# hwwang55/GraphGAN

Measured on AMD Instinct MI355X. Metric: sampled_edges_per_sec, higher is better.
Workload: dtype f32

## Files before the change

graphgan_amd/_lib.py:

```python
from __future__ import annotations

import ctypes
import os

_HERE = os.path.dirname(os.path.abspath(__file__))
LIB_PATH = os.path.join(_HERE, "libgraphgan_hip.so")
HEADER_PATH = os.path.join(os.path.dirname(_HERE), "include", "graphgan_hip.h")
ABI_VERSION = 9


def header_abi_version(path=HEADER_PATH):
    import re
    with open(path) as f:
        m = re.search(r"^#define\s+GG_ABI_VERSION\s+(\d+)", f.read(), flags=re.M)
    if not m:
        raise RuntimeError("GG_ABI_VERSION not found in %s" % path)
    return int(m.group(1))

GG_OK, GG_EINVAL, GG_ECAPACITY, GG_EHIP, GG_ECOMM, GG_ENOMEM, GG_EIO = 0, -1, -2, -3, -4, -5, -6
GG_OPT_ADAM_DENSE, GG_OPT_ADAM_LAZY, GG_OPT_SGD = 0, 1, 2
GG_ROOT_OK, GG_ROOT_ABORTED, GG_ROOT_EMPTY = 0, 1, 2
GG_GS_FOR_D, GG_GS_Q3_STORE = 1, 2
GRAM_MAX_GRID = 512
PAIR_NEIGHBORS_CHUNK = 512
NEIGHBOR_SUM_CHUNK = 512
NEIGHBOR_SUM_MAX_COL = 128
NEIGHBOR_MODE_LDS_CAP = 2048
TWO_HOP_LDS_CAP = 2048
PPR_LDS_CAP = 1024
PARTITION_EDGES_CHUNK = 512
SF_MAX_SWEEPS = 34
ERROR_NAMES = {GG_EINVAL: "GG_EINVAL", GG_ECAPACITY: "GG_ECAPACITY", GG_EHIP: "GG_EHIP", GG_ECOMM: "GG_ECOMM",
               GG_ENOMEM: "GG_ENOMEM", GG_EIO: "GG_EIO"}


class GGConfig(ctypes.Structure):
    _fields_ = [("lr_gen", ctypes.c_float), ("lr_dis", ctypes.c_float),
                ("lambda_gen", ctypes.c_float), ("lambda_dis", ctypes.c_float),
                ("adam_beta1", ctypes.c_float), ("adam_beta2", ctypes.c_float), ("adam_eps", ctypes.c_float),
                ("window_size", ctypes.c_int32), ("optimizer", ctypes.c_int32), ("device", ctypes.c_int32),
                ("reserved", ctypes.c_int32 * 6)]


class GGCounters(ctypes.Structure):
    _fields_ = [("walks", ctypes.c_int64), ("hops", ctypes.c_int64), ("nbr_reads", ctypes.c_int64),
                ("reward_pairs", ctypes.c_int64), ("d_pairs", ctypes.c_int64), ("g_pairs", ctypes.c_int64),
                ("d_steps", ctypes.c_int64), ("g_steps", ctypes.c_int64),
                ("last_kernel_ms", ctypes.c_double), ("walk_kernel_ms", ctypes.c_double),
                ("walk_launches", ctypes.c_int64), ("rows_scored", ctypes.c_int64), ("score_kernel_ms", ctypes.c_double),
                ("score_launches", ctypes.c_int64), ("score_chunks", ctypes.c_int64), ("score_rows", ctypes.c_int64),
                ("bfs_kernel_ms", ctypes.c_double), ("bfs_trees", ctypes.c_int64), ("score_dists", ctypes.c_int64),
                ("reward_kernel_ms", ctypes.c_double), ("reward_pairs_timed", ctypes.c_int64),
                ("d_grad_ms", ctypes.c_double), ("d_opt_ms", ctypes.c_double), ("d_pairs_timed", ctypes.c_int64), ("d_rows_timed", ctypes.c_int64),
                ("g_grad_ms", ctypes.c_double), ("g_opt_ms", ctypes.c_double), ("g_pairs_timed", ctypes.c_int64), ("g_rows_timed", ctypes.c_int64),
                ("d_passes_timed", ctypes.c_int64), ("g_passes_timed", ctypes.c_int64),
                ("g_walk_nodes_timed", ctypes.c_int64),
                ("es_gathers", ctypes.c_int64), ("es_nodes", ctypes.c_int64), ("score_gathers", ctypes.c_int64), ("score_nodes", ctypes.c_int64),
                ("walk_reruns", ctypes.c_int64)]


class GGGraph(ctypes.Structure):
    _fields_ = [("n_node", ctypes.c_int32), ("nnz", ctypes.c_int64), ("n_train_edges", ctypes.c_int64),
                ("n_test_edges", ctypes.c_int64), ("rowptr", ctypes.POINTER(ctypes.c_int64)), ("col", ctypes.POINTER(ctypes.c_int32))]


class GraphGANHipError(RuntimeError):
    def __init__(self, code, msg):
        super().__init__("%s (%d): %s" % (ERROR_NAMES.get(code, "GG_E?"), code, msg))
        self.code = code


_P = ctypes.c_void_p
_i32, _i64, _u32, _u64 = ctypes.c_int32, ctypes.c_int64, ctypes.c_uint32, ctypes.c_uint64

SIGNATURES = {
    "gg_abi_version": (ctypes.c_int, []),
    "gg_last_error": (ctypes.c_char_p, [_P]),
    "gg_create": (ctypes.c_int, [_i32, _i32, _P, _P, ctypes.POINTER(GGConfig), ctypes.POINTER(_P)]),
    "gg_destroy": (ctypes.c_int, [_P]),
    "gg_set_graph_csr": (ctypes.c_int, [_P, _P, _P]),
    "gg_host_build_trees": (_i64, [_i32, _P, _P, _P, _i32, _P, _P, _P, _i64, _i32, _P]),
    "gg_build_trees": (ctypes.c_int, [_P, _P, _i32, _i32]),
    "gg_build_trees_device": (ctypes.c_int, [_P, _P, _i32]),
    "gg_set_tree_mode": (ctypes.c_int, [_P, _i32, _i64]),
    "gg_debug_words": (ctypes.c_int, [_P, _i32, _i32, _P]),
    "gg_lazy_stats": (ctypes.c_int, [_P, _P]),
    "gg_get_lazy_trees": (ctypes.c_int, [_P, _P, _P, _P, _P, _P, _P, _P]),
    "gg_set_trees": (ctypes.c_int, [_P, _P, _i32, _P, _P, _P, _i32]),
    "gg_tree_info": (ctypes.c_int, [_P, _P, _P, _P]),
    "gg_tree_roots": (ctypes.c_int, [_P, _P]),
    "gg_save_trees": (ctypes.c_int, [_P, ctypes.c_char_p]),
    "gg_load_trees": (ctypes.c_int, [_P, ctypes.c_char_p]),
    "gg_get_trees": (ctypes.c_int, [_P, _P, _P, _P]),
    "gg_get_tree_order": (ctypes.c_int, [_P, _P, _P, _P, _P, _P]),
    "gg_walk_sample": (ctypes.c_int, [_P, _P, _P, _i32, _i32, _u64, _u32, _P, _P, _P, _i32, _P]),
    "gg_walk_info": (ctypes.c_int, [_P, _P, _P, _P]),
    "gg_get_walks": (ctypes.c_int, [_P, _P, _P, _P, _P]),
    "gg_prepare_d": (ctypes.c_int, [_P, _P, _i32, _u64, _u32, _P, _P]),
    "gg_get_d_data": (ctypes.c_int, [_P, _P, _P, _P]),
    "gg_prepare_g": (ctypes.c_int, [_P, _P, _i32, _i32, _u64, _u32, _P, _P]),
    "gg_prepare_g_begin": (ctypes.c_int, [_P, _P, _i32, _i32, _u64, _u32]),
    "gg_get_g_data": (ctypes.c_int, [_P, _P, _P, _P]),
    "gg_epoch_begin": (ctypes.c_int, [_P, _i32, _i32]),
    "gg_epoch_add": (ctypes.c_int, [_P, _P, _i32, _i32, _i32, _i32, _u64, _u32, _u32, _P, _P]),
    "gg_epoch_commit": (ctypes.c_int, [_P, _i32, _P]),
    "gg_q3_clear": (ctypes.c_int, [_P]),
    "gg_q3_get": (ctypes.c_int, [_P, _P, _P]),
    "gg_d_pass": (ctypes.c_int, [_P, _P, _i64, _i32]),
    "gg_g_pass": (ctypes.c_int, [_P, _P, _i64, _i32]),
    "gg_pair_reward": (ctypes.c_int, [_P, _P, _P, _i64, _P]),
    "gg_d_step": (ctypes.c_int, [_P, _P, _P, _P, _i32]),
    "gg_g_step": (ctypes.c_int, [_P, _P, _P, _P, _i32]),
    "gg_all_score": (ctypes.c_int, [_P, _P, _i32, _P]),
    "gg_all_score_reduce": (ctypes.c_int, [_P, _P, _i32, _i32, _i32, _P, _P, _P, _P]),
    "gg_topk_scores": (ctypes.c_int, [_P, _i32, _P, _i32, _i32, _i32, _i32, _P, _P, _P]),
    "gg_topk_metric": (ctypes.c_int, [_P, _i32, _P, _i32, _i32, _i32, _i32, _i32, _P, _i64, _P, _P, _P]),
    "gg_rank_scores": (ctypes.c_int, [_P, _i32, _P, _P, _i64, _i32, _i32, _P, _P, _P, _P]),
    "gg_top_pairs": (ctypes.c_int, [_P, _i32, _i32, _P, _i64, _i64, _i32, _i64, _P, _P, _P, _P, _P, _P]),
    "gg_distinct_degrees": (ctypes.c_int, [_P, _P]),
    "gg_pair_neighbors": (ctypes.c_int, [_P, _P, _P, _i64, _P, _i32, _P, _P, _P, _P, _P]),
    "gg_neighbor_sum": (ctypes.c_int, [_P, _P, _i32, _P, _P, _P, _i64, _P, _P]),
    "gg_label_spread": (ctypes.c_int, [_P, _P, _P, _i64, _i32, ctypes.c_double, _i32, _P, _P, _P, _i64, _P, _P, _P]),
    "gg_neighbor_mode": (ctypes.c_int, [_P, _P, _u32, _i32, _P, _i64, _P, _P]),
    "gg_label_propagation": (ctypes.c_int, [_P, _u32, _i32, _P, _P, _P, _P, _P]),
    "gg_partition_edges": (ctypes.c_int, [_P, _P, _i32, _P, _P, _P]),
    "gg_undirected_edges": (ctypes.c_int, [_P, _P, _P]),
    "gg_spanning_forest": (ctypes.c_int, [_P, _u32, _P, _i64, _P, _P, _P, _P, _P, _P]),
    "gg_two_hop_topk": (ctypes.c_int, [_P, _P, _i64, _i32, _P, _i32, _i64, _P, _P, _P, _P]),
    "gg_two_hop_rank": (ctypes.c_int, [_P, _P, _P, _i64, _P, _i32, _i64, _P, _P, _P, _P, _P]),
    "gg_ppr_topk": (ctypes.c_int, [_P, _P, _i64, _i32, _u32, _u64, _i32, _i32, _i64, _P, _P, _P, _P, _P, _P, _P]),
    "gg_ppr_rank": (ctypes.c_int, [_P, _P, _P, _i64, _u32, _u64, _i32, _i32, _i64, _P, _P, _P, _P, _P, _P, _P, _P]),
    "gg_graph_softmax": (ctypes.c_int, [_P, _P, _i32, _i32, _P, _P, _P, _P, _P, _P]),
    "gg_pretrain_set_noise": (ctypes.c_int, [_P, _P]),
    "gg_pretrain_set_walk_bias": (ctypes.c_int, [_P, _u32, _u32, _u32]),
    "gg_prepare_pretrain": (ctypes.c_int, [_P, _P, _i32, _i32, _i32, _i32, _i32, _u64, _u32, _P, _P, _P]),
    "gg_classifier_lossgrad": (ctypes.c_int, [_P, ctypes.c_int, _P, _P, _i64, ctypes.c_int, _P, _P, ctypes.c_float, _P, _P, _P]),
    "gg_classifier_fit": (ctypes.c_int, [_P, ctypes.c_int, _P, _P, _i64, ctypes.c_int, ctypes.c_int, ctypes.c_float, ctypes.c_float, _P, _P, _P, _P]),
    "gg_classifier_predict": (ctypes.c_int, [_P, ctypes.c_int, _P, _i64, ctypes.c_int, _P, _P, _P, _P]),
    "gg_classifier_ml_lossgrad": (ctypes.c_int, [_P, ctypes.c_int, _P, _P, _i64, ctypes.c_int, _P, _P, ctypes.c_float, _P, _P, _P]),
    "gg_classifier_ml_fit": (ctypes.c_int, [_P, ctypes.c_int, _P, _P, _i64, ctypes.c_int, ctypes.c_int, ctypes.c_float, ctypes.c_float, _P, _P, _P, _P]),
    "gg_classifier_ml_predict": (ctypes.c_int, [_P, ctypes.c_int, _P, _i64, ctypes.c_int, _P, _P, _P, _P, _P]),
    "gg_edge_classifier_lossgrad": (ctypes.c_int, [_P, ctypes.c_int, ctypes.c_int, _P, _P, _P, _i64, _P, _P, ctypes.c_float, _P, _P, _P]),
    "gg_edge_classifier_fit": (ctypes.c_int, [_P, ctypes.c_int, ctypes.c_int, _P, _P, _P, _i64, ctypes.c_int, ctypes.c_float, ctypes.c_float,
                                               _P, _P, _P, _P]),
    "gg_edge_classifier_predict": (ctypes.c_int, [_P, ctypes.c_int, ctypes.c_int, _P, _P, _i64, _P, _P, _P]),
    "gg_kmeans_step": (ctypes.c_int, [_P, ctypes.c_int, _P, _i64, ctypes.c_int, _P, _P, _P, _P, _P, _P, _P]),
    "gg_kmeans_fit": (ctypes.c_int, [_P, ctypes.c_int, _P, _i64, ctypes.c_int, ctypes.c_int, _P, _P, _P, _P, _P, _P, _P, _P, _P]),
    "gg_silhouette": (ctypes.c_int, [_P, ctypes.c_int, _P, _P, _i64, ctypes.c_int, _P, _i64, ctypes.c_int, _P, _P, _P, _P, _P, _P]),
    "gg_gram": (ctypes.c_int, [_P, ctypes.c_int, _P, _i64, _P, _P, _P, _P]),
    "gg_get_embeddings": (ctypes.c_int, [_P, _i32, _P]),
    "gg_get_bias": (ctypes.c_int, [_P, _i32, _P]),
    "gg_write_embeddings": (ctypes.c_int, [_P, _i32, ctypes.c_char_p, _i32]),
    "gg_host_write_embeddings": (ctypes.c_int, [_P, _i64, _i32, ctypes.c_char_p, _i32]),
    "gg_write_embeddings_bin": (ctypes.c_int, [_P, _i32, ctypes.c_char_p]),
    "gg_edge_scores": (ctypes.c_int, [_P, _i32, _P, _P, _i64, _P]),
    "gg_set_embeddings": (ctypes.c_int, [_P, _i32, _P]),
    "gg_set_bias": (ctypes.c_int, [_P, _i32, _P]),
    "gg_save_state": (ctypes.c_int, [_P, ctypes.c_char_p]),
    "gg_load_state": (ctypes.c_int, [_P, ctypes.c_char_p]),
    "gg_get_counters": (ctypes.c_int, [_P, ctypes.POINTER(GGCounters)]),
    "gg_set_profiling": (ctypes.c_int, [_P, _i32]),
    "gg_set_profiling_solo": (ctypes.c_int, [_P, _i32]),
    "gg_synchronize": (ctypes.c_int, [_P]),
    "gg_comm_unique_id": (ctypes.c_int, [_P]),
    "gg_comm_init": (ctypes.c_int, [_P, _P, _i32, _i32]),
    "gg_comm_barrier": (ctypes.c_int, [_P]),
    "gg_comm_stats": (ctypes.c_int, [_P, _P]),
    "gg_comm_stats_ex": (ctypes.c_int, [_P, _P]),
    "gg_synth_powerlaw": (_i64, [_i32, _i32, _u64, _u64, _P, _i64]),
    "gg_host_read_edges": (ctypes.c_int, [ctypes.c_char_p, ctypes.c_char_p, ctypes.POINTER(GGGraph)]),
    "gg_host_free_graph": (None, [ctypes.POINTER(GGGraph)]),
}


def _load():
    if not os.path.exists(LIB_PATH):
        raise ImportError(
            "graphgan_amd: %s is missing -- build the HIP extension first "
            "(`make -C graphgan_amd/csrc` or `python -c 'import __graft_entry__ as g; g.build()'`). "
            "There is no CPU fallback." % LIB_PATH)
    lib = ctypes.CDLL(LIB_PATH)
# ... 19 lines not shown
```

graphgan_amd/csrc/epoch.hip:

```cpp
#include <algorithm>
#include <vector>

#include "gg_internal.h"

namespace gg {

int launch_pair_reward(gg_ctx *ctx, const int32_t *d_u, const int32_t *d_v, int64_t n, float *d_out);

__global__ __launch_bounds__(256) void q3_copy_kernel(const int32_t *t_root, const int64_t *t_q3off, uint32_t *t_q3, const int64_t *s_off,
                                                      uint32_t *store, int n_slots, int to_store) {
    const int s = blockIdx.x * blockDim.x + threadIdx.x;
    if (s >= n_slots) return;
    const int v = t_root[s];
    const int64_t a = t_q3off[s], b = s_off[v], words = min(t_q3off[s + 1] - a, s_off[v + 1] - b);
    for (int64_t k = 0; k < words; ++k) {
        if (to_store) store[b + k] = t_q3[a + k];
        else t_q3[a + k] = store[b + k];
    }
}

static int ensure_q3_store(gg_ctx *ctx) {
    if (ctx->q3_store_ready) return GG_OK;
    GG_CHECK(ctx, !ctx->h_rowptr.empty(), GG_EINVAL, "epoch: call gg_set_graph_csr first");
    const int n = ctx->n_node;
// ... 35 lines not shown
    if (rc != GG_OK) return rc;
    if (add) GG_HIP(ctx, hipMemcpyAsync((char *)acc.p + elem * (size_t)have, src.p, elem * (size_t)add, hipMemcpyDeviceToDevice, ctx->stream));
    return GG_OK;
}

}

using namespace gg;

extern "C" {

int gg_epoch_begin(gg_ctx *ctx, int32_t reset_d, int32_t reset_g) {
    if (!ctx) return fail(nullptr, GG_EINVAL, "ctx is NULL");
    GG_HIP(ctx, hipSetDevice(ctx->device));
    int rc = ensure_q3_store(ctx);
    if (rc != GG_OK) return rc;
    if (reset_d) {
        ctx->ep_rows = 0;
        ctx->ep_d_open = true;
    }
    if (reset_g) ctx->ep_pairs = 0;
    return GG_OK;
}

int gg_epoch_add(gg_ctx *ctx, const int32_t *roots, int32_t n_roots, int32_t do_d, int32_t do_g, int32_t n_sample, uint64_t seed,
                 uint32_t stream_d, uint32_t stream_g, int64_t *rows_total_out, int64_t *pairs_total_out) {
    if (!ctx) return fail(nullptr, GG_EINVAL, "ctx is NULL");
    GG_CHECK(ctx, n_roots >= 0 && (roots || n_roots == 0), GG_EINVAL, "gg_epoch_add: bad roots");
    if (n_roots > 1 && (do_d || do_g)) {
        std::vector<int32_t> sorted(roots, roots + n_roots);
        std::sort(sorted.begin(), sorted.end());
        const auto dup = std::adjacent_find(sorted.begin(), sorted.end());
        GG_CHECK(ctx, dup == sorted.end(), GG_EINVAL, "gg_epoch_add: root %d appears twice in one batch", dup == sorted.end() ? -1 : *dup);
    }
    GG_HIP(ctx, hipSetDevice(ctx->device));
    int rc = ensure_q3_store(ctx);
    if (rc != GG_OK) return rc;
    if (n_roots > 0 && (do_d || do_g)) {
        ctx->in_epoch_add = true;
        rc = gg_build_trees_device(ctx, roots, n_roots);
        ctx->in_epoch_add = false;
        if (rc != GG_OK) return rc;
        rc = q3_copy(ctx, n_roots, false);
        if (rc != GG_OK) return rc;
        std::vector<int32_t> &slots = ctx->ep_slots;
        if ((int32_t)slots.size() < n_roots) {
            const int32_t old = (int32_t)slots.size();
            slots.resize(n_roots);
            for (int32_t i = old; i < n_roots; ++i) slots[i] = i;
        }
        ctx->in_epoch_add = true;
        if (do_d) {
            ctx->ep_d_open = true;
            int64_t rows = 0;
            rc = gg_prepare_d(ctx, slots.data(), n_roots, seed, stream_d, &rows, nullptr);
            if (rc == GG_OK) rc = q3_copy(ctx, n_roots, true);
            if (rc == GG_OK) rc = append(ctx, ctx->ep_center, ctx->d_center, ctx->ep_rows, rows, sizeof(int32_t));
            if (rc == GG_OK) rc = append(ctx, ctx->ep_neighbor, ctx->d_neighbor, ctx->ep_rows, rows, sizeof(int32_t));
            if (rc == GG_OK) rc = append(ctx, ctx->ep_label, ctx->d_label, ctx->ep_rows, rows, sizeof(float));
            if (rc == GG_OK) ctx->ep_rows += rows;
        }
        if (rc == GG_OK && do_g) {
            int64_t pairs = 0;
            rc = gg_prepare_g(ctx, slots.data(), n_roots, n_sample, seed, stream_g, &pairs, nullptr);
            if (rc == GG_OK) rc = ensure_g_pairs(ctx);
            if (rc == GG_OK) rc = append(ctx, ctx->ep_node1, ctx->g_node1, ctx->ep_pairs, pairs, sizeof(int32_t));
            if (rc == GG_OK) rc = append(ctx, ctx->ep_node2, ctx->g_node2, ctx->ep_pairs, pairs, sizeof(int32_t));
            if (rc == GG_OK) ctx->ep_pairs += pairs;
        }
        ctx->in_epoch_add = false;
        if (rc != GG_OK) return rc;
        GG_HIP(ctx, hipStreamSynchronize(ctx->stream));
    }
    if (rows_total_out) *rows_total_out = ctx->ep_rows;
    if (pairs_total_out) *pairs_total_out = ctx->ep_pairs;
    return GG_OK;
}

int gg_epoch_commit(gg_ctx *ctx, int32_t which, int64_t *n_out) {
    if (!ctx) return fail(nullptr, GG_EINVAL, "ctx is NULL");
    GG_CHECK(ctx, which == 0 || which == 1, GG_EINVAL, "gg_epoch_commit: which must be 0 (generator pairs) or 1 (discriminator rows)");
    GG_HIP(ctx, hipSetDevice(ctx->device));
    discard_begun_walk(ctx);
    GG_HIP(ctx, hipStreamSynchronize(ctx->stream));
    int rc;
    if (which == 1) {
        const int64_t rows = ctx->ep_rows;
        GG_HIP(ctx, ctx->ep_center.reserve(sizeof(int32_t)));
        GG_HIP(ctx, ctx->ep_neighbor.reserve(sizeof(int32_t)));
        GG_HIP(ctx, ctx->ep_label.reserve(sizeof(float)));
        std::swap(ctx->d_center, ctx->ep_center);
        std::swap(ctx->d_neighbor, ctx->ep_neighbor);
        std::swap(ctx->d_label, ctx->ep_label);
        ctx->d_rows = rows;
        ctx->ep_rows = 0;
        ctx->ep_d_open = false;
        rc = exchange_count_max(ctx, ctx->d_rows, &ctx->d_rows_max);
        if (rc != GG_OK) return rc;
        if (n_out) *n_out = rows;
    } else {
        const int64_t pairs = ctx->ep_pairs;
        GG_HIP(ctx, ctx->ep_node1.reserve(sizeof(int32_t)));
        GG_HIP(ctx, ctx->ep_node2.reserve(sizeof(int32_t)));
        GG_HIP(ctx, ctx->ep_reward.reserve(sizeof(float) * (size_t)(pairs + 1)));
        rc = launch_pair_reward(ctx, ctx->ep_node1.as<int32_t>(), ctx->ep_node2.as<int32_t>(), pairs, ctx->ep_reward.as<float>());
        if (rc != GG_OK) return rc;
        GG_HIP(ctx, hipStreamSynchronize(ctx->stream));
        std::swap(ctx->g_node1, ctx->ep_node1);
        std::swap(ctx->g_node2, ctx->ep_node2);
        std::swap(ctx->g_reward, ctx->ep_reward);
        ctx->g_pairs = pairs;
        ctx->g_pairs_filled = true;
        ctx->g_paths_valid = false;
        ctx->ep_pairs = 0;
        rc = exchange_count_max(ctx, ctx->g_pairs, &ctx->g_pairs_max);
        if (rc != GG_OK) return rc;
        if (n_out) *n_out = pairs;
    }
    return GG_OK;
}

int gg_q3_clear(gg_ctx *ctx) {
    if (!ctx) return fail(nullptr, GG_EINVAL, "ctx is NULL");
    GG_HIP(ctx, hipSetDevice(ctx->device));
    int rc = ensure_q3_store(ctx);
    if (rc != GG_OK) return rc;
    GG_HIP(ctx, hipStreamSynchronize(ctx->stream));
    GG_HIP(ctx, hipMemset(ctx->q3_store.p, 0, sizeof(uint32_t) * (size_t)std::max<int64_t>(ctx->q3_words, 1)));
    return GG_OK;
}

int gg_q3_get(gg_ctx *ctx, int64_t *word_off , uint32_t *words ) {
    if (!ctx) return fail(nullptr, GG_EINVAL, "ctx is NULL");
    GG_HIP(ctx, hipSetDevice(ctx->device));
    int rc = ensure_q3_store(ctx);
    if (rc != GG_OK) return rc;
    GG_HIP(ctx, hipStreamSynchronize(ctx->stream));
    if (word_off) GG_HIP(ctx, hipMemcpy(word_off, ctx->q3s_off.p, sizeof(int64_t) * (ctx->n_node + 1), hipMemcpyDeviceToHost));
    if (words && ctx->q3_words) GG_HIP(ctx, hipMemcpy(words, ctx->q3_store.p, sizeof(uint32_t) * (size_t)ctx->q3_words, hipMemcpyDeviceToHost));
    return GG_OK;
}

}
```

graphgan_amd/csrc/gg_api.hip:

```cpp
#include <stdarg.h>
#include <stdlib.h>
#include <string.h>
#include <sys/stat.h>
#include <unistd.h>

#include <algorithm>
#include <atomic>
#include <thread>

#include "gg_internal.h"

namespace gg {

thread_local std::string g_last_error;

int fail(gg_ctx *ctx, int code, const char *fmt, ...) {
    char buf[1024];
    va_list ap;
    va_start(ap, fmt);
    vsnprintf(buf, sizeof(buf), fmt, ap);
    va_end(ap);
    g_last_error = buf;
    if (ctx) ctx->err = buf;
    return code;
// ... 132 lines not shown
    }
    return GG_OK;
}

void gg::discard_begun_walk(gg_ctx *ctx) {
    if (!ctx->g_begun) return;
    (void)hipStreamSynchronize(ctx->stream2);
    ctx->g_begun = false;
    ctx->dc_request = 0;
    ctx->walk_stream = ctx->stream;
    ctx->w_nslots = 0;
    ctx->w_total = 0;
    generator_changed(ctx);
}

int gg::walk_launch_async(gg_ctx *ctx, const int32_t *slots, const int32_t *n_walks, int32_t uniform_walks, int32_t n_slots,
                          int32_t for_d, uint64_t seed, uint32_t stream, int32_t stride, bool side_stream, bool defer_join) {
    discard_begun_walk(ctx);
    GG_CHECK(ctx, ctx->n_tree_roots > 0 || n_slots == 0, GG_EINVAL, "walk: no trees loaded (gg_build_trees / gg_set_trees)");
    GG_CHECK(ctx, n_slots >= 0 && (slots || n_slots == 0), GG_EINVAL, "walk: bad slots");
    GG_CHECK(ctx, stride >= 2, GG_ECAPACITY, "walk: stride %d < 2", stride);
    std::vector<int64_t> &ptr = ctx->h_ptr_new;
    ptr.assign(n_slots + 1, 0);
    for (int i = 0; i < n_slots; ++i) {
        GG_CHECK(ctx, slots[i] >= 0 && slots[i] < ctx->n_tree_roots, GG_EINVAL, "walk: slot %d out of range", slots[i]);
        int64_t nw;
        if (n_walks) nw = n_walks[i];
        else if (uniform_walks >= 0) nw = uniform_walks;
        else {
            GG_CHECK(ctx, !ctx->h_rowptr.empty(), GG_EINVAL, "walk: graph CSR needed for D-mode degrees");
            const int r = ctx->h_troot[slots[i]];
            nw = ctx->h_rowptr[r + 1] - ctx->h_rowptr[r];
        }
        GG_CHECK(ctx, nw >= 0, GG_EINVAL, "walk: negative n_walks");
        ptr[i + 1] = ptr[i] + nw;
    }
    const int64_t total = ptr[n_slots];
    GG_HIP(ctx, hipSetDevice(ctx->device));
    const int mode = for_d ? 1 : 0;
    ctx->w_mode = mode;
    GG_HIP(ctx, ctx->w_slots_m[mode].reserve(sizeof(int32_t) * (n_slots + 1)));
    GG_HIP(ctx, ctx->w_ptr_m[mode].reserve(sizeof(int64_t) * (n_slots + 1)));
    GG_HIP(ctx, ctx->w_status.reserve(sizeof(int32_t) * (n_slots + 1)));
    GG_HIP(ctx, ctx->w_abort.reserve(sizeof(int32_t) * (n_slots + 1)));
    GG_HIP(ctx, ctx->w_samples.reserve(sizeof(int32_t) * (total + 1)));
    GG_HIP(ctx, ctx->w_len.reserve(sizeof(int32_t) * (total + 1)));
    GG_HIP(ctx, ctx->w_first.reserve(sizeof(int32_t) * (total + 1)));
    GG_HIP(ctx, ctx->w_paths.reserve(sizeof(int32_t) * ((size_t)total * stride + 1)));
    ctx->walk_stream = side_stream ? ctx->stream2 : ctx->stream;
    if (side_stream && ctx->gen_dirty) {
        GG_HIP(ctx, hipEventRecord(ctx->ev_main_mark, ctx->stream));
        GG_HIP(ctx, hipStreamWaitEvent(ctx->stream2, ctx->ev_main_mark, 0));
        ctx->gen_dirty = false;
    } else if (side_stream && ctx->gen_pass_recorded) {
        GG_HIP(ctx, hipStreamWaitEvent(ctx->stream2, ctx->ev_gen_pass, 0));
    }
    std::vector<int32_t> &hs = ctx->h_slots_m[mode];
    if (hs.size() != (size_t)n_slots || (n_slots && memcmp(hs.data(), slots, sizeof(int32_t) * n_slots) != 0)) {
        hs.assign(slots, slots + n_slots);
        if (n_slots) GG_HIP(ctx, hipMemcpyAsync(ctx->w_slots_m[mode].p, hs.data(), sizeof(int32_t) * n_slots, hipMemcpyHostToDevice, ctx->walk_stream));
    }
    if (ctx->h_ptr_m[mode] != ptr) {
        ctx->h_ptr_m[mode].swap(ptr);
        GG_HIP(ctx, hipMemcpyAsync(ctx->w_ptr_m[mode].p, ctx->h_ptr_m[mode].data(), sizeof(int64_t) * (n_slots + 1), hipMemcpyHostToDevice, ctx->walk_stream));
    }
    ctx->w_total = total;
    ctx->w_stride = stride;
    ctx->w_nslots = n_slots;
    ctx->w_uniform = (!n_walks && uniform_walks >= 0) ? uniform_walks : -1;
    ctx->w_args = {for_d, seed, stream};
    ctx->g_paths_valid = false;
    if (ctx->g_slots_ready) {
        GG_HIP(ctx, hipStreamWaitEvent(ctx->stream, ctx->ev_slots_done, 0));
        ctx->g_slots_ready = false;
        ctx->g_slots_unused++;
    }
    if (n_slots == 0) {
        ctx->walk_stream = ctx->stream;
        return GG_OK;
    }
    return launch_and_join(ctx, n_slots, total, for_d, seed, stream, stride, !defer_join);
}

int gg::walk_finalize(gg_ctx *ctx, bool *retried) {
    if (retried) *retried = false;
    if (ctx->w_nslots == 0) {
        GG_HIP(ctx, hipStreamSynchronize(ctx->stream));
        return GG_OK;
    }
    const int64_t total = ctx->w_total;
    unsigned long long *c = ctx->h_pin;
    constexpr int CW = gg_ctx::CTR_WORDS;
    GG_HIP(ctx, hipMemcpyAsync(c, ctx->dev_ctr, sizeof(unsigned long long) * 2 * CW, hipMemcpyDeviceToHost, ctx->stream));
    GG_HIP(ctx, hipStreamSynchronize(ctx->stream));
    harvest_timings(ctx);
    for (int attempt = 0; c[3] == 2ull || (c[2] != 0ull && ctx->t_lazy); ++attempt) {
        GG_CHECK(ctx, attempt < 16, GG_EHIP, "walk: the launch was voided %d times in a row", attempt);
        if (c[2] != 0ull && ctx->t_lazy) {
            int rebuilt = 0;
            int rc = lazy_fallback_rebuild(ctx, &rebuilt);
            if (rc == GG_ECAPACITY) rc = lazy_rebuild_whole(ctx);
            if (rc != GG_OK) return rc;
            if (ctx->dc_request == 2) ctx->dc_request = 0;
            if (ctx->tree_max_depth + 3 > ctx->w_stride) {
                ctx->w_stride = ctx->tree_max_depth + 3;
                GG_HIP(ctx, ctx->w_paths.reserve(sizeof(int32_t) * ((size_t)total * ctx->w_stride + 1)));
            }
        } else {
            ctx->walk_force_sized = true;
        }
        ctx->ctr.walk_reruns += 1;
        generator_changed(ctx);
        int rc = launch_and_join(ctx, ctx->w_nslots, total, ctx->w_args.for_d, ctx->w_args.seed, ctx->w_args.stream, ctx->w_stride);
        ctx->walk_force_sized = false;
        if (rc != GG_OK) return rc;
        GG_HIP(ctx, hipMemcpyAsync(c, ctx->dev_ctr, sizeof(unsigned long long) * 2 * CW, hipMemcpyDeviceToHost, ctx->stream));
        GG_HIP(ctx, hipStreamSynchronize(ctx->stream));
        if (retried) *retried = true;
    }
    const int n_half = ctx->w_split ? 2 : 1;
    if (n_half == 2)
        for (int i = 8; i < CW; ++i) c[i] += c[CW + i];
    {
        int64_t *prof = ctx->alive_prof[ctx->w_args.for_d ? 1 : 0];
        const int run = ctx->w_levels_run;
        for (int i = 0; i < 64; ++i) prof[i] = i < run ? (int64_t)c[8 + i] : -1;
        if (run > 0 && run < 64 && ctx->w_fin_follows) prof[run] = (int64_t)c[7];
        if (ctx->w_net && c[7] > 2048ull && ctx->lv_levels_learned < ctx->tree_max_depth + 2) ctx->lv_levels_learned += 1;
    }
    unsigned long long hops = c[0], reads = c[1], rows = c[5];
    unsigned long long gathers = 0, nodes = 0;
    for (int i = 0; i < 64; ++i) { hops += c[264 + i]; reads += c[328 + i]; rows += c[200 + i]; gathers += c[520 + i]; nodes += c[584 + i]; }
    ctx->ctr.es_gathers += (int64_t)gathers;
    ctx->ctr.es_nodes += (int64_t)nodes;
    ctx->ctr.hops += (int64_t)hops;
    ctx->ctr.nbr_reads += (int64_t)reads;
    ctx->ctr.rows_scored += (int64_t)rows;
    ctx->ctr.walks += total;
    if (total && ctx->walk_timed) {
        float ms = 0.f;
        GG_HIP(ctx, hipEventElapsedTime(&ms, ctx->ev0, ctx->ev1));
        ctx->ctr.last_kernel_ms = ms;
        ctx->ctr.walk_kernel_ms += ms;
        ctx->ctr.walk_launches += 1;
        for (int i = 0; i < ctx->lv_ev_used; ++i) {
            float lms = 0.f;
            for (int k = 0; k < n_half; ++k) {
                float e = 0.f;
                GG_HIP(ctx, hipEventElapsedTime(&e, ctx->lv_ev[4 * i + 2 * k], ctx->lv_ev[4 * i + 2 * k + 1]));
                lms += e;
            }
            ctx->ctr.score_kernel_ms += lms;
            ctx->ctr.score_launches += n_half;
            ctx->ctr.score_chunks += (int64_t)(c[136 + i] >> 32);
            if (getenv("GG_WALK_DEBUG"))
                fprintf(stderr, "[walk] for_d=%d level %d alive %llu score chunks %llu prefix chunks %llu big %llu small %llu rows %llu score %.1f us\n", ctx->w_args.for_d, i,
                        c[8 + i], c[136 + i] >> 32, c[136 + i] & 0xffffffffull, c[72 + i] & 0xffffffffull, c[72 + i] >> 32, c[456 + i], lms * 1e3);
        }
        if (ctx->lv_ev_used) {
            ctx->ctr.score_rows += (int64_t)(rows - c[5]);
            unsigned long long dists = 0;
            for (int i = 0; i < 64; ++i) dists += c[392 + i];
            ctx->ctr.score_dists += (int64_t)dists;
            ctx->ctr.score_gathers += (int64_t)gathers;
            ctx->ctr.score_nodes += (int64_t)nodes;
        }
    }
    if (c[3] || c[6]) generator_changed(ctx);
    if (c[3]) return fail(ctx, GG_ECAPACITY, "walk: a path needed more than stride=%d entries", ctx->w_stride);
    if (c[6]) return fail(ctx, GG_EINVAL, "walk: non-finite generator scores (a softmax had total weight 0, or the generator's tables hold a non-finite value)");
    return GG_OK;
}

int gg::walk_resident(gg_ctx *ctx, const int32_t *slots, const int32_t *n_walks, int32_t uniform_walks, int32_t n_slots,
                      int32_t for_d, uint64_t seed, uint32_t stream, int32_t stride) {
    int rc = walk_launch_async(ctx, slots, n_walks, uniform_walks, n_slots, for_d, seed, stream, stride);
    if (rc != GG_OK) return rc;
    return walk_finalize(ctx, nullptr);
}

extern "C" {

int gg_abi_version(void) { return GG_ABI_VERSION; }

const char *gg_last_error(const gg_ctx *ctx) { return ctx ? ctx->err.c_str() : g_last_error.c_str(); }

int gg_create(int32_t n_node, int32_t n_emb, const float *emb_gen, const float *emb_dis, const gg_config *cfg,
              gg_ctx **out) {
    if (!out) return fail(nullptr, GG_EINVAL, "gg_create: out is NULL");
    *out = nullptr;
    if (n_node <= 0 || n_emb <= 0 || n_emb > 512 || !emb_gen || !emb_dis || !cfg)
        return fail(nullptr, GG_EINVAL, "gg_create: bad argument (n_node=%d n_emb=%d)", n_node, n_emb);
    if (cfg->window_size < 1) return fail(nullptr, GG_EINVAL, "gg_create: window_size = %d is below 1", cfg->window_size);
    int ndev = 0;
    hipError_t e = hipGetDeviceCount(&ndev);
    if (e != hipSuccess || ndev <= 0)
        return fail(nullptr, GG_EHIP, "gg_create: no HIP device (%s); this engine has no CPU fallback",
                    e == hipSuccess ? "count = 0" : hipGetErrorString(e));
    if (cfg->device < 0 || cfg->device >= ndev) return fail(nullptr, GG_EINVAL, "gg_create: device %d of %d", cfg->device, ndev);
    hipDeviceProp_t prop;
    GG_HIP(nullptr, hipGetDeviceProperties(&prop, cfg->device));
    if (strncmp(prop.gcnArchName, "gfx950", 6) != 0)
        return fail(nullptr, GG_EHIP, "gg_create: device %d is %s; kernels are built for gfx950 only", cfg->device, prop.gcnArchName);
    GG_HIP(nullptr, hipSetDevice(cfg->device));

    gg_ctx *ctx = new gg_ctx();
    ctx->n_node = n_node;
    ctx->n_emb = n_emb;
    ctx->ld = (n_emb + 3) / 4 * 4;
    ctx->cfg = *cfg;
    ctx->device = cfg->device;
    ctx->n_cus = prop.multiProcessorCount > 0 ? prop.multiProcessorCount : 256;
    if (const char *lv = getenv("GG_WALK_LEVELS")) ctx->walk_levels = atoi(lv);
    if (const char *pe = getenv("GG_PROFILE_EVERY")) ctx->profile_every = std::max(0, atoi(pe));
    if (const char *fw = getenv("GG_COMM_FAKE_WORLD")) ctx->fake_world = atoi(fw);
    if (const char *ow = getenv("GG_COMM_OWNER")) ctx->owner_exchange = atoi(ow);
    if (const char *bf = getenv("GG_COMM_BF16")) ctx->comm_bf16 = atoi(bf) != 0;
    if (const char *om = getenv("GG_COMM_OWNER_MIN")) ctx->owner_min_bound = atoll(om);
    if (const char *dt = getenv("GG_DETERMINISTIC")) ctx->deterministic = atoi(dt) != 0;
    if (const char *nc = getenv("GG_NO_DIST_CACHE")) ctx->dc_enabled = atoi(nc) == 0;
    if (const char *ft = getenv("GG_FIN_THRESHOLD")) ctx->fin_threshold = std::max(0, atoi(ft));
    if (const char *st = getenv("GG_STAGE_T")) ctx->sg_threshold = std::max(0, atoi(st));
    if (const char *ws = getenv("GG_WALK_SPLIT")) ctx->split_enabled = atoi(ws) != 0;
    if (const char *em = getenv("GG_ES_MODE")) ctx->es_mode = std::min(2, std::max(0, atoi(em)));
    if (const char *er = getenv("GG_ES_RATIO")) ctx->es_ratio_num = std::max(1, atoi(er));
    if (const char *eh = getenv("GG_ES_HUB")) ctx->es_hub = std::max(0, atoi(eh));
    if (const char *wm = getenv("GG_WALK_SPLIT_MIN")) ctx->split_min_walks = std::max(512, atoi(wm));
    for (auto &m : ctx->alive_prof) for (auto &v : m) v = -1;
    if (const char *dr = getenv("GG_COMM_DENSE_RATIO")) ctx->dense_exchange_ratio = (float)atof(dr);
#define GG_TRY(call)                        \
    do {                                    \
        int rc__ = (call);                  \
        if (rc__ != GG_OK) {                \
            g_last_error = ctx->err;        \
            gg_destroy(ctx);                \
            return rc__;                    \
        }                                   \
    } while (0)
    auto body = [&]() -> int {
        GG_HIP(ctx, hipStreamCreateWithFlags(&ctx->stream, hipStreamNonBlocking));
        {
            int lo = 0, hi = 0;
            const char *wp = getenv("GG_WALK_PRIORITY");
            if (wp && atoi(wp) != 0 && hipDeviceGetStreamPriorityRange(&lo, &hi) == hipSuccess && hi != lo)
                GG_HIP(ctx, hipStreamCreateWithPriority(&ctx->stream2, hipStreamNonBlocking, atoi(wp) > 0 ? hi : lo));
            else
                GG_HIP(ctx, hipStreamCreateWithFlags(&ctx->stream2, hipStreamNonBlocking));
        }
        GG_HIP(ctx, hipStreamCreateWithFlags(&ctx->stream3, hipStreamNonBlocking));
        GG_HIP(ctx, hipEventCreateWithFlags(&ctx->ev_fork, hipEventDisableTiming));
        GG_HIP(ctx, hipEventCreateWithFlags(&ctx->ev_join, hipEventDisableTiming));
        GG_HIP(ctx, hipEventCreateWithFlags(&ctx->ev_score[0], hipEventDisableTiming));
        GG_HIP(ctx, hipEventCreateWithFlags(&ctx->ev_score[1], hipEventDisableTiming));
        ctx->walk_stream = ctx->stream;
        GG_HIP(ctx, hipEventCreate(&ctx->ev0));
        GG_HIP(ctx, hipEventCreate(&ctx->ev1));
        GG_HIP(ctx, hipEventCreateWithFlags(&ctx->ev_walk_done, hipEventDisableTiming));
        GG_HIP(ctx, hipEventCreateWithFlags(&ctx->ev_gen_pass, hipEventDisableTiming));
        GG_HIP(ctx, hipEventCreateWithFlags(&ctx->ev_main_mark, hipEventDisableTiming));
        GG_HIP(ctx, hipHostMalloc((void **)&ctx->h_pin, sizeof(unsigned long long) * gg_ctx::PIN_WORDS, hipHostMallocDefault));
        memset(ctx->h_pin, 0, sizeof(unsigned long long) * gg_ctx::PIN_WORDS);
        const size_t tb = sizeof(float) * (size_t)n_node * ctx->ld, vb = sizeof(float) * (size_t)n_node;
        for (int m = 0; m < 2; ++m) {
            Model &M = ctx->model[m];
            GG_HIP(ctx, hipMalloc((void **)&M.E, tb));
            GG_HIP(ctx, hipMalloc((void **)&M.b, vb));
            GG_HIP(ctx, hipMemset(M.b, 0, vb));
            if (cfg->optimizer != GG_OPT_SGD) {
                GG_HIP(ctx, hipMalloc((void **)&M.mE, tb));
                GG_HIP(ctx, hipMalloc((void **)&M.vE, tb));
                GG_HIP(ctx, hipMalloc((void **)&M.mb, vb));
                GG_HIP(ctx, hipMalloc((void **)&M.vb, vb));
                GG_HIP(ctx, hipMemset(M.mE, 0, tb));
                GG_HIP(ctx, hipMemset(M.vE, 0, tb));
                GG_HIP(ctx, hipMemset(M.mb, 0, vb));
                GG_HIP(ctx, hipMemset(M.vb, 0, vb));
            }
            M.b1p = cfg->adam_beta1;
            M.b2p = cfg->adam_beta2;
            M.lr = m == 0 ? cfg->lr_gen : cfg->lr_dis;
            M.lambda = m == 0 ? cfg->lambda_gen : cfg->lambda_dis;
            int rc = upload_table(ctx, M.E, m == 0 ? emb_gen : emb_dis);
            if (rc != GG_OK) return rc;
        }
        GG_HIP(ctx, hipMalloc((void **)&ctx->gradE, tb));
        GG_HIP(ctx, hipMalloc((void **)&ctx->gradb, vb));
        GG_HIP(ctx, hipMemset(ctx->gradE, 0, tb));
        ctx->grad_elems_padded = (size_t)n_node * ctx->ld;
        GG_HIP(ctx, hipMemset(ctx->gradb, 0, vb));
        GG_HIP(ctx, hipMalloc((void **)&ctx->touched, sizeof(int32_t) * n_node));
        GG_HIP(ctx, hipMalloc((void **)&ctx->touched_list, sizeof(int32_t) * n_node));
        GG_HIP(ctx, hipMalloc((void **)&ctx->touched_cnt, sizeof(int32_t) * 4));
        GG_HIP(ctx, hipMemset(ctx->touched, 0, sizeof(int32_t) * n_node));
        GG_HIP(ctx, hipMemset(ctx->touched_cnt, 0, sizeof(int32_t) * 4));
        GG_HIP(ctx, hipMalloc((void **)&ctx->dev_ctr, sizeof(unsigned long long) * gg_ctx::PIN_WORDS));
        GG_HIP(ctx, hipMemset(ctx->dev_ctr, 0, sizeof(unsigned long long) * gg_ctx::PIN_WORDS));
        GG_HIP(ctx, ctx->table_bad.reserve(sizeof(unsigned long long) * 2));
        for (int m = 0; m < 2; ++m) {
            int rc = rescan_table_finite(ctx, m);
            if (rc != GG_OK) return rc;
        }
        GG_HIP(ctx, hipDeviceSynchronize());
        return GG_OK;
    };
    GG_TRY(body());
#undef GG_TRY
    *out = ctx;
    return GG_OK;
}

int gg_destroy(gg_ctx *ctx) {
    if (!ctx) return GG_OK;
    (void)hipSetDevice(ctx->device);
    if (ctx->stream) (void)hipStreamSynchronize(ctx->stream);
    if (ctx->stream2) (void)hipStreamSynchronize(ctx->stream2);
    comm_destroy(ctx);
    for (int m = 0; m < 2; ++m) {
        Model &M = ctx->model[m];
        float *ps[] = {M.E, M.b, M.mE, M.vE, M.mb, M.vb};
        for (float *p : ps)
            if (p) (void)hipFree(p);
    }
    void *ps[] = {ctx->gradE, ctx->gradb, ctx->touched, ctx->touched_list, ctx->touched_cnt, ctx->g_rowptr, ctx->g_col, ctx->dev_ctr,
                  ctx->es, ctx->es_stamp, ctx->g_rev};
    for (void *p : ps)
        if (p) (void)hipFree(p);
    free_trees(ctx);
    DevBuf *bufs[] = {&ctx->w_slots_m[0], &ctx->w_slots_m[1], &ctx->w_ptr_m[0], &ctx->w_ptr_m[1], &ctx->w_samples, &ctx->w_paths, &ctx->w_len, &ctx->w_status,
                      &ctx->w_first, &ctx->w_abort, &ctx->w_scratch, &ctx->d_center, &ctx->d_neighbor, &ctx->d_label, &ctx->d_cnt,
                      &ctx->d_ptr, &ctx->g_node1, &ctx->g_node2, &ctx->g_reward, &ctx->g_cnt, &ctx->g_ptr, &ctx->scan_tmp,
                      &ctx->step_u, &ctx->step_v, &ctx->step_x, &ctx->sg_rows, &ctx->sg_bias, &ctx->touched_ptr, &ctx->x_cnt, &ctx->x_send_ids, &ctx->x_send_rows,
                      &ctx->x_recv_ids, &ctx->x_recv_rows, &ctx->x_nglob, &ctx->x_own, &ctx->st_item, &ctx->st_item2, &ctx->st_cur, &ctx->st_prev, &ctx->st_len,
                      &ctx->st_alive, &ctx->st_rank, &ctx->bfs_key, &ctx->bfs_bm, &ctx->bfs_misc, &ctx->bfs_sparse, &ctx->bfs_rowptr32, &ctx->lv_pfx, &ctx->dc_keys, &ctx->dc_vals, &ctx->dc_words, &ctx->lv_beg, &ctx->lv_k, &ctx->lv_chunks, &ctx->lv_coff, &ctx->lv_scores, &ctx->lv_chunk_owner, &ctx->lv_prefix, &ctx->lv_big, &ctx->lv_fe, &ctx->fin_list, &ctx->table_bad, &ctx->hub_acc,
                      &ctx->q3_store, &ctx->q3s_off, &ctx->ep_center, &ctx->ep_neighbor, &ctx->ep_label, &ctx->ep_node1, &ctx->ep_node2, &ctx->ep_reward, &ctx->topk_adj,
                      &ctx->gs_es, &ctx->gs_cpre, &ctx->pt_starts, &ctx->pt_paths, &ctx->pt_len, &ctx->pt_cnt, &ctx->pt_ptr, &ctx->pt_noise, &ctx->pt_sample};
    for (DevBuf *b : bufs) b->release();
    ctx->set.release();
    for (StageIndex *ix : {&ctx->sg_own, &ctx->sg_early}) ix->release();
    for (hipEvent_t e : ctx->lv_ev)
        if (e) (void)hipEventDestroy(e);
    for (auto &tr : ctx->tm_ev)
        for (hipEvent_t e : tr)
            if (e) (void)hipEventDestroy(e);
    for (hipEvent_t e : ctx->pt_ev)
        if (e) (void)hipEventDestroy(e);
    if (ctx->h_pin) (void)hipHostFree(ctx->h_pin);
    for (hipEvent_t e : {ctx->ev_walk_done, ctx->ev_slots_done, ctx->ev_gen_pass, ctx->ev_main_mark, ctx->ev_fork, ctx->ev_join, ctx->ev_score[0], ctx->ev_score[1]})
        if (e) (void)hipEventDestroy(e);
    if (ctx->stream3) {
        (void)hipStreamSynchronize(ctx->stream3);
        (void)hipStreamDestroy(ctx->stream3);
    }
    if (ctx->stream2) {
        (void)hipStreamSynchronize(ctx->stream2);
        (void)hipStreamDestroy(ctx->stream2);
    }
    if (ctx->ev0) (void)hipEventDestroy(ctx->ev0);
    if (ctx->ev1) (void)hipEventDestroy(ctx->ev1);
    if (ctx->stream) (void)hipStreamDestroy(ctx->stream);
    delete ctx;
    return GG_OK;
}

int gg_set_graph_csr(gg_ctx *ctx, const int64_t *rowptr, const int32_t *col) {
    if (!ctx) return fail(nullptr, GG_EINVAL, "ctx is NULL");
    GG_CHECK(ctx, rowptr && rowptr[0] == 0, GG_EINVAL, "gg_set_graph_csr: rowptr[0] must be 0");
    discard_begun_walk(ctx);
    const int n = ctx->n_node;
    const int64_t nnz = rowptr[n];
    GG_CHECK(ctx, nnz >= 0 && (col || nnz == 0), GG_EINVAL, "gg_set_graph_csr: col is NULL");
    for (int v = 0; v < n; ++v) GG_CHECK(ctx, rowptr[v + 1] >= rowptr[v], GG_EINVAL, "gg_set_graph_csr: rowptr not monotone at %d", v);
    for (int64_t e = 0; e < nnz; ++e) GG_CHECK(ctx, col[e] >= 0 && col[e] < n, GG_EINVAL, "gg_set_graph_csr: col[%lld]=%d out of range", (long long)e, col[e]);
    GG_HIP(ctx, hipSetDevice(ctx->device));
    (void)hipDeviceSynchronize();
    for (void *p : {(void *)ctx->g_rowptr, (void *)ctx->g_col, (void *)ctx->es, (void *)ctx->es_stamp, (void *)ctx->g_rev})
        if (p) (void)hipFree(p);
    ctx->g_rowptr = nullptr;
    ctx->g_col = nullptr;
    ctx->es = nullptr;
    ctx->es_stamp = nullptr;
    ctx->g_rev = nullptr;
    ctx->t_edge_valid = false;
    ctx->q3_store_ready = false;
    ctx->bfs_rowptr32_valid = false;
    ctx->topk_adj.release();
    ctx->topk_adj_valid = false;
    ctx->set.drop();
    ctx->gs_es_valid = ctx->gs_cpre_valid = false;
    ctx->pt_noise_set = false;
    GG_HIP(ctx, hipMalloc((void **)&ctx->g_rowptr, sizeof(int64_t) * (n + 1)));
    GG_HIP(ctx, hipMalloc((void **)&ctx->g_col, sizeof(int32_t) * (std::max<int64_t>(nnz, 1) + 4)));
    GG_HIP(ctx, hipMemcpy(ctx->g_rowptr, rowptr, sizeof(int64_t) * (n + 1), hipMemcpyHostToDevice));
    if (nnz) GG_HIP(ctx, hipMemcpy(ctx->g_col, col, sizeof(int32_t) * nnz, hipMemcpyHostToDevice));
    ctx->g_nnz = nnz;
    ctx->g_max_deg = 0;
    for (int v = 0; v < n; ++v) ctx->g_max_deg = (int32_t)std::min<int64_t>(std::max<int64_t>(ctx->g_max_deg, rowptr[v + 1] - rowptr[v]), 0x7fffffff);
    ctx->g_multi = true;
    ctx->h_rowptr.assign(rowptr, rowptr + n + 1);
    ctx->h_col.assign(col, col + nnz);
    ctx->h_comp_size.clear();
    uint64_t h = 1469598103934665603ull;
    for (int v = 0; v <= n; ++v) h = (h ^ (uint64_t)rowptr[v]) * 1099511628211ull;
    for (int64_t e = 0; e + 1 < nnz; e += 2) h = (h ^ ((uint64_t)(uint32_t)col[e] | ((uint64_t)(uint32_t)col[e + 1] << 32))) * 1099511628211ull;
    if (nnz & 1) h = (h ^ (uint64_t)(uint32_t)col[nnz - 1]) * 1099511628211ull;
    ctx->g_hash = h;
    if (nnz > 0 && nnz < (1ll << 31)) {
        hipError_t e = hipMalloc((void **)&ctx->es, sizeof(float) * (size_t)nnz);
        if (e == hipSuccess) e = hipMalloc((void **)&ctx->es_stamp, sizeof(long long) * (size_t)n);
        if (e == hipSuccess) e = hipMalloc((void **)&ctx->g_rev, sizeof(int32_t) * (size_t)nnz);
        if (e == hipSuccess) e = hipMemset(ctx->es_stamp, 0, sizeof(long long) * (size_t)n);
        generator_changed(ctx);
        int rc = e == hipSuccess ? compute_reverse_edges(ctx) : GG_ENOMEM;
        if (rc != GG_OK) {
            (void)hipGetLastError();
            for (void *p : {(void *)ctx->es, (void *)ctx->es_stamp, (void *)ctx->g_rev})
                if (p) (void)hipFree(p);
            ctx->es = nullptr;
            ctx->es_stamp = nullptr;
            ctx->g_rev = nullptr;
            if (getenv("GG_WALK_DEBUG")) fprintf(stderr, "[graph] edge-score cache not allocated (%s): walks score privately\n", e == hipSuccess ? ctx->err.c_str() : hipGetErrorString(e));
        }
    }
    return GG_OK;
}

int gg_build_trees(gg_ctx *ctx, const int32_t *roots, int32_t n_roots, int32_t n_threads) {
    if (!ctx) return fail(nullptr, GG_EINVAL, "ctx is NULL");
    GG_CHECK(ctx, !ctx->h_rowptr.empty(), GG_EINVAL, "gg_build_trees: call gg_set_graph_csr first");
    GG_CHECK(ctx, n_roots >= 0 && (roots || n_roots == 0), GG_EINVAL, "gg_build_trees: bad roots");
    const int n = ctx->n_node;
// ... 240 lines not shown
                              sizeof(int32_t) * (2 * (size_t)h.nodes + (size_t)h.n_roots);
        if (fstat(fileno(f), &st) != 0 || (size_t)st.st_size != expect)
            rc = fail(ctx, GG_EIO, "gg_load_trees: %s is truncated (%lld bytes, expected %zu)", path, (long long)st.st_size, expect);
    }
    if (rc == GG_OK) {
        roots.resize(h.n_roots);
        base.resize((size_t)h.n_roots + 1);
        if (fread(roots.data(), sizeof(int32_t), h.n_roots, f) != (size_t)h.n_roots || fread(base.data(), sizeof(int64_t), (size_t)h.n_roots + 1, f) != (size_t)h.n_roots + 1)
            rc = fail(ctx, GG_EIO, "gg_load_trees: short read");
    }
    if (rc == GG_OK) {
        counts.resize(h.n_roots);
        for (int r = 0; r < h.n_roots && rc == GG_OK; ++r) {
            counts[r] = base[r + 1] - base[r];
            if (roots[r] < 0 || roots[r] >= ctx->n_node || counts[r] < 1 || counts[r] > ctx->n_node) rc = fail(ctx, GG_EIO, "gg_load_trees: %s: bad root table", path);
        }
        if (rc == GG_OK && (base[0] != 0 || base[h.n_roots] != h.nodes)) rc = fail(ctx, GG_EIO, "gg_load_trees: %s: bad root table", path);
    }
    if (rc == GG_OK) rc = alloc_trees(ctx, roots.data(), h.n_roots, counts.data(), nullptr);
    if (rc == GG_OK) rc = stream_dev(ctx, f, ctx->t_order, (size_t)h.nodes, false);
    if (rc == GG_OK) rc = stream_dev(ctx, f, ctx->t_cstart, (size_t)h.nodes + h.n_roots, false);
    fclose(f);
    if (rc == GG_OK) {
        int32_t *bad = (int32_t *)(ctx->dev_ctr + 2000);
        int32_t h_bad = 0;
        hipError_t e = hipMemset(bad, 0, sizeof(int32_t));
        if (e == hipSuccess) {
            hipLaunchKernelGGL(validate_trees_kernel, dim3((unsigned)cdiv(h.nodes, 256)), dim3(256), 0, ctx->stream, ctx->t_order, ctx->t_cstart,
                               ctx->t_base, ctx->t_root, h.n_roots, ctx->n_node, bad);
            e = hipStreamSynchronize(ctx->stream);
        }
        if (e == hipSuccess) e = hipMemcpy(&h_bad, bad, sizeof(int32_t), hipMemcpyDeviceToHost);
        if (e == hipSuccess) e = hipMemset(bad, 0, sizeof(int32_t));
        if (e != hipSuccess) rc = fail(ctx, GG_EHIP, "gg_load_trees: %s", hipGetErrorString(e));
        else if (h_bad || h.max_depth < 0 || h.max_depth > ctx->n_node || h.max_list < 0 || h.max_list > ctx->n_node)
            rc = fail(ctx, GG_EIO, "gg_load_trees: %s: the tree arrays are corrupt (node id out of range or child ranges not a BFS order)", path);
    }
    if (rc != GG_OK) {
        ctx->n_tree_roots = 0;
        ctx->tree_nodes = 0;
        return rc;
    }
    ctx->tree_max_depth = h.max_depth;
    ctx->tree_max_list = h.max_list;
    return derive_tree_edges(ctx);
}

int gg_walk_sample(gg_ctx *ctx, const int32_t *slots, const int32_t *n_walks, int32_t n_slots, int32_t for_d,
                   uint64_t seed, uint32_t stream, int32_t *samples, int32_t *paths, int32_t *path_len, int32_t stride,
                   int32_t *root_status) {
    if (!ctx) return fail(nullptr, GG_EINVAL, "ctx is NULL");
    GG_CHECK(ctx, n_walks || n_slots == 0, GG_EINVAL, "gg_walk_sample: n_walks is NULL");
    ctx->dc_request = 0;
    ctx->dc_valid = false;
    int rc = walk_resident(ctx, slots, n_walks, -1, n_slots, for_d ? 1 : 0, seed, stream, stride);
    if (rc != GG_OK) return rc;
    const int64_t total = ctx->w_total;
    if (samples && total) GG_HIP(ctx, hipMemcpy(samples, ctx->w_samples.p, sizeof(int32_t) * total, hipMemcpyDeviceToHost));
    if (path_len && total) GG_HIP(ctx, hipMemcpy(path_len, ctx->w_len.p, sizeof(int32_t) * total, hipMemcpyDeviceToHost));
    if (paths && total && ctx->w_stride == stride) GG_HIP(ctx, hipMemcpy(paths, ctx->w_paths.p, sizeof(int32_t) * (size_t)total * stride, hipMemcpyDeviceToHost));
    if (ctx->w_stride != stride && total) {
        std::vector<int32_t> len((size_t)total);
        GG_HIP(ctx, hipMemcpy(len.data(), ctx->w_len.p, sizeof(int32_t) * total, hipMemcpyDeviceToHost));
        for (int64_t w = 0; w < total; ++w)
            GG_CHECK(ctx, len[w] <= stride, GG_ECAPACITY, "walk: a path needed %d entries, stride is %d (gg_tree_info reports the depth of the trees as rebuilt)", len[w], stride);
        if (paths) GG_HIP(ctx, hipMemcpy2D(paths, sizeof(int32_t) * (size_t)stride, ctx->w_paths.p, sizeof(int32_t) * (size_t)ctx->w_stride, sizeof(int32_t) * (size_t)stride, (size_t)total, hipMemcpyDeviceToHost));
    }
    if (root_status && n_slots) GG_HIP(ctx, hipMemcpy(root_status, ctx->w_status.p, sizeof(int32_t) * n_slots, hipMemcpyDeviceToHost));
    return GG_OK;
}

int gg_debug_words(gg_ctx *ctx, int32_t first, int32_t n, uint64_t *out) {
    if (!ctx || !out || first < 0 || n < 0 || first + n > gg_ctx::PIN_WORDS) return fail(ctx, GG_EINVAL, "gg_debug_words: bad argument");
    GG_HIP(ctx, hipSetDevice(ctx->device));
    hipStream_t s;
    GG_HIP(ctx, hipStreamCreateWithFlags(&s, hipStreamNonBlocking));
    hipError_t e = hipMemcpyAsync(out, ctx->dev_ctr + first, sizeof(uint64_t) * (size_t)n, hipMemcpyDeviceToHost, s);
    if (e == hipSuccess) e = hipStreamSynchronize(s);
    (void)hipStreamDestroy(s);
    GG_HIP(ctx, e);
    return GG_OK;
}

int gg_set_tree_mode(gg_ctx *ctx, int32_t mode, int64_t node_cap) {
    if (!ctx) return fail(nullptr, GG_EINVAL, "ctx is NULL");
    GG_CHECK(ctx, mode >= -1 && mode <= 1 && node_cap >= 0, GG_EINVAL, "gg_set_tree_mode: mode must be -1 (auto), 0 (whole trees) or 1 (lazy), node_cap >= 0");
    ctx->tree_mode = mode;
    ctx->lz_cap = node_cap;
    return GG_OK;
}

int gg_lazy_stats(gg_ctx *ctx, int64_t *out8) {
    if (!ctx || !out8) return fail(ctx, GG_EINVAL, "gg_lazy_stats: NULL argument");
    GG_HIP(ctx, hipSetDevice(ctx->device));
    for (int i = 0; i < 24; ++i) out8[i] = 0;
    out8[0] = ctx->t_lazy ? 1 : 0;
    out8[1] = ctx->t_lazy ? ctx->lz_min_level : 0;
    out8[2] = ctx->lz_fallback_roots;
    out8[3] = ctx->lz_fallback_rounds;
    if (ctx->t_lazy && ctx->n_tree_roots > 0) {
        GG_HIP(ctx, hipStreamSynchronize(ctx->stream));
        const int R = ctx->n_tree_roots;
        std::vector<int4> info((size_t)R);
        std::vector<int32_t> cur((size_t)R);
        GG_HIP(ctx, hipMemcpy(info.data(), ctx->lz_info.p, sizeof(int4) * (size_t)R, hipMemcpyDeviceToHost));
        GG_HIP(ctx, hipMemcpy(cur.data(), ctx->lz_cursor.p, sizeof(int32_t) * (size_t)R, hipMemcpyDeviceToHost));
        for (int r = 0; r < R; ++r) {
            out8[4] += info[r].y;
            out8[5] += std::max(0, cur[r] - info[r].y);
            out8[6] += info[r].x < info[r].y ? 1 : 0;
            out8[7] = std::max<int64_t>(out8[7], info[r].z);
            if (info[r].x < info[r].y && info[r].z >= 0 && info[r].z < 8) out8[16 + info[r].z] += 1;
        }
        unsigned long long c[8];
        GG_HIP(ctx, hipMemcpy(c, ctx->dev_ctr + 1500, sizeof(c), hipMemcpyDeviceToHost));
        for (int i = 0; i < 8; ++i) out8[8 + i] = (int64_t)c[i];
    }
    return GG_OK;
}

int gg_get_lazy_trees(gg_ctx *ctx, int64_t *n_entries, int32_t *info4, int64_t *base, int32_t *order, int32_t *cstart, int32_t *edge, uint64_t *pair) {
    if (!ctx) return fail(nullptr, GG_EINVAL, "ctx is NULL");
    GG_CHECK(ctx, ctx->t_lazy, GG_EINVAL, "gg_get_lazy_trees: the resident trees are not lazy");
    GG_HIP(ctx, hipSetDevice(ctx->device));
    GG_HIP(ctx, hipDeviceSynchronize());
    const size_t R = (size_t)ctx->n_tree_roots, nodes = (size_t)ctx->arena_end;
    if (n_entries) *n_entries = (int64_t)nodes;
    if (info4) GG_HIP(ctx, hipMemcpy(info4, ctx->lz_info.p, sizeof(int4) * R, hipMemcpyDeviceToHost));
    if (base) GG_HIP(ctx, hipMemcpy(base, ctx->t_base, sizeof(int64_t) * R, hipMemcpyDeviceToHost));
    if (order) GG_HIP(ctx, hipMemcpy(order, ctx->t_order, sizeof(int32_t) * nodes, hipMemcpyDeviceToHost));
    if (cstart) GG_HIP(ctx, hipMemcpy(cstart, ctx->t_cstart, sizeof(int32_t) * (nodes + R), hipMemcpyDeviceToHost));
    if (edge) GG_HIP(ctx, hipMemcpy(edge, ctx->t_edge, sizeof(int32_t) * nodes, hipMemcpyDeviceToHost));
    if (pair) GG_HIP(ctx, hipMemcpy(pair, ctx->lz_pair.p, sizeof(uint64_t) * std::min(nodes, ctx->lz_pair.bytes / sizeof(uint64_t)), hipMemcpyDeviceToHost));
    return GG_OK;
}

int gg_walk_info(const gg_ctx *ctx, int64_t *total_walks, int32_t *stride, int32_t *n_slots) {
    if (!ctx) return fail(nullptr, GG_EINVAL, "ctx is NULL");
    if (total_walks) *total_walks = ctx->w_total;
    if (stride) *stride = ctx->w_stride;
    if (n_slots) *n_slots = ctx->w_nslots;
    return GG_OK;
}

int gg_get_walks(gg_ctx *ctx, int32_t *samples, int32_t *paths, int32_t *path_len, int32_t *root_status) {
    if (!ctx) return fail(nullptr, GG_EINVAL, "ctx is NULL");
    GG_HIP(ctx, hipSetDevice(ctx->device));
    const bool begun = ctx->g_begun;
    discard_begun_walk(ctx);
    GG_CHECK(ctx, !begun, GG_EINVAL, "gg_get_walks: the walks of the last completed launch were overwritten by gg_prepare_g_begin (fetch them before it, or after the gg_prepare_g that adopts it)");
    GG_HIP(ctx, hipStreamSynchronize(ctx->stream));
    const int64_t total = ctx->w_total;
    if (samples && total) GG_HIP(ctx, hipMemcpy(samples, ctx->w_samples.p, sizeof(int32_t) * total, hipMemcpyDeviceToHost));
    if (path_len && total) GG_HIP(ctx, hipMemcpy(path_len, ctx->w_len.p, sizeof(int32_t) * total, hipMemcpyDeviceToHost));
    if (paths && total) GG_HIP(ctx, hipMemcpy(paths, ctx->w_paths.p, sizeof(int32_t) * (size_t)total * ctx->w_stride, hipMemcpyDeviceToHost));
    if (root_status && ctx->w_nslots) GG_HIP(ctx, hipMemcpy(root_status, ctx->w_status.p, sizeof(int32_t) * ctx->w_nslots, hipMemcpyDeviceToHost));
    return GG_OK;
}

static int table_io(gg_ctx *ctx, int32_t which, float *out, const float *in, bool bias) {
    if (!ctx) return fail(nullptr, GG_EINVAL, "ctx is NULL");
    GG_CHECK(ctx, which == 0 || which == 1, GG_EINVAL, "which must be 0 (gen) or 1 (dis)");
    GG_CHECK(ctx, out || in, GG_EINVAL, "buffer is NULL");
    GG_HIP(ctx, hipSetDevice(ctx->device));
    GG_HIP(ctx, hipStreamSynchronize(ctx->stream));
    Model &M = ctx->model[which];
    const int n = ctx->n_node, d = ctx->n_emb, ld = ctx->ld;
    if (in && which == 0) { discard_begun_walk(ctx); generator_changed(ctx); }
    if (bias) {
        if (out) GG_HIP(ctx, hipMemcpy(out, M.b, sizeof(float) * n, hipMemcpyDeviceToHost));
        else GG_HIP(ctx, hipMemcpy(M.b, in, sizeof(float) * n, hipMemcpyHostToDevice));
    } else if (out) {
        GG_HIP(ctx, hipMemcpy2D(out, sizeof(float) * d, M.E, sizeof(float) * ld, sizeof(float) * d, n, hipMemcpyDeviceToHost));
    } else {
        int rc = upload_table(ctx, M.E, in);
        if (rc != GG_OK) return rc;
    }
    if (in) return rescan_table_finite(ctx, which);
    return GG_OK;
}

int gg_get_embeddings(gg_ctx *ctx, int32_t which, float *out) { return table_io(ctx, which, out, nullptr, false); }
int gg_get_bias(gg_ctx *ctx, int32_t which, float *out) { return table_io(ctx, which, out, nullptr, true); }
int gg_set_embeddings(gg_ctx *ctx, int32_t which, const float *emb) { return table_io(ctx, which, nullptr, emb, false); }
int gg_set_bias(gg_ctx *ctx, int32_t which, const float *bias) { return table_io(ctx, which, nullptr, bias, true); }

int gg_get_counters(gg_ctx *ctx, gg_counters *out) {
    if (!ctx || !out) return fail(ctx, GG_EINVAL, "gg_get_counters: NULL argument");
    if (!ctx->tm_pending.empty()) {
        GG_HIP(ctx, hipSetDevice(ctx->device));
        GG_HIP(ctx, hipStreamSynchronize(ctx->stream));
        harvest_timings(ctx);
    }
    *out = ctx->ctr;
    return GG_OK;
}

int gg_set_profiling_solo(gg_ctx *ctx, int32_t solo) {
    if (!ctx) return fail(nullptr, GG_EINVAL, "ctx is NULL");
    ctx->profile_solo = solo != 0;
    return GG_OK;
}

int gg_set_profiling(gg_ctx *ctx, int32_t every_n) {
    if (!ctx) return fail(nullptr, GG_EINVAL, "ctx is NULL");
    GG_CHECK(ctx, every_n >= 0, GG_EINVAL, "gg_set_profiling: every_n < 0");
    ctx->profile_every = every_n;
    ctx->walk_call_index = 0;
    return GG_OK;
}

int gg_synchronize(gg_ctx *ctx) {
    if (!ctx) return fail(nullptr, GG_EINVAL, "ctx is NULL");
    GG_HIP(ctx, hipSetDevice(ctx->device));
    GG_HIP(ctx, hipStreamSynchronize(ctx->stream));
    if (ctx->g_begun) GG_HIP(ctx, hipStreamSynchronize(ctx->stream2));
    harvest_timings(ctx);
    return check_exchange_flag(ctx);
}

}

int gg::check_exchange_flag(gg_ctx *ctx) {
    if (!ctx->comm && ctx->fake_world <= 1) return GG_OK;
    int32_t flag = 0;
    GG_HIP(ctx, hipMemcpy(&flag, ctx->touched_cnt + 2, sizeof(int32_t), hipMemcpyDeviceToHost));
    if (flag) return fail(ctx, GG_ECOMM, "replica exchange: a rank touched more rows than the pack capacity of its step");
    return GG_OK;
}

void gg::harvest_timings(gg_ctx *ctx) {
    size_t keep = 0;
    for (size_t i = 0; i < ctx->tm_pending.size(); ++i) {
        const gg_ctx::PendingTiming t = ctx->tm_pending[i];
        hipEvent_t *ev = ctx->tm_ev[t.slot];
        if (hipEventQuery(ev[2]) != hipSuccess) {
            ctx->tm_pending[keep++] = t;
            continue;
        }
        float a = 0.f, b = 0.f;
        (void)hipEventElapsedTime(&a, ev[0], ev[1]);
        (void)hipEventElapsedTime(&b, ev[1], ev[2]);
        const int64_t rows = t.has_rows ? (int64_t)ctx->h_pin[gg_ctx::H_ROWS + t.slot] : (int64_t)ctx->n_node;
        if (t.kind == 0) {
            ctx->ctr.reward_kernel_ms += a + b;
            ctx->ctr.reward_pairs_timed += t.units;
        } else if (t.kind == 1) {
            ctx->ctr.d_grad_ms += a; ctx->ctr.d_opt_ms += b;
            ctx->ctr.d_pairs_timed += t.units; ctx->ctr.d_rows_timed += rows; ctx->ctr.d_passes_timed += 1;
        } else {
            ctx->ctr.g_grad_ms += a; ctx->ctr.g_opt_ms += b;
            ctx->ctr.g_pairs_timed += t.units; ctx->ctr.g_rows_timed += rows; ctx->ctr.g_passes_timed += 1;
        }
    }
    ctx->tm_pending.resize(keep);
}

int gg::timing_slot(gg_ctx *ctx) {
    for (int s = 0; s < 8; ++s) {
        bool busy = false;
        for (const auto &t : ctx->tm_pending) busy |= t.slot == s;
        if (busy) continue;
        for (int k = 0; k < 3; ++k)
            if (!ctx->tm_ev[s][k] && hipEventCreate(&ctx->tm_ev[s][k]) != hipSuccess) return -1;
        return s;
    }
    return -1;
}

namespace {
struct StateHeader {
    char magic[4];
    int32_t version, n_node, n_emb, ld, optimizer;
};

int io_dev(gg_ctx *ctx, FILE *f, float *dev, size_t count, bool save, std::vector<float> &tmp) {
    tmp.resize(count);
    if (save) {
        GG_HIP(ctx, hipMemcpy(tmp.data(), dev, sizeof(float) * count, hipMemcpyDeviceToHost));
        if (fwrite(tmp.data(), sizeof(float), count, f) != count) return gg::fail(ctx, GG_EIO, "state: short write");
    } else {
        if (fread(tmp.data(), sizeof(float), count, f) != count) return gg::fail(ctx, GG_EIO, "state: short read");
        GG_HIP(ctx, hipMemcpy(dev, tmp.data(), sizeof(float) * count, hipMemcpyHostToDevice));
    }
    return GG_OK;
}

int state_io(gg_ctx *ctx, const char *path, bool save) {
    if (!ctx) return gg::fail(nullptr, GG_EINVAL, "ctx is NULL");
    GG_CHECK(ctx, path, GG_EINVAL, "state: path is NULL");
    GG_HIP(ctx, hipSetDevice(ctx->device));
    GG_HIP(ctx, hipStreamSynchronize(ctx->stream));
    if (!save) discard_begun_walk(ctx);
    const bool slots = ctx->cfg.optimizer != GG_OPT_SGD;
    const size_t ne = (size_t)ctx->n_node * ctx->ld, nb = (size_t)ctx->n_node;
    struct Scalars { int64_t t; float b1p, b2p; };
    const size_t per_model = sizeof(Scalars) + sizeof(float) * (ne + nb) * (slots ? 3 : 1);
    const size_t expect = sizeof(StateHeader) + 2 * per_model;
    const std::string tmp_path = std::string(path) + ".tmp";
    FILE *f = fopen(save ? tmp_path.c_str() : path, save ? "wb" : "rb");
    if (!f) return gg::fail(ctx, GG_EIO, "state: cannot open %s", save ? tmp_path.c_str() : path);
    StateHeader h{{'G', 'G', 'S', 'T'}, 1, ctx->n_node, ctx->n_emb, ctx->ld, ctx->cfg.optimizer};
    int rc = GG_OK;
    if (save) {
        if (fwrite(&h, sizeof(h), 1, f) != 1) rc = gg::fail(ctx, GG_EIO, "state: short write");
    } else {
        StateHeader g;
        if (fread(&g, sizeof(g), 1, f) != 1 || memcmp(g.magic, "GGST", 4) != 0 || g.version != 1)
            rc = gg::fail(ctx, GG_EIO, "state: %s is not a GGST v1 file", path);
        else if (g.n_node != h.n_node || g.n_emb != h.n_emb || g.ld != h.ld || (g.optimizer == GG_OPT_SGD) != (h.optimizer == GG_OPT_SGD))
            rc = gg::fail(ctx, GG_EINVAL, "state: shape/optimizer mismatch (file %dx%d opt %d)", g.n_node, g.n_emb, g.optimizer);
        if (rc == GG_OK) {
            struct stat st;
            if (fstat(fileno(f), &st) != 0 || (size_t)st.st_size != expect)
                rc = gg::fail(ctx, GG_EIO, "state: %s is truncated or has trailing bytes (%lld bytes, expected %zu); nothing was loaded", path,
                              (long long)st.st_size, expect);
        }
    }
    std::vector<float> tmp;
    Scalars loaded[2] = {};
    for (int m = 0; m < 2 && rc == GG_OK; ++m) {
        gg::Model &M = ctx->model[m];
        Scalars sc{M.t, M.b1p, M.b2p};
        if (save) {
            if (fwrite(&sc, sizeof(sc), 1, f) != 1) rc = gg::fail(ctx, GG_EIO, "state: short write");
        } else {
            if (fread(&sc, sizeof(sc), 1, f) != 1) rc = gg::fail(ctx, GG_EIO, "state: short read");
            else loaded[m] = sc;
        }
        if (rc == GG_OK) rc = io_dev(ctx, f, M.E, ne, save, tmp);
        if (rc == GG_OK) rc = io_dev(ctx, f, M.b, nb, save, tmp);
        if (slots) {
            if (rc == GG_OK) rc = io_dev(ctx, f, M.mE, ne, save, tmp);
            if (rc == GG_OK) rc = io_dev(ctx, f, M.vE, ne, save, tmp);
            if (rc == GG_OK) rc = io_dev(ctx, f, M.mb, nb, save, tmp);
            if (rc == GG_OK) rc = io_dev(ctx, f, M.vb, nb, save, tmp);
        }
    }
    if (save) {
        if (rc == GG_OK && (fflush(f) != 0 || fsync(fileno(f)) != 0)) rc = gg::fail(ctx, GG_EIO, "state: cannot flush %s", tmp_path.c_str());
        fclose(f);
        if (rc == GG_OK && rename(tmp_path.c_str(), path) != 0) rc = gg::fail(ctx, GG_EIO, "state: cannot rename %s to %s", tmp_path.c_str(), path);
        if (rc != GG_OK) (void)remove(tmp_path.c_str());
        return rc;
    }
    fclose(f);
    generator_changed(ctx);
    for (int m = 0; m < 2; ++m) {
        const int rs = gg::rescan_table_finite(ctx, m);
        if (rc == GG_OK) rc = rs;
    }
    if (rc == GG_OK)
        for (int m = 0; m < 2; ++m) { ctx->model[m].t = loaded[m].t; ctx->model[m].b1p = loaded[m].b1p; ctx->model[m].b2p = loaded[m].b2p; }
    return rc;
}
}

extern "C" int gg_save_state(gg_ctx *ctx, const char *path) { return state_io(ctx, path, true); }
extern "C" int gg_load_state(gg_ctx *ctx, const char *path) { return state_io(ctx, path, false); }
```

graphgan_amd/csrc/gg_internal.h:

```cpp
#pragma once
#include <hip/hip_runtime.h>
#include <stdint.h>
#include <stdio.h>
#include <string>
#include <vector>

#include "../../include/graphgan_hip.h"

namespace gg {

struct DevBuf {
    void *p = nullptr;
    size_t bytes = 0;
    hipError_t reserve(size_t need) {
        if (need <= bytes) return hipSuccess;
        if (p) {
            (void)hipDeviceSynchronize();
            (void)hipFree(p);
        }
        p = nullptr;
        bytes = 0;
        size_t want = need + need / 4 + 256;
        hipError_t e = hipMalloc(&p, want);
        if (e == hipSuccess) bytes = want;
// ... 143 lines not shown
    std::vector<int32_t> h_comp_size;

    int32_t tree_mode = -1;
    int64_t lz_cap = 0;
    bool t_lazy = false;
    bool lz_force_whole = false;
    int32_t lz_min_level = 0x7fffffff;
    uint32_t lz_stamp = 0;
    gg::DevBuf lz_info, lz_pair, lz_rank, lz_bm, lz_cursor, lz_flag, lz_limit, lz_expect, lz_list, lz_scratch, lz_fb_scratch;
    int64_t arena_next = 0, arena_end = 0;
    int64_t lz_fallback_roots = 0, lz_fallback_rounds = 0, lz_resolved = 0;
    bool g_multi = true;
    int32_t g_max_deg = 0;

    gg::DevBuf w_slots_m[2], w_ptr_m[2];
    std::vector<int32_t> h_slots_m[2];
    std::vector<int64_t> h_ptr_m[2], h_ptr_new;
    int w_mode = 0;
    int64_t alive_prof[2][64];
    int64_t fin_threshold = 0;
    int w_levels_run = 0;
    bool w_fin_follows = false;
    bool w_net = false;
    const gg::DevBuf &w_slots_buf() const { return w_slots_m[w_mode]; }
    const gg::DevBuf &w_ptr_buf() const { return w_ptr_m[w_mode]; }
    gg::DevBuf w_samples, w_paths, w_len, w_status, w_first, w_abort, w_scratch;
    gg::DevBuf st_cur, st_prev, st_len, st_alive, st_rank, st_item, st_item2, lv_beg, lv_k, lv_chunks, lv_coff, lv_scores, lv_chunk_owner, lv_prefix, lv_big, lv_fe;
    gg::DevBuf lv_pfx, dc_keys, dc_vals, dc_words;
    size_t dc_size = 0;
    int32_t dc_request = 0;
    bool dc_valid = false;
    bool dc_enabled = true;
    int64_t lv_cap_total = 0;
    int32_t lv_levels_learned = 0;
    int64_t lv_cap_chunks = 0;
    bool walk_force_sized = false;
    bool walk_used_speculation = false;
    int32_t walk_levels = 64;
    int64_t w_total = 0;
    int32_t w_stride = 0, w_nslots = 0;
    int32_t w_uniform = -1;
    struct { int32_t for_d; uint64_t seed; uint32_t stream; } w_args{};

    static constexpr int CTR_WORDS = 720;
    static constexpr int PIN_WORDS = 2048;
    static constexpr int H_TOTAL = 1960;
    static constexpr int H_ROWS = 1940;
    unsigned long long *h_pin = nullptr;
    int32_t profile_every = 1;
    int64_t walk_call_index = 0;
    bool walk_timed = false;
    bool profile_solo = true;
    struct PendingTiming { int kind; int64_t units; int slot; bool has_rows; };
    hipEvent_t tm_ev[8][3] = {};
    std::vector<PendingTiming> tm_pending;
    int64_t pass_call_index[2] = {0, 0};
    int tm_cur = -1;

    gg::DevBuf d_center, d_neighbor, d_label, d_cnt, d_ptr;
    int64_t d_rows = 0;
    gg::DevBuf g_node1, g_node2, g_reward, g_cnt, g_ptr;
    int64_t g_pairs = 0;
    bool g_paths_valid = false;
    bool g_begun = false;
    struct { int32_t n_slots = 0, n_sample = 0; uint64_t seed = 0; uint32_t stream = 0; } g_begun_args;
    gg::DevBuf touched_ptr;
    gg::DevBuf bfs_key, bfs_bm, bfs_misc, bfs_sparse, bfs_rowptr32;
    bool bfs_rowptr32_valid = false;
    gg::DevBuf q3_store, q3s_off;
    int64_t q3_words = 0;
    bool q3_store_ready = false;
    gg::DevBuf ep_center, ep_neighbor, ep_label, ep_node1, ep_node2, ep_reward;
    int64_t ep_rows = 0, ep_pairs = 0;
    std::vector<int32_t> ep_slots;
    bool in_epoch_add = false;
    int n_cus = 256;
    gg::DevBuf scan_tmp, step_u, step_v, step_x;
    bool g_pairs_filled = false;
    gg::StageIndex sg_own, sg_early;
    hipEvent_t ev_slots_done = nullptr;
    bool g_slots_ready = false;
    int64_t g_slots_walks = 0; int32_t g_slots_stride = 0;
    int g_slots_unused = 0;
    const gg::StageIndex *sg_applying = nullptr;
    gg::DevBuf sg_rows, sg_bias, hub_acc;
    int64_t hub_cap = 0;
    int sg_threshold = 64;

    unsigned long long *dev_ctr = nullptr;
    gg_counters ctr{};

    void *comm = nullptr;
    bool comm_rsag = true;
    size_t grad_elems_padded = 0;
    int64_t d_rows_max = 0, g_pairs_max = 0;
    int64_t step_bound = 0;
    int64_t comm_steps_sparse = 0, comm_steps_dense = 0, comm_bytes_sent = 0;
    int32_t rank = 0, world = 1;
    bool deterministic = true;
    float dense_exchange_ratio = 1.5f;
    int32_t fake_world = 0;
    gg::DevBuf x_cnt, x_send_ids, x_send_rows, x_recv_ids, x_recv_rows;
    gg::DevBuf x_nglob;
    gg::DevBuf x_own;
    int32_t owner_exchange = 1;
    bool comm_bf16 = false;
    int64_t owner_min_bound = 4096;
    int64_t comm_steps_owner = 0;

    gg::DevBuf topk_adj;
    bool topk_adj_valid = false;

    gg::SetGraph set;

    gg::DevBuf gs_es, gs_cpre;
    int64_t gs_chunks = 0;
    bool gs_es_valid = false, gs_cpre_valid = false;

    gg::DevBuf pt_starts, pt_paths, pt_len, pt_cnt, pt_ptr, pt_noise, pt_sample;
    bool pt_noise_set = false;
    uint64_t pt_noise_total = 0;
    int32_t pt_sample_n = 0, pt_sample_stride = 1;
    uint32_t pt_bias[3] = {1, 1, 1};
    hipEvent_t pt_ev[4] = {};
    bool ep_d_open = false;

    std::string err;
};

namespace gg {

extern thread_local std::string g_last_error;

int fail(gg_ctx *ctx, int code, const char *fmt, ...);

#define GG_HIP(ctx, call)                                                                      \
    do {                                                                                       \
        hipError_t e__ = (call);                                                               \
        if (e__ != hipSuccess)                                                                 \
            return gg::fail(ctx, GG_EHIP, "%s:%d %s -> %s", __FILE__, __LINE__, #call,         \
                            hipGetErrorString(e__));                                           \
    } while (0)

#define GG_HIP_FN(call)                                                                            \
    do {                                                                                           \
        const hipError_t e__ = (call);                                                             \
        if (e__ != hipSuccess) return gg::fail(ctx, GG_EHIP, "%s: %s", fn, hipGetErrorString(e__)); \
    } while (0)

#define GG_CHECK(ctx, cond, code, ...)                        \
    do {                                                      \
        if (!(cond)) return gg::fail(ctx, code, __VA_ARGS__); \
    } while (0)

int device_exclusive_scan(gg_ctx *ctx, const int32_t *cnt, int64_t *ptr, int64_t n);
int ensure_sorted_adjacency(gg_ctx *ctx);
int ensure_set_adjacency(gg_ctx *ctx);
int ensure_g_pairs(gg_ctx *ctx);
int device_compact_flags(gg_ctx *ctx, const int32_t *flag, int64_t n, int32_t *list, int64_t *total_out);
int device_segment_rows(gg_ctx *ctx, const int32_t *cnt, int64_t n, int T, int32_t *off, int4 *list, int64_t *totals, hipStream_t stream = nullptr,
                        DevBuf *scratch = nullptr);

int alloc_trees(gg_ctx *ctx, const int32_t *roots, int32_t n_roots, const int64_t *node_counts, const int64_t *root_children, int64_t extra_nodes = 0);
bool lazy_build_wanted(const gg_ctx *ctx);
int lazy_rebuild_whole(gg_ctx *ctx);
int lazy_fallback_rebuild(gg_ctx *ctx, int *n_out);
void component_sizes(int n, const int64_t *rowptr, const int32_t *col, std::vector<int32_t> &comp_size);
int32_t host_bfs_order(const int64_t *rowptr, const int32_t *col, int32_t root, int32_t *order, int32_t *cstart,
                       std::vector<uint32_t> &stamp, uint32_t &epoch, int32_t *depth_out, int32_t *max_children_out);
void order_to_lists(int32_t n, int32_t C, const int32_t *order, const int32_t *cstart, const uint32_t *q3, int32_t *off, int32_t *nbr);
int32_t lists_to_order(int32_t n, int32_t root, const int32_t *off, const int32_t *nbr, int32_t *order, int32_t *cstart,
                       uint32_t *q3, int32_t q3_words, int32_t *depth_out, int32_t *max_children_out);

int walk_launch_async(gg_ctx *ctx, const int32_t *slots, const int32_t *n_walks, int32_t uniform_walks, int32_t n_slots,
                      int32_t for_d, uint64_t seed, uint32_t stream, int32_t stride, bool side_stream = false, bool defer_join = false);
void discard_begun_walk(gg_ctx *ctx);
int walk_finalize(gg_ctx *ctx, bool *retried);
int timing_slot(gg_ctx *ctx);
int check_exchange_flag(gg_ctx *ctx);
void harvest_timings(gg_ctx *ctx);
int derive_tree_edges(gg_ctx *ctx);
int compute_reverse_edges(gg_ctx *ctx);
int rescan_table_finite(gg_ctx *ctx, int which);
int enqueue_path_slots(gg_ctx *ctx);
void generator_changed(gg_ctx *ctx);
int walk_resident(gg_ctx *ctx, const int32_t *slots, const int32_t *n_walks, int32_t uniform_walks, int32_t n_slots,
                  int32_t for_d, uint64_t seed, uint32_t stream, int32_t stride);
int launch_walk_sample(gg_ctx *ctx, int32_t n_slots, int64_t total_walks, int for_d, uint64_t seed, uint32_t stream,
                       int32_t stride);
int run_step(gg_ctx *ctx, int which, const int32_t *d_u, const int32_t *d_v, const float *d_x, int32_t n);
int comm_allreduce_grads(gg_ctx *ctx);
int comm_allreduce_flags(gg_ctx *ctx);
int comm_allreduce_i64(gg_ctx *ctx, int64_t *buf, size_t count);
int comm_allreduce_max_i64(gg_ctx *ctx, int64_t *buf, size_t count);
size_t comm_dense_bytes(const gg_ctx *ctx);
int exchange_count_max(gg_ctx *ctx, int64_t local, int64_t *max_out);
int comm_allgather(gg_ctx *ctx, const void *send, void *recv, size_t count, int elem_bytes);
bool comm_has_p2p(const gg_ctx *ctx);
int comm_exchange_v(gg_ctx *ctx, const float *send, const int64_t *send_off, const int64_t *send_cnt, float *recv, const int64_t *recv_off,
                    const int64_t *recv_cnt);
void comm_destroy(gg_ctx *ctx);

static inline int cdiv(int64_t a, int64_t b) { return (int)((a + b - 1) / b); }

}
```

graphgan_amd/csrc/prepare.hip:

```cpp
#include <algorithm>

#include <cstring>

#include "gg_internal.h"

namespace gg {

constexpr int SCAN_THREADS = 256;
constexpr int SCAN_ITEMS = 8;
constexpr int SCAN_TILE = SCAN_THREADS * SCAN_ITEMS;

__device__ __forceinline__ int64_t block_excl_scan(int64_t v, int64_t *total, int64_t *sh ) {
    const int lane = threadIdx.x & 63, wv = threadIdx.x >> 6;
    int64_t inc = v;
#pragma unroll
    for (int off = 1; off < 64; off <<= 1) {
        const int64_t o = __shfl_up(inc, off, 64);
        if (lane >= off) inc += o;
    }
    if (lane == 63) sh[wv] = inc;
    __syncthreads();
    int64_t base = 0, tot = 0;
#pragma unroll
    for (int i = 0; i < SCAN_THREADS / 64; ++i) {
// ... 271 lines not shown
    fetch(1, R[1], bv[1], have[1]);
    fetch(2, R[2], bv[2], have[2]);
    auto n_pairs_of = [&](int i) { return min(i, window) + min(L - 1 - i, window); };
    int base = 0;
    for (int c = 0; c < L; ++c) {
        float4 Rn[NCH];
        float nb;
        bool nh;
        fetch(c + 3, Rn, nb, nh);
        const int back_c = min(c, window);
        int base_d = base + n_pairs_of(c);
        float myval = 0.f;
        int myidx = -1;
#pragma unroll
        for (int d = 1; d <= 2; ++d) {
            if (d <= window && have[d]) {
                float acc = 0.f;
#pragma unroll
                for (int i = 0; i < NCH; ++i) {
                    acc = __builtin_fmaf(R[0][i].x, R[d][i].x, acc);
                    acc = __builtin_fmaf(R[0][i].y, R[d][i].y, acc);
                    acc = __builtin_fmaf(R[0][i].z, R[d][i].z, acc);
                    acc = __builtin_fmaf(R[0][i].w, R[d][i].w, acc);
                }
                acc += __shfl_xor(acc, 8, 64);
                acc += __shfl_xor(acc, 4, 64);
                acc += __shfl_xor(acc, 2, 64);
                acc += __shfl_xor(acc, 1, 64);
                if (t == 2 * d - 2) { myval = acc + bv[d]; myidx = base + back_c + (d - 1); }
                if (t == 2 * d - 1) { myval = acc + bv[0]; myidx = base_d + (c - max(c + d - window, 0)); }
            }
            base_d += n_pairs_of(c + d);
        }
        if (myidx >= 0) {
            const float sc = fminf(fmaxf(myval, -10.0f), 10.0f);
            out[pi0 + myidx] = logf(1.0f + expf(sc));
        }
        base += n_pairs_of(c);
#pragma unroll
        for (int i = 0; i < NCH; ++i) { R[0][i] = R[1][i]; R[1][i] = R[2][i]; R[2][i] = Rn[i]; }
        have[0] = have[1]; have[1] = have[2]; have[2] = nh;
        bv[0] = bv[1]; bv[1] = bv[2]; bv[2] = nb;
    }
}

__global__ __launch_bounds__(256) void edge_dot_f64_kernel(const float *E, int ld, const int32_t *u, const int32_t *v, int64_t n, double *out) {
    const int t = threadIdx.x & 15;
    const int64_t g0 = ((int64_t)blockIdx.x * blockDim.x + threadIdx.x) >> 4, ng = ((int64_t)gridDim.x * blockDim.x) >> 4;
    for (int64_t p = g0; p < n; p += ng) {
        const float *ra = E + (int64_t)u[p] * ld, *rb = E + (int64_t)v[p] * ld;
        double acc = 0.0;
        for (int k = t; k < ld; k += 16) acc = fma((double)ra[k], (double)rb[k], acc);
        acc += __shfl_xor(acc, 8, 64);
        acc += __shfl_xor(acc, 4, 64);
        acc += __shfl_xor(acc, 2, 64);
        acc += __shfl_xor(acc, 1, 64);
        if (t == 0) out[p] = acc;
    }
}

int launch_pair_reward(gg_ctx *ctx, const int32_t *d_u, const int32_t *d_v, int64_t n, float *d_out) {
    if (n == 0) return GG_OK;
    const Model &D = ctx->model[1];
    int64_t blocks = (n * 16 + 255) / 256;
    if (blocks > 256 * 16) blocks = 256 * 16;
    hipLaunchKernelGGL(pair_reward_kernel, dim3((unsigned)blocks), dim3(256), 0, ctx->stream, D.E, D.b, ctx->ld, d_u, d_v, n,
                       (const int64_t *)nullptr, d_out);
    GG_HIP(ctx, hipGetLastError());
    ctx->ctr.reward_pairs += n;
    return GG_OK;
}

__global__ void d_count_kernel(const int32_t *status, const int64_t *walk_ptr, int n_slots, int32_t *cnt, const unsigned long long *flag) {
    const int i = blockIdx.x * blockDim.x + threadIdx.x;
    if (i >= n_slots) return;
    if (*flag == 2ull) { cnt[i] = 0; return; }
    const int64_t deg = walk_ptr[i + 1] - walk_ptr[i];
    cnt[i] = (status[i] == GG_ROOT_OK && deg > 0) ? (int32_t)(2 * deg) : 0;
}

__global__ __launch_bounds__(256) void d_fill_kernel(const int32_t *slots, const int32_t *t_root, const int64_t *g_rowptr,
                                                     const int32_t *g_col, const int32_t *samples, const int64_t *walk_ptr,
                                                     const int64_t *row_ptr, int n_slots, int32_t *center, int32_t *neighbor,
                                                     float *label, const unsigned long long *flag) {
    const int lane = threadIdx.x & 63;
    const int i = (blockIdx.x * blockDim.x + threadIdx.x) >> 6;
    if (i >= n_slots || *flag == 2ull) return;
    const int64_t o = row_ptr[i], rows = row_ptr[i + 1] - o;
    if (rows == 0) return;
    const int64_t deg = rows / 2;
    const int root = t_root[slots[i]];
    const int64_t e0 = g_rowptr[root], w0 = walk_ptr[i];
    for (int64_t e = lane; e < deg; e += 64) {
        center[o + e] = root;
        neighbor[o + e] = g_col[e0 + e];
        label[o + e] = 1.0f;
        center[o + deg + e] = root;
        neighbor[o + deg + e] = samples[w0 + e];
        label[o + deg + e] = 0.0f;
    }
}

static inline int effective_window(const gg_ctx *ctx, int stride) { return std::min<int>(ctx->cfg.window_size, stride); }

static int fill_g_pairs(gg_ctx *ctx) {
    const int64_t nw = ctx->w_total;
    hipLaunchKernelGGL(pair_fill_kernel, dim3(cdiv(nw, 256)), dim3(256), 0, ctx->stream, ctx->w_paths.as<int32_t>(),
                       ctx->w_len.as<int32_t>(), ctx->w_stride, nw, effective_window(ctx, ctx->w_stride), ctx->g_ptr.as<int64_t>(),
                       ctx->g_node1.as<int32_t>(), ctx->g_node2.as<int32_t>(), ctx->dev_ctr + 3);
    GG_HIP(ctx, hipGetLastError());
    ctx->g_pairs_filled = true;
    return GG_OK;
}

int ensure_g_pairs(gg_ctx *ctx) {
    if (ctx->g_pairs_filled || ctx->g_pairs == 0) return GG_OK;
    GG_CHECK(ctx, ctx->g_paths_valid, GG_EINVAL,
             "the walks of the last gg_prepare_g were overwritten by a later walk launch before its pairs were read: fetch the pairs "
             "(gg_get_g_data) or run the minibatch passes before the next prepare call");
    return fill_g_pairs(ctx);
}

}

using namespace gg;

extern "C" {

static int enqueue_d_rows(gg_ctx *ctx, int32_t n_slots) {
    hipLaunchKernelGGL(d_count_kernel, dim3(cdiv(n_slots, 256)), dim3(256), 0, ctx->stream, ctx->w_status.as<int32_t>(),
                       ctx->w_ptr_buf().as<int64_t>(), n_slots, ctx->d_cnt.as<int32_t>(), ctx->dev_ctr + 3);
    int rc = device_exclusive_scan(ctx, ctx->d_cnt.as<int32_t>(), ctx->d_ptr.as<int64_t>(), n_slots);
    if (rc != GG_OK) return rc;
    hipLaunchKernelGGL(d_fill_kernel, dim3(cdiv((int64_t)n_slots * 64, 256)), dim3(256), 0, ctx->stream,
                       ctx->w_slots_buf().as<int32_t>(), ctx->t_root, ctx->g_rowptr, ctx->g_col, ctx->w_samples.as<int32_t>(),
                       ctx->w_ptr_buf().as<int64_t>(), ctx->d_ptr.as<int64_t>(), n_slots, ctx->d_center.as<int32_t>(),
                       ctx->d_neighbor.as<int32_t>(), ctx->d_label.as<float>(), ctx->dev_ctr + 3);
    GG_HIP(ctx, hipMemcpyAsync(ctx->h_pin + gg_ctx::H_TOTAL, ctx->d_ptr.as<int64_t>() + n_slots, sizeof(int64_t), hipMemcpyDeviceToHost, ctx->stream));
    GG_HIP(ctx, hipGetLastError());
    return GG_OK;
}

int gg_prepare_d(gg_ctx *ctx, const int32_t *slots, int32_t n_slots, uint64_t seed, uint32_t stream, int64_t *n_rows_out,
                 int32_t *root_status) {
    if (!ctx) return fail(nullptr, GG_EINVAL, "ctx is NULL");
    GG_CHECK(ctx, ctx->g_rowptr, GG_EINVAL, "gg_prepare_d: call gg_set_graph_csr first");
    const int stride = ctx->tree_max_depth + 3;
    ctx->d_rows = 0;
    ctx->dc_valid = false;
    discard_begun_walk(ctx);
    ctx->dc_request = ctx->dc_enabled ? 1 : 0;
    int rc = walk_launch_async(ctx, slots, nullptr, -1, n_slots, 1, seed, stream, stride);
    if (rc != GG_OK) { ctx->dc_request = 0; return rc; }
    if (n_slots > 0) {
        const int64_t cap = 2 * ctx->w_total;
        GG_HIP(ctx, ctx->d_cnt.reserve(sizeof(int32_t) * n_slots));
        GG_HIP(ctx, ctx->d_ptr.reserve(sizeof(int64_t) * (n_slots + 1)));
        GG_HIP(ctx, ctx->d_center.reserve(sizeof(int32_t) * (cap + 1)));
        GG_HIP(ctx, ctx->d_neighbor.reserve(sizeof(int32_t) * (cap + 1)));
        GG_HIP(ctx, ctx->d_label.reserve(sizeof(float) * (cap + 1)));
        rc = enqueue_d_rows(ctx, n_slots);
        if (rc != GG_OK) return rc;
    }
    bool retried = false;
    rc = walk_finalize(ctx, &retried);
    ctx->dc_request = 0;
    if (rc != GG_OK) return rc;
    if (n_slots > 0) {
        if (retried) {
            rc = enqueue_d_rows(ctx, n_slots);
            if (rc != GG_OK) return rc;
            GG_HIP(ctx, hipStreamSynchronize(ctx->stream));
        }
        ctx->d_rows = (int64_t)ctx->h_pin[gg_ctx::H_TOTAL];
        ctx->dc_valid = ctx->dc_enabled && ctx->walk_levels > 0;
        if (root_status) GG_HIP(ctx, hipMemcpy(root_status, ctx->w_status.p, sizeof(int32_t) * n_slots, hipMemcpyDeviceToHost));
    }
    if (!ctx->in_epoch_add) {
        rc = exchange_count_max(ctx, ctx->d_rows, &ctx->d_rows_max);
        if (rc != GG_OK) return rc;
    }
    if (n_rows_out) *n_rows_out = ctx->d_rows;
    return GG_OK;
}

int gg_get_d_data(gg_ctx *ctx, int32_t *center, int32_t *neighbor, float *label) {
    if (!ctx) return fail(nullptr, GG_EINVAL, "ctx is NULL");
    const int64_t n = ctx->d_rows;
    if (n == 0) return GG_OK;
    GG_HIP(ctx, hipSetDevice(ctx->device));
    GG_HIP(ctx, hipStreamSynchronize(ctx->stream));
    if (center) GG_HIP(ctx, hipMemcpy(center, ctx->d_center.p, sizeof(int32_t) * n, hipMemcpyDeviceToHost));
    if (neighbor) GG_HIP(ctx, hipMemcpy(neighbor, ctx->d_neighbor.p, sizeof(int32_t) * n, hipMemcpyDeviceToHost));
    if (label) GG_HIP(ctx, hipMemcpy(label, ctx->d_label.p, sizeof(float) * n, hipMemcpyDeviceToHost));
    return GG_OK;
}

static int enqueue_g_pairs(gg_ctx *ctx, int64_t nw, int64_t cap) {
    const int window = ctx->cfg.window_size;
    hipLaunchKernelGGL(pair_count_kernel, dim3(cdiv(nw, 256)), dim3(256), 0, ctx->stream, ctx->w_len.as<int32_t>(), nw,
                       effective_window(ctx, ctx->w_stride), ctx->g_cnt.as<int32_t>(), ctx->dev_ctr + 3);
    int rc = device_exclusive_scan(ctx, ctx->g_cnt.as<int32_t>(), ctx->g_ptr.as<int64_t>(), nw);
    if (rc != GG_OK) return rc;
    const int nch = (ctx->ld / 4 + 15) / 16;
    const bool path_reward = window <= 2 && nch <= 4 && ctx->ld % 4 == 0 && !getenv("GG_NO_PATH_REWARD");
    ctx->g_pairs_filled = false;
    if (!path_reward) {
        rc = fill_g_pairs(ctx);
        if (rc != GG_OK) return rc;
    }
    const Model &D = ctx->model[1];
    const int ts = ctx->walk_timed ? timing_slot(ctx) : -1;
    if (ts >= 0) GG_HIP(ctx, hipEventRecord(ctx->tm_ev[ts][0], ctx->stream));
    if (path_reward) {
        const dim3 grid(cdiv(nw * 16, 256)), blk(256);
#define GG_PATH_REWARD(N)                                                                                                              \
    hipLaunchKernelGGL(path_reward_kernel<N>, grid, blk, 0, ctx->stream, D.E, D.b, ctx->ld, ctx->w_paths.as<int32_t>(),                 \
                       ctx->w_len.as<int32_t>(), ctx->w_stride, nw, window, ctx->g_ptr.as<int64_t>(), ctx->g_reward.as<float>(), ctx->dev_ctr + 3)
        if (nch <= 1) GG_PATH_REWARD(1);
        else if (nch == 2) GG_PATH_REWARD(2);
        else GG_PATH_REWARD(4);
#undef GG_PATH_REWARD
    } else {
        hipLaunchKernelGGL(pair_reward_kernel, dim3(256 * 16), dim3(256), 0, ctx->stream, D.E, D.b, ctx->ld, ctx->g_node1.as<int32_t>(),
                           ctx->g_node2.as<int32_t>(), (int64_t)-1, ctx->g_ptr.as<int64_t>() + nw, ctx->g_reward.as<float>());
    }
    if (ts >= 0) {
        GG_HIP(ctx, hipEventRecord(ctx->tm_ev[ts][1], ctx->stream));
        GG_HIP(ctx, hipEventRecord(ctx->tm_ev[ts][2], ctx->stream));
        ctx->tm_pending.push_back({0, 0, ts, false});
    }
    GG_HIP(ctx, hipMemcpyAsync(ctx->h_pin + gg_ctx::H_TOTAL, ctx->g_ptr.as<int64_t>() + nw, sizeof(int64_t), hipMemcpyDeviceToHost, ctx->stream));
    GG_HIP(ctx, hipGetLastError());
    (void)cap;
    return GG_OK;
}

int gg_prepare_g_begin(gg_ctx *ctx, const int32_t *slots, int32_t n_slots, int32_t n_sample, uint64_t seed, uint32_t stream) {
    if (!ctx) return fail(nullptr, GG_EINVAL, "ctx is NULL");
    GG_CHECK(ctx, n_sample >= 0, GG_EINVAL, "gg_prepare_g_begin: n_sample < 0");
    const int stride = ctx->tree_max_depth + 3;
    discard_begun_walk(ctx);
    ctx->dc_request = ctx->dc_valid ? 2 : 0;
    int rc = walk_launch_async(ctx, slots, nullptr, n_sample, n_slots, 0, seed, stream, stride, true, true);
    if (rc != GG_OK) { ctx->dc_request = 0; return rc; }
    if (n_slots == 0) { ctx->dc_request = 0; return GG_OK; }
    ctx->g_begun = true;
    ctx->g_begun_args.n_slots = n_slots;
    ctx->g_begun_args.n_sample = n_sample;
    ctx->g_begun_args.seed = seed;
    ctx->g_begun_args.stream = stream;
    return GG_OK;
}

int gg_prepare_g(gg_ctx *ctx, const int32_t *slots, int32_t n_slots, int32_t n_sample, uint64_t seed, uint32_t stream,
                 int64_t *n_pairs_out, int32_t *root_status) {
    if (!ctx) return fail(nullptr, GG_EINVAL, "ctx is NULL");
// ... 119 lines not shown
```

graphgan_amd/csrc/pretrain.hip:

```cpp
#include <algorithm>
#include <vector>

#include "gg_arith.h"
#include "gg_internal.h"

namespace gg {

constexpr int PT_MAX_LEN = 256, PT_MAX_WINDOW = 16, PT_MAX_NEG = 64;
constexpr int PT_WAVES = 4;
constexpr int PT_SAMPLE = 2048;
constexpr int H_PT_TOTAL = gg_ctx::H_TOTAL + 8;

__host__ __device__ __forceinline__ int pt_pairs_of(int i, int len, int window) {
    const int back = i < window ? i : window, fwd = len - 1 - i < window ? len - 1 - i : window;
    return back + fwd;
}

static int64_t pt_pairs_of_path(int len, int window) {
    int64_t c = 0;
    for (int i = 0; i < len; ++i) c += pt_pairs_of(i, len, window);
    return c;
}

__global__ __launch_bounds__(256) void pt_walk_kernel(const int64_t *__restrict__ rowptr, const int32_t *__restrict__ col,
// ... 223 lines not shown
                        node = (int32_t)threshold(m, (uint64_t)n_node);
                    }
                    while (node == c || node == x) node = node + 1 == n_node ? 0 : node + 1;
                    nb = node;
                    lab = 0.0f;
                }
                center[o + r] = c;
                neighbor[o + r] = nb;
                label[o + r] = lab;
            }
        }
        __syncthreads();
    }
}

}

using namespace gg;

extern "C" {

int gg_pretrain_set_noise(gg_ctx *ctx, const uint32_t *weight) {
    if (!ctx) return fail(nullptr, GG_EINVAL, "ctx is NULL");
    GG_HIP(ctx, hipSetDevice(ctx->device));
    GG_HIP(ctx, hipStreamSynchronize(ctx->stream));
    if (!weight) {
        ctx->pt_noise_set = false;
        return GG_OK;
    }
    const int64_t n = ctx->n_node;
    std::vector<uint64_t> cum((size_t)n);
    uint64_t run = 0;
    for (int64_t j = 0; j < n; ++j) cum[j] = (run += weight[j]);
    GG_CHECK(ctx, run >= 1, GG_EINVAL, "gg_pretrain_set_noise: every weight is zero");
    const int64_t stride = (n + PT_SAMPLE - 1) / PT_SAMPLE, ns = (n + stride - 1) / stride;
    std::vector<uint64_t> sample((size_t)ns);
    for (int64_t k = 0; k < ns; ++k) sample[k] = cum[std::min<int64_t>((k + 1) * stride, n) - 1];
    ctx->pt_noise_set = false;
    GG_HIP(ctx, ctx->pt_noise.reserve(sizeof(uint64_t) * (size_t)n));
    GG_HIP(ctx, ctx->pt_sample.reserve(sizeof(uint64_t) * PT_SAMPLE));
    GG_HIP(ctx, hipMemcpy(ctx->pt_noise.p, cum.data(), sizeof(uint64_t) * (size_t)n, hipMemcpyHostToDevice));
    GG_HIP(ctx, hipMemcpy(ctx->pt_sample.p, sample.data(), sizeof(uint64_t) * (size_t)ns, hipMemcpyHostToDevice));
    ctx->pt_noise_total = run;
    ctx->pt_sample_n = (int32_t)ns;
    ctx->pt_sample_stride = (int32_t)stride;
    ctx->pt_noise_set = true;
    return GG_OK;
}

int gg_pretrain_set_walk_bias(gg_ctx *ctx, uint32_t w_ret, uint32_t w_com, uint32_t w_out) {
    if (!ctx) return fail(nullptr, GG_EINVAL, "ctx is NULL");
    for (uint32_t v : {w_ret, w_com, w_out})
        GG_CHECK(ctx, v >= 1 && v <= 65536, GG_EINVAL, "gg_pretrain_set_walk_bias: weights must be in [1, 65536], got (%u, %u, %u)", w_ret, w_com, w_out);
    ctx->pt_bias[0] = w_ret;
    ctx->pt_bias[1] = w_com;
    ctx->pt_bias[2] = w_out;
    return GG_OK;
}

int gg_prepare_pretrain(gg_ctx *ctx, const int32_t *starts, int32_t n_starts, int32_t walks_per_start, int32_t walk_len,
                        int32_t window, int32_t n_neg, uint64_t seed, uint32_t stream, int64_t *n_rows_out, int32_t *paths,
                        int32_t *path_len) {
    if (!ctx) return fail(nullptr, GG_EINVAL, "ctx is NULL");
    GG_CHECK(ctx, ctx->g_rowptr, GG_EINVAL, "gg_prepare_pretrain: call gg_set_graph_csr first");
    GG_CHECK(ctx, !ctx->comm, GG_EINVAL, "gg_prepare_pretrain: a communicator is attached (pre-training is single rank)");
    GG_CHECK(ctx, !ctx->ep_d_open, GG_EINVAL, "gg_prepare_pretrain: called between gg_epoch_begin and gg_epoch_commit(1)");
    GG_CHECK(ctx, n_starts >= 0 && (starts || n_starts == 0), GG_EINVAL, "gg_prepare_pretrain: bad starts");
    GG_CHECK(ctx, walks_per_start >= 1, GG_EINVAL, "gg_prepare_pretrain: walks_per_start must be >= 1");
    GG_CHECK(ctx, walk_len >= 1 && walk_len <= PT_MAX_LEN, GG_EINVAL, "gg_prepare_pretrain: walk_len must be in [1, %d]", PT_MAX_LEN);
    GG_CHECK(ctx, window >= 1 && window <= PT_MAX_WINDOW, GG_EINVAL, "gg_prepare_pretrain: window must be in [1, %d]", PT_MAX_WINDOW);
    GG_CHECK(ctx, n_neg >= 0 && n_neg <= PT_MAX_NEG, GG_EINVAL, "gg_prepare_pretrain: n_neg must be in [0, %d]", PT_MAX_NEG);
    GG_CHECK(ctx, ctx->n_node >= 3, GG_EINVAL, "gg_prepare_pretrain: the collision rule of the negatives needs n_node >= 3");
    for (int32_t i = 0; i < n_starts; ++i)
        GG_CHECK(ctx, starts[i] >= 0 && starts[i] < ctx->n_node, GG_EINVAL, "gg_prepare_pretrain: starts[%d] = %d out of range", i, starts[i]);
    const int64_t nw = (int64_t)n_starts * walks_per_start;
    GG_CHECK(ctx, nw <= 0x7fffffffll, GG_ECAPACITY, "gg_prepare_pretrain: %lld walks in one call", (long long)nw);
    GG_HIP(ctx, hipSetDevice(ctx->device));
    const uint32_t *wb = ctx->pt_bias;
    const bool biased = !(wb[0] == wb[1] && wb[1] == wb[2]);
    if (biased && nw > 0) {
        const int rc = ensure_sorted_adjacency(ctx);
        if (rc != GG_OK) return rc;
    }
    ctx->d_rows = 0;
    if (nw > 0) {
        const int64_t rows_bound = nw * (1 + n_neg) * pt_pairs_of_path(walk_len, window);
        const bool sized = rows_bound <= 0x7fffffffll;
        GG_HIP(ctx, ctx->pt_starts.reserve(sizeof(int32_t) * (size_t)n_starts));
        GG_HIP(ctx, ctx->pt_paths.reserve(sizeof(int32_t) * (size_t)nw * walk_len));
        GG_HIP(ctx, ctx->pt_len.reserve(sizeof(int32_t) * (size_t)nw));
        GG_HIP(ctx, ctx->pt_cnt.reserve(sizeof(int32_t) * (size_t)nw));
        GG_HIP(ctx, ctx->pt_ptr.reserve(sizeof(int64_t) * (size_t)(nw + 1)));
        const bool timed = ctx->profile_every == 1;
        if (timed && !ctx->pt_ev[0])
            for (hipEvent_t &e : ctx->pt_ev) GG_HIP(ctx, hipEventCreate(&e));
        GG_HIP(ctx, hipMemcpyAsync(ctx->pt_starts.p, starts, sizeof(int32_t) * (size_t)n_starts, hipMemcpyHostToDevice, ctx->stream));
        if (timed) GG_HIP(ctx, hipEventRecord(ctx->pt_ev[0], ctx->stream));
        if (biased)
            hipLaunchKernelGGL(pt_walk_bias_kernel, dim3(cdiv(nw, 256)), dim3(256), 0, ctx->stream, ctx->g_rowptr, ctx->g_col,
                               ctx->topk_adj.as<int32_t>(), ctx->pt_starts.as<int32_t>(), nw, walks_per_start, walk_len, seed, stream,
                               PtBias{wb[0], wb[1], wb[2], std::max(wb[0], std::max(wb[1], wb[2]))}, ctx->pt_paths.as<int32_t>(),
                               ctx->pt_len.as<int32_t>());
        else
            hipLaunchKernelGGL(pt_walk_kernel, dim3(cdiv(nw, 256)), dim3(256), 0, ctx->stream, ctx->g_rowptr, ctx->g_col,
                               ctx->pt_starts.as<int32_t>(), nw, walks_per_start, walk_len, seed, stream, ctx->pt_paths.as<int32_t>(),
                               ctx->pt_len.as<int32_t>());
        if (timed) GG_HIP(ctx, hipEventRecord(ctx->pt_ev[1], ctx->stream));
        hipLaunchKernelGGL(pt_count_kernel, dim3(cdiv(nw, 256)), dim3(256), 0, ctx->stream, ctx->pt_len.as<int32_t>(), nw, window, n_neg,
                           ctx->pt_cnt.as<int32_t>());
        GG_HIP(ctx, hipGetLastError());
        int rc = device_exclusive_scan(ctx, ctx->pt_cnt.as<int32_t>(), ctx->pt_ptr.as<int64_t>(), nw);
        if (rc != GG_OK) return rc;
        GG_HIP(ctx, hipMemcpyAsync(ctx->h_pin + H_PT_TOTAL, ctx->pt_ptr.as<int64_t>() + nw, sizeof(int64_t), hipMemcpyDeviceToHost, ctx->stream));
        int64_t cap = rows_bound;
        if (!sized) {
            GG_HIP(ctx, hipStreamSynchronize(ctx->stream));
            cap = (int64_t)ctx->h_pin[H_PT_TOTAL];
            GG_CHECK(ctx, cap <= 0x7fffffffll, GG_ECAPACITY, "gg_prepare_pretrain: %lld rows in one call (at most 2^31 - 1): pass fewer starts",
                     (long long)cap);
        }
        GG_HIP(ctx, ctx->d_center.reserve(sizeof(int32_t) * (size_t)(cap + 1)));
        GG_HIP(ctx, ctx->d_neighbor.reserve(sizeof(int32_t) * (size_t)(cap + 1)));
        GG_HIP(ctx, ctx->d_label.reserve(sizeof(float) * (size_t)(cap + 1)));
        const bool noise = ctx->pt_noise_set;
        const int64_t blocks = std::min<int64_t>((nw + PT_WAVES - 1) / PT_WAVES, (int64_t)ctx->n_cus * 12);
        if (timed) GG_HIP(ctx, hipEventRecord(ctx->pt_ev[2], ctx->stream));
        hipLaunchKernelGGL(pt_fill_kernel, dim3((unsigned)blocks), dim3(64 * PT_WAVES), 0, ctx->stream, ctx->pt_paths.as<int32_t>(),
                           ctx->pt_len.as<int32_t>(), ctx->pt_starts.as<int32_t>(), ctx->pt_ptr.as<int64_t>(), nw, walks_per_start, walk_len,
                           window, n_neg, seed, stream, ctx->n_node, noise ? ctx->pt_noise.as<uint64_t>() : (const uint64_t *)nullptr,
                           noise ? ctx->pt_noise_total : 0ull, ctx->pt_sample.as<uint64_t>(), noise ? ctx->pt_sample_n : 0,
                           noise ? ctx->pt_sample_stride : 1, ctx->d_center.as<int32_t>(), ctx->d_neighbor.as<int32_t>(),
                           ctx->d_label.as<float>());
        if (timed) GG_HIP(ctx, hipEventRecord(ctx->pt_ev[3], ctx->stream));
        GG_HIP(ctx, hipGetLastError());
        GG_HIP(ctx, hipStreamSynchronize(ctx->stream));
        harvest_timings(ctx);
        ctx->d_rows = (int64_t)ctx->h_pin[H_PT_TOTAL];
        if (timed) {
            float walk_ms = 0.f, fill_ms = 0.f;
            GG_HIP(ctx, hipEventElapsedTime(&walk_ms, ctx->pt_ev[0], ctx->pt_ev[1]));
            GG_HIP(ctx, hipEventElapsedTime(&fill_ms, ctx->pt_ev[2], ctx->pt_ev[3]));
            ctx->ctr.walk_kernel_ms += walk_ms;
            ctx->ctr.walk_launches += 1;
            ctx->ctr.last_kernel_ms = fill_ms;
        }
        if (paths) GG_HIP(ctx, hipMemcpy(paths, ctx->pt_paths.p, sizeof(int32_t) * (size_t)nw * walk_len, hipMemcpyDeviceToHost));
        if (path_len) GG_HIP(ctx, hipMemcpy(path_len, ctx->pt_len.p, sizeof(int32_t) * (size_t)nw, hipMemcpyDeviceToHost));
    } else {
        GG_HIP(ctx, hipStreamSynchronize(ctx->stream));
    }
    ctx->d_rows_max = ctx->d_rows;
    if (n_rows_out) *n_rows_out = ctx->d_rows;
    return GG_OK;
}

}
```

graphgan_amd/csrc/steps.hip:

```cpp
#include <stdlib.h>

#include <algorithm>
#include <cmath>
#include <vector>

#include "gg_internal.h"

namespace gg {

struct HubAcc {
    unsigned long long *acc;
    int64_t cap;
    float scale;
};
__device__ __forceinline__ unsigned long long *hub_row(const HubAcc &h, int slot, int ld) {
    const int64_t k = -3 - (int64_t)slot;
    return (slot <= -3 && k < h.cap) ? h.acc + k * (ld + 1) : nullptr;
}
__device__ __forceinline__ void hub_add(unsigned long long *p, float x, float scale) {
    atomicAdd(p, (unsigned long long)__float2ll_rn(x * scale));
}

struct StepArgs {
    float *E, *b;
    float *gE, *gb;
    int32_t *touched, *touched_list, *touched_cnt;
    int ld, track;
    const int32_t *u, *v;
    const float *x;
    int n;
    float lambda, inv_n;
    const int64_t *n_glob;
    int is_d;
    int ppg;
    const int32_t *slot_v, *slot_u;
    float *stage, *stage_b;
    HubAcc hub;
};

__global__ __launch_bounds__(256) void pair_occ_count_kernel(const int32_t *u, const int32_t *v, int n, int ppg, int32_t *cnt,
                                                             int32_t *slot_v, int32_t *slot_u) {
    const int p = blockIdx.x * blockDim.x + threadIdx.x;
    if (p >= n) return;
    slot_v[p] = atomicAdd(&cnt[v[p]], 1);
    const bool run_end = p == n - 1 || (p + 1) % ppg == 0 || u[p + 1] != u[p];
    slot_u[p] = run_end ? atomicAdd(&cnt[u[p]], 1) : -2;
}

__global__ __launch_bounds__(256) void pair_occ_slot_kernel(const int32_t *u, const int32_t *v, int n, const int32_t *cnt, const int32_t *off,
                                                            int T, int32_t *slot_v, int32_t *slot_u, int32_t *key) {
    const int p = blockIdx.x * blockDim.x + threadIdx.x;
    if (p >= n) return;
    const int iv = v[p], iu = u[p];
    const int sv = cnt[iv] <= T ? off[iv] + slot_v[p] : -3 - off[iv];
    slot_v[p] = sv;
    if (sv >= 0) key[sv] = 2 * p + 1;
    if (slot_u[p] != -2) {
        const int su = cnt[iu] <= T ? off[iu] + slot_u[p] : -3 - off[iu];
        slot_u[p] = su;
        if (su >= 0) key[su] = 2 * p;
    }
}

constexpr int PAIRS_PER_GROUP = 16;

template <int NF, bool STAGED>
__global__ __launch_bounds__(256) void pair_grad_kernel(const StepArgs a) {
    const int t = threadIdx.x & 15;
    const int g = (blockIdx.x * blockDim.x + threadIdx.x) >> 4;
    const int p0 = g * a.ppg;
    if (p0 >= a.n) return;
    const int p1 = min(p0 + a.ppg, a.n);
    const int nchunk = a.ld >> 2;
    const float inv_n = a.n_glob ? 1.0f / (float)(*a.n_glob) : a.inv_n;
    float accu[NF];
#pragma unroll
    for (int i = 0; i < NF; ++i) accu[i] = 0.f;
    int run_u = a.u[p0];
    auto flush_u = [&](int q) {
        const int sl = STAGED ? a.slot_u[q] : -1;
        if (STAGED && sl >= 0) {
            float *g = a.stage + (int64_t)sl * a.ld;
#pragma unroll
            for (int i = 0; i < NF; ++i) {
                const int f = t + 16 * i;
                if (f < a.ld) g[f] = accu[i];
            }
            if (t == 0) a.stage_b[sl] = 0.f;
            return;
        }
        float *gu = a.gE + (int64_t)run_u * a.ld;
#pragma unroll
        for (int i = 0; i < NF; ++i) {
            const int f = t + 16 * i;
            if (f < a.ld) atomicAdd(gu + f, accu[i]);
        }
        if (t == 0 && a.track) a.touched[run_u] = 1;
    };
    for (int p = p0; p < p1; ++p) {
        const int iu = a.u[p], iv = a.v[p];
        if (iu != run_u) {
            flush_u(p - 1);
#pragma unroll
            for (int i = 0; i < NF; ++i) accu[i] = 0.f;
            run_u = iu;
        }
        const float4 *ru = (const float4 *)(a.E + (int64_t)iu * a.ld);
        const float4 *rv = (const float4 *)(a.E + (int64_t)iv * a.ld);
        float acc = 0.f;
        for (int c = t; c < nchunk; c += 16) {
            const float4 x = ru[c], y = rv[c];
            acc = __builtin_fmaf(x.x, y.x, acc);
            acc = __builtin_fmaf(x.y, y.y, acc);
            acc = __builtin_fmaf(x.z, y.z, acc);
            acc = __builtin_fmaf(x.w, y.w, acc);
        }
        acc += __shfl_xor(acc, 8, 64);
        acc += __shfl_xor(acc, 4, 64);
        acc += __shfl_xor(acc, 2, 64);
        acc += __shfl_xor(acc, 1, 64);
        const float bv = a.b[iv];
        const float s = acc + bv;
        const float sg = 1.0f / (1.0f + expf(-s));
        float ds;
        if (a.is_d) {
            ds = sg - a.x[p];
        } else {
            const bool inside = (sg >= 1e-5f) && (sg <= 1.0f);
            ds = inside ? -(a.x[p] * inv_n) * (1.0f - sg) : 0.0f;
        }
        const float *fu = (const float *)ru, *fv = (const float *)rv;
        const int slv = STAGED ? a.slot_v[p] : -1;
        const bool st = STAGED && slv >= 0;
        float *gv = st ? a.stage + (int64_t)slv * a.ld : a.gE + (int64_t)iv * a.ld;
#pragma unroll
        for (int i = 0; i < NF; ++i) {
            const int f = t + 16 * i;
            if (f < a.ld) {
                const float x = fu[f], y = fv[f];
                accu[i] += ds * y + a.lambda * x;
                const float gval = ds * x + a.lambda * y;
                if (st) gv[f] = gval;
                else atomicAdd(gv + f, gval);
            }
        }
        if (t == 0) {
            const float gbv = a.is_d ? ds + a.lambda * bv : ds;
            if (st) {
                a.stage_b[slv] = gbv;
            } else {
                atomicAdd(a.gb + iv, gbv);
                if (a.track) a.touched[iv] = 1;
            }
        }
    }
    flush_u(p1 - 1);
}

template <int NF, bool STAGED>
__global__ __launch_bounds__(256) void pair_grad16_kernel(const StepArgs a) {
    const int t = threadIdx.x & 15;
    const int64_t g = ((int64_t)blockIdx.x * blockDim.x + threadIdx.x) >> 4;
    const int64_t p0 = g * 16;
    if (p0 >= a.n) return;
    const int np = (int)min((int64_t)16, (int64_t)a.n - p0);
    const float inv_n = a.n_glob ? 1.0f / (float)(*a.n_glob) : a.inv_n;
    const bool mine = t < np;
    const int myu = mine ? a.u[p0 + t] : 0, myv = mine ? a.v[p0 + t] : 0;
    const float myx = mine ? a.x[p0 + t] : 0.f;
    const int my_sv = (STAGED && mine) ? a.slot_v[p0 + t] : -1;
    const int my_su = (STAGED && mine) ? a.slot_u[p0 + t] : -1;
    const float mybv = a.b[myv];
    const int nextu = __shfl(myu, (t + 1) & 15, 16);
    const bool my_end = mine && (t == np - 1 || nextu != myu);
    auto fetch = [&](int j, float (&ru)[NF], float (&rv)[NF]) {
        const int jj = j < np ? j : 0;
        const float *su = a.E + (int64_t)__shfl(myu, jj, 16) * a.ld, *sv = a.E + (int64_t)__shfl(myv, jj, 16) * a.ld;
#pragma unroll
        for (int i = 0; i < NF; ++i) {
            const int f = t + 16 * i;
            const int fc = f < a.ld ? f : a.ld - 1;
            ru[i] = su[fc];
            rv[i] = sv[fc];
        }
    };
    float U[3][NF], V[3][NF], accu[NF];
#pragma unroll
    for (int i = 0; i < NF; ++i) accu[i] = 0.f;
    fetch(0, U[0], V[0]);
    fetch(1, U[1], V[1]);
#pragma unroll 1
    for (int j0 = 0; j0 < np; j0 += 3) {
#pragma unroll
        for (int r = 0; r < 3; ++r) {
            const int j = j0 + r;
            if (j >= np) break;
            fetch(j + 2, U[(r + 2) % 3], V[(r + 2) % 3]);
            float acc = 0.f;
#pragma unroll
            for (int i = 0; i < NF; ++i) {
                const bool in = t + 16 * i < a.ld;
                const float x = in ? U[r][i] : 0.f, y = in ? V[r][i] : 0.f;
                U[r][i] = x; V[r][i] = y;
                acc = __builtin_fmaf(x, y, acc);
            }
            acc += __shfl_xor(acc, 8, 64);
            acc += __shfl_xor(acc, 4, 64);
            acc += __shfl_xor(acc, 2, 64);
            acc += __shfl_xor(acc, 1, 64);
            const float bv = __shfl(mybv, j, 16), xj = __shfl(myx, j, 16);
            const float s = acc + bv;
            const float sg = 1.0f / (1.0f + expf(-s));
            float ds;
            if (a.is_d) {
                ds = sg - xj;
            } else {
                const bool inside = (sg >= 1e-5f) && (sg <= 1.0f);
                ds = inside ? -(xj * inv_n) * (1.0f - sg) : 0.0f;
            }
            const int iv = __shfl(myv, j, 16), iu = __shfl(myu, j, 16);
            const int slv = __shfl(my_sv, j, 16), slu = __shfl(my_su, j, 16);
            const bool st = STAGED && slv >= 0;
            unsigned long long *hv = STAGED && !st ? hub_row(a.hub, slv, a.ld) : nullptr;
            float *gv = st ? a.stage + (int64_t)slv * a.ld : a.gE + (int64_t)iv * a.ld;
#pragma unroll
            for (int i = 0; i < NF; ++i) {
                const int f = t + 16 * i;
                if (f < a.ld) {
                    accu[i] += ds * V[r][i] + a.lambda * U[r][i];
                    const float gval = ds * U[r][i] + a.lambda * V[r][i];
                    if (st) gv[f] = gval;
                    else if (STAGED && hv) hub_add(hv + f, gval, a.hub.scale);
                    else atomicAdd(gv + f, gval);
                }
            }
            if (t == 0) {
                const float gbv = a.is_d ? ds + a.lambda * bv : ds;
                if (st) {
                    a.stage_b[slv] = gbv;
                } else {
                    if (STAGED && hv) hub_add(hv + a.ld, gbv, a.hub.scale);
                    else atomicAdd(a.gb + iv, gbv);
                    if (a.track) a.touched[iv] = 1;
                }
            }
            if (__shfl((int)my_end, j, 16)) {
                if (STAGED && slu >= 0) {
// ... 885 lines not shown
    o.sg_cnt = ix.cnt.as<int32_t>(); o.sg_list = ix.list.as<int4>(); o.sg_tot = ix.tot.as<int64_t>(); o.stage_key = ix.key.as<int32_t>();
}

__global__ void set_count_kernel(int64_t *dst, int64_t v) { *dst = v; }

static int global_pair_count(gg_ctx *ctx, int64_t n_local, const int64_t **out) {
    *out = nullptr;
    const int world = ctx->comm ? ctx->world : ctx->fake_world;
    if (world <= 1) return GG_OK;
    GG_HIP(ctx, ctx->x_nglob.reserve(sizeof(int64_t) * 2));
    int64_t *w = ctx->x_nglob.as<int64_t>();
    hipLaunchKernelGGL(set_count_kernel, dim3(1), dim3(1), 0, ctx->stream, w, ctx->comm ? n_local : n_local * world);
    if (ctx->comm) {
        int rc = comm_allreduce_i64(ctx, w, 1);
        if (rc != GG_OK) return rc;
    }
    *out = w;
    return GG_OK;
}

static int64_t stage_bytes_cap() {
    static const int64_t cap = [] {
        const char *e = getenv("GG_STAGE_MAX_BYTES");
        return e ? (int64_t)atoll(e) : (int64_t)24 << 30;
    }();
    return cap;
}

__global__ __launch_bounds__(256) void hub_index_kernel(const int32_t *cnt, int64_t n, int T, int32_t *off, int32_t *rows, int64_t *nhub) {
    const int64_t i = (int64_t)blockIdx.x * blockDim.x + threadIdx.x;
    if (i >= n || cnt[i] <= T) return;
    const int h = (int)atomicAdd((unsigned long long *)nhub, 1ull);
    off[i] = h;
    rows[h] = (int32_t)i;
}

__global__ __launch_bounds__(256) void hub_finalize_kernel(unsigned long long *acc, const int32_t *rows, const int64_t *nhub, int64_t cap, int ld,
                                                           double inv_scale, float *gE, float *gb) {
    const int64_t n = min(*nhub, cap) * (ld + 1);
    for (int64_t i = (int64_t)blockIdx.x * blockDim.x + threadIdx.x; i < n; i += (int64_t)gridDim.x * blockDim.x) {
        const unsigned long long v = acc[i];
        if (!v) continue;
        acc[i] = 0ull;
        const int64_t h = i / (ld + 1);
        const int f = (int)(i - h * (ld + 1));
        const float x = (float)((double)(long long)v * inv_scale);
        if (f < ld) gE[(int64_t)rows[h] * ld + f] += x;
        else gb[rows[h]] += x;
    }
}

static float hub_scale(bool per_pair_mean, int64_t n) {
    return std::ldexp(1.0f, 32 + (per_pair_mean && n > 1 ? (int)std::ilogb((double)n) : 0));
}

static HubAcc hub_args(gg_ctx *ctx, float scale) {
    return HubAcc{ctx->hub_acc.as<unsigned long long>(), ctx->hub_cap, scale};
}

int StageIndex::reserve(gg_ctx *ctx, int64_t n_node, int64_t n_occ, int64_t n_key, hipStream_t stream) {
    const size_t cnt_before = cnt.bytes;
    GG_HIP(ctx, cnt.reserve(sizeof(int32_t) * (size_t)n_node));
    if (cnt.bytes != cnt_before || !counts_zero) GG_HIP(ctx, hipMemsetAsync(cnt.p, 0, cnt.bytes, stream));
    counts_zero = false;
    for (DevBuf *b : {&off, &hub}) GG_HIP(ctx, b->reserve(sizeof(int32_t) * (size_t)n_node));
    GG_HIP(ctx, list.reserve(sizeof(int4) * (size_t)n_node));
    GG_HIP(ctx, slot.reserve(sizeof(int32_t) * (size_t)n_occ));
    GG_HIP(ctx, key.reserve(sizeof(int32_t) * (size_t)n_key));
    GG_HIP(ctx, tot.reserve(sizeof(int64_t) * 4));
    return GG_OK;
}

static int index_rows(gg_ctx *ctx, StageIndex &ix, hipStream_t stream) {
    int32_t *cnt = ix.cnt.as<int32_t>(), *off = ix.off.as<int32_t>();
    int64_t *tot = ix.tot.as<int64_t>();
    const int rc = device_segment_rows(ctx, cnt, ctx->n_node, ctx->sg_threshold, off, ix.list.as<int4>(), tot, stream, stream == ctx->stream ? nullptr : &ix.scan);
    if (rc != GG_OK) return rc;
    GG_HIP(ctx, hipMemsetAsync(tot + 2, 0, sizeof(int64_t), stream));
    hipLaunchKernelGGL(hub_index_kernel, dim3((unsigned)cdiv(ctx->n_node, 256)), dim3(256), 0, stream, cnt, (int64_t)ctx->n_node, ctx->sg_threshold, off,
                       ix.hub.as<int32_t>(), tot + 2);
    return GG_OK;
}

static int build_from_pairs(gg_ctx *ctx, StageIndex &ix, const int32_t *u, const int32_t *v, int32_t n, int ppg, hipStream_t stream) {
    int32_t *cnt = ix.cnt.as<int32_t>(), *slot_v = ix.slots(), *slot_u = slot_v + n;
    hipLaunchKernelGGL(pair_occ_count_kernel, dim3(cdiv(n, 256)), dim3(256), 0, stream, u, v, n, ppg, cnt, slot_v, slot_u);
    const int rc = index_rows(ctx, ix, stream);
    if (rc != GG_OK) return rc;
    hipLaunchKernelGGL(pair_occ_slot_kernel, dim3(cdiv(n, 256)), dim3(256), 0, stream, u, v, n, cnt, ix.off.as<int32_t>(), ctx->sg_threshold, slot_v, slot_u,
                       ix.key.as<int32_t>());
    GG_HIP(ctx, hipGetLastError());
    return GG_OK;
}

static int build_from_paths(gg_ctx *ctx, StageIndex &ix, const int32_t *paths, const int32_t *len, int32_t stride, int64_t n_walks, const unsigned long long *flag, hipStream_t stream) {
    const dim3 grid((unsigned)cdiv(n_walks * (int64_t)stride, 256));
    int32_t *cnt = ix.cnt.as<int32_t>();
    hipLaunchKernelGGL(path_count_kernel, grid, dim3(256), 0, stream, paths, len, stride, n_walks, cnt, ix.slots(), flag);
    const int rc = index_rows(ctx, ix, stream);
    if (rc != GG_OK) return rc;
    hipLaunchKernelGGL(path_slot_kernel, grid, dim3(256), 0, stream, paths, len, stride, n_walks, cnt, ix.off.as<int32_t>(), ctx->sg_threshold, ix.slots(),
                       ix.key.as<int32_t>(), flag);
    GG_HIP(ctx, hipGetLastError());
    return GG_OK;
}

static void hub_finalize(gg_ctx *ctx, const StageIndex &ix, float scale) {
    const int64_t n = ctx->hub_cap * (ctx->ld + 1);
    const unsigned nb = (unsigned)std::max<int64_t>(1, std::min<int64_t>(cdiv(n, 256), 2048));
    hipLaunchKernelGGL(hub_finalize_kernel, dim3(nb), dim3(256), 0, ctx->stream, ctx->hub_acc.as<unsigned long long>(), ix.hub.as<int32_t>(),
                       ix.tot.as<int64_t>() + 2, ctx->hub_cap, ctx->ld, 1.0 / (double)scale, ctx->gradE, ctx->gradb);
}

static int staged_reserve(gg_ctx *ctx, int64_t n_occ, int64_t n_stage) {
    if (n_stage * (int64_t)(ctx->ld + 2) * 4 > stage_bytes_cap()) return 1;
    const bool was_dirty = !ctx->sg_own.counts_zero;
    const int rc = ctx->sg_own.reserve(ctx, ctx->n_node, n_occ, n_stage, ctx->stream);
    if (rc != GG_OK) return rc;
    GG_HIP(ctx, ctx->sg_bias.reserve(sizeof(float) * (size_t)n_stage));
    {
        const int64_t cap = std::min<int64_t>(ctx->n_node, n_occ / ((int64_t)ctx->sg_threshold + 1) + 1);
        const size_t before = ctx->hub_acc.bytes;
        if (ctx->hub_acc.reserve(sizeof(unsigned long long) * (size_t)cap * (ctx->ld + 1)) != hipSuccess) {
            (void)hipGetLastError();
            ctx->hub_cap = 0;
            return 1;
        }
        if (ctx->hub_acc.bytes != before || was_dirty) GG_HIP(ctx, hipMemsetAsync(ctx->hub_acc.p, 0, ctx->hub_acc.bytes, ctx->stream));
        ctx->hub_cap = (int64_t)(ctx->hub_acc.bytes / (sizeof(unsigned long long) * (ctx->ld + 1)));
    }
    if (ctx->sg_rows.reserve(sizeof(float) * (size_t)n_stage * ctx->ld) != hipSuccess) {
        (void)hipGetLastError();
        return 1;
    }
    return GG_OK;
}

template <int MODE>
static void launch_staged_opt(gg_ctx *ctx, const OptArgs &o, int64_t max_rows) {
    const dim3 g((unsigned)std::max<int64_t>(1, (max_rows * 16 + 255) / 256)), b(256);
    if (ctx->ld <= 64) hipLaunchKernelGGL((staged_opt_kernel<MODE, 1>), g, b, 0, ctx->stream, o);
    else if (ctx->ld <= 128) hipLaunchKernelGGL((staged_opt_kernel<MODE, 2>), g, b, 0, ctx->stream, o);
    else hipLaunchKernelGGL((staged_opt_kernel<MODE, 4>), g, b, 0, ctx->stream, o);
}

static int staged_finish(gg_ctx *ctx, int which, int64_t n, int64_t n_occ, StageIndex &ix, float scale) {
    hub_finalize(ctx, ix, scale);
    if (ctx->tm_cur >= 0) GG_HIP(ctx, hipEventRecord(ctx->tm_ev[ctx->tm_cur][1], ctx->stream));
    OptArgs o = make_opt_args(ctx, which);
    set_index_args(o, ix);
    o.stage = ctx->sg_rows.as<float>(); o.stage_b = ctx->sg_bias.as<float>();
    const int64_t max_rows = std::min<int64_t>(n_occ, ctx->n_node);
    const bool replicas = ctx->comm || ctx->fake_world > 1;
    if (replicas) launch_staged_opt<2>(ctx, o, max_rows);
    else if (ctx->cfg.optimizer == GG_OPT_SGD) launch_staged_opt<1>(ctx, o, max_rows);
    else launch_staged_opt<0>(ctx, o, max_rows);
    ctx->sg_applying = &ix;
    const int rc = apply_optimizer(ctx, which, n);
    ctx->sg_applying = nullptr;
    if (rc != GG_OK) return rc;
    if (!replicas)
        hipLaunchKernelGGL(add_word_kernel, dim3(1), dim3(1), 0, ctx->stream, ctx->touched_ptr.as<int64_t>() + ctx->n_node, o.sg_tot);
    GG_HIP(ctx, hipGetLastError());
    ix.counts_zero = true;
    return GG_OK;
}

static bool staged_allowed(const gg_ctx *ctx) {
    return ctx->sg_threshold > 0 && ctx->ld <= 256 && ctx->cfg.optimizer != GG_OPT_ADAM_DENSE && !getenv("GG_NO_STAGED_GRAD");
}

template <bool STAGED>
static void launch_pair_grad(gg_ctx *ctx, const StepArgs &s, int blocks, int nf) {
    const dim3 g(blocks), b(256);
    if (STAGED || (s.ppg == PAIRS_PER_GROUP && nf <= 16 && !getenv("GG_OLD_PAIR_GRAD"))) {
        if (nf <= 4) hipLaunchKernelGGL((pair_grad16_kernel<4, STAGED>), g, b, 0, ctx->stream, s);
        else if (nf <= 8) hipLaunchKernelGGL((pair_grad16_kernel<8, STAGED>), g, b, 0, ctx->stream, s);
        else hipLaunchKernelGGL((pair_grad16_kernel<16, STAGED>), g, b, 0, ctx->stream, s);
    } else if constexpr (!STAGED) {
        if (nf <= 4) hipLaunchKernelGGL((pair_grad_kernel<4, false>), g, b, 0, ctx->stream, s);
        else if (nf <= 8) hipLaunchKernelGGL((pair_grad_kernel<8, false>), g, b, 0, ctx->stream, s);
        else if (nf <= 16) hipLaunchKernelGGL((pair_grad_kernel<16, false>), g, b, 0, ctx->stream, s);
        else hipLaunchKernelGGL((pair_grad_kernel<32, false>), g, b, 0, ctx->stream, s);
    }
}

int run_step(gg_ctx *ctx, int which, const int32_t *d_u, const int32_t *d_v, const float *d_x, int32_t n) {
    if (n <= 0) return GG_OK;
    Model &M = ctx->model[which];
    const int opt = ctx->cfg.optimizer;
    StepArgs s{};
    s.E = M.E; s.b = M.b; s.gE = ctx->gradE; s.gb = ctx->gradb;
    s.touched = ctx->touched; s.touched_list = ctx->touched_list; s.touched_cnt = ctx->touched_cnt;
    s.ld = ctx->ld;
    s.track = opt != GG_OPT_ADAM_DENSE;
    s.u = d_u; s.v = d_v; s.x = d_x; s.n = n;
    s.lambda = M.lambda;
    s.inv_n = 1.0f / (float)n;
    s.is_d = which == 1;
    if (which == 0) {
        int rc = global_pair_count(ctx, n, &s.n_glob);
        if (rc != GG_OK) return rc;
    }
    s.ppg = n >= 16384 ? PAIRS_PER_GROUP : (n >= 2048 ? 4 : 1);
    if (ctx->deterministic && n <= DET_MAX_PAIRS) {
        const int nfd = (ctx->ld + 15) / 16;
        const bool replicas = ctx->comm || ctx->fake_world > 1;
        const int fused = (!replicas && opt != GG_OPT_ADAM_DENSE && det_rows_fit_lds(ctx, s) && !getenv("GG_NO_FUSED_SMALL_STEP")) ? (opt == GG_OPT_SGD ? 2 : 1) : 0;
        const OptArgs o = make_opt_args(ctx, which);
        hipError_t e;
        if (nfd <= 4) e = launch_pair_grad_det<4>(ctx, s, o, fused);
        else if (nfd <= 8) e = launch_pair_grad_det<8>(ctx, s, o, fused);
        else if (nfd <= 16) e = launch_pair_grad_det<16>(ctx, s, o, fused);
        else e = launch_pair_grad_det<32>(ctx, s, o, fused);
        GG_HIP(ctx, e);
        if (fused) {
            GG_HIP(ctx, hipGetLastError());
            step_done(ctx, which, n);
            return GG_OK;
        }
        return apply_optimizer(ctx, which, n);
    }
    const int groups = cdiv(n, s.ppg);
    const int blocks = cdiv((int64_t)groups * 16, 256);
    const int nf = (ctx->ld + 15) / 16;
    const int fit = n >= 16384 && n < (1 << 30) && staged_allowed(ctx) ? staged_reserve(ctx, 2 * (int64_t)n, 2 * (int64_t)n) : 1;
    if (fit < 0) return fit;
    if (fit == GG_OK) {
        StageIndex &ix = ctx->sg_own;
        const int rc = build_from_pairs(ctx, ix, d_u, d_v, n, s.ppg, ctx->stream);
        if (rc != GG_OK) return rc;
        s.slot_v = ix.slots(); s.slot_u = s.slot_v + n;
        s.stage = ctx->sg_rows.as<float>(); s.stage_b = ctx->sg_bias.as<float>();
        const float scale = hub_scale(!s.is_d, n);
        s.hub = hub_args(ctx, scale);
        launch_pair_grad<true>(ctx, s, blocks, nf);
        return staged_finish(ctx, which, n, 2 * (int64_t)n, ix, scale);
    }
    launch_pair_grad<false>(ctx, s, blocks, nf);
    if (ctx->tm_cur >= 0) GG_HIP(ctx, hipEventRecord(ctx->tm_ev[ctx->tm_cur][1], ctx->stream));
    return apply_optimizer(ctx, which, n);
}

template <bool STAGED>
static void launch_path_grad(gg_ctx *ctx, const PathArgs &p, int blocks, int nf) {
    const dim3 g(blocks), b(256);
    if (p.stride <= 17) {
        if (nf <= 4) hipLaunchKernelGGL((path_grad_kernel<4, STAGED, true>), g, b, 0, ctx->stream, p);
        else if (nf <= 8) hipLaunchKernelGGL((path_grad_kernel<8, STAGED, true>), g, b, 0, ctx->stream, p);
        else hipLaunchKernelGGL((path_grad_kernel<16, STAGED, true>), g, b, 0, ctx->stream, p);
    } else {
        if (nf <= 4) hipLaunchKernelGGL((path_grad_kernel<4, STAGED, false>), g, b, 0, ctx->stream, p);
        else if (nf <= 8) hipLaunchKernelGGL((path_grad_kernel<8, STAGED, false>), g, b, 0, ctx->stream, p);
        else hipLaunchKernelGGL((path_grad_kernel<16, STAGED, false>), g, b, 0, ctx->stream, p);
    }
}

int run_path_step(gg_ctx *ctx) {
    Model &M = ctx->model[0];
    const int64_t n = ctx->g_pairs;
    PathArgs p{};
    p.E = M.E; p.b = M.b; p.gE = ctx->gradE; p.gb = ctx->gradb;
    p.touched = ctx->touched; p.touched_list = ctx->touched_list; p.touched_cnt = ctx->touched_cnt;
    p.ld = ctx->ld;
    p.track = ctx->cfg.optimizer != GG_OPT_ADAM_DENSE;
    p.window = ctx->cfg.window_size;
    p.paths = ctx->w_paths.as<int32_t>();
    p.path_len = ctx->w_len.as<int32_t>();
    p.stride = ctx->w_stride;
    p.pair_ptr = ctx->g_ptr.as<int64_t>();
    p.reward = ctx->g_reward.as<float>();
    p.n_walks = ctx->w_total;
    p.lambda = M.lambda;
    p.inv_n = 1.0f / (float)n;
    {
        int rc = global_pair_count(ctx, n, &p.n_glob);
        if (rc != GG_OK) return rc;
    }
    const int blocks = cdiv(p.n_walks * 16, 256);
    const int nf = (ctx->ld + 15) / 16;
    const int64_t n_pos = p.n_walks * (int64_t)p.stride;
    const int64_t n_stage = std::min<int64_t>(n_pos, p.window >= 2 ? (n + 6 * p.n_walks) / 4 + 1 : (n + 2 * p.n_walks) / 2 + 1);
    const int fit = staged_allowed(ctx) && n_pos < (1ll << 31) ? staged_reserve(ctx, n_pos, n_stage) : 1;
    if (fit < 0) return fit;
    if (fit != GG_OK) {
        launch_path_grad<false>(ctx, p, blocks, nf);
        if (ctx->tm_cur >= 0) GG_HIP(ctx, hipEventRecord(ctx->tm_ev[ctx->tm_cur][1], ctx->stream));
        return apply_optimizer(ctx, 0, n);
    }
    const bool early = ctx->g_slots_ready && ctx->g_slots_walks == p.n_walks && ctx->g_slots_stride == p.stride;
    ctx->g_slots_ready = false;
    ctx->g_slots_unused = 0;
    StageIndex &ix = early ? ctx->sg_early : ctx->sg_own;
    if (early) {
        ctx->sg_own.counts_zero = true;
        GG_HIP(ctx, hipStreamWaitEvent(ctx->stream, ctx->ev_slots_done, 0));
    } else {
        const int rc = build_from_paths(ctx, ix, p.paths, p.path_len, p.stride, p.n_walks, nullptr, ctx->stream);
        if (rc != GG_OK) return rc;
    }
    p.slot = ix.slots();
    p.stage = ctx->sg_rows.as<float>();
    p.stage_b = ctx->sg_bias.as<float>();
    const float scale = hub_scale(true, n);
    p.hub = hub_args(ctx, scale);
    launch_path_grad<true>(ctx, p, blocks, nf);
    return staged_finish(ctx, 0, n, n_pos, ix, scale);
}

int enqueue_path_slots(gg_ctx *ctx) {
    ctx->g_slots_ready = false;
    if (ctx->walk_stream == ctx->stream || ctx->in_epoch_add || getenv("GG_NO_EARLY_SLOTS")) return GG_OK;
    const int64_t n_walks = ctx->w_total, n_pos = n_walks * (int64_t)ctx->w_stride;
    if (!staged_allowed(ctx) || ctx->cfg.window_size > 2 || n_walks == 0 || n_pos >= (1ll << 31)) return GG_OK;
// ... 324 lines not shown
    }
    if (rc != GG_OK) return rc;

    OptArgs o = make_opt_args(ctx, which);
    if (ctx->sg_applying) o.sg_cnt = ctx->sg_applying->cnt.as<int32_t>();
    if (opt == GG_OPT_ADAM_DENSE) {
        int64_t nb = (o.nE / 4 + 255) / 256;
        if (nb > 2048) nb = 2048;
        if (nb < 1) nb = 1;
        hipLaunchKernelGGL(adam_dense_kernel, dim3((unsigned)nb), dim3(256), 0, ctx->stream, o);
    } else {
        GG_HIP(ctx, ctx->touched_ptr.reserve(sizeof(int64_t) * ((size_t)ctx->n_node + 1)));
        o.touched_ptr = ctx->touched_ptr.as<int64_t>();
        o.touched_total = o.touched_ptr + ctx->n_node;
        const int world = ctx->comm ? ctx->world : ctx->fake_world;
        if (world > 1 || (ctx->comm && ctx->world == 1)) {
            rc = exchange_sparse(ctx, o, world < 1 ? 1 : world, ctx->step_bound > 0 ? ctx->step_bound : n);
            if (rc != GG_OK) return rc;
        }
        rc = device_compact_flags(ctx, ctx->touched, ctx->n_node, ctx->touched_list, ctx->touched_ptr.as<int64_t>() + ctx->n_node);
        if (rc != GG_OK) return rc;
        int nb = cdiv((int64_t)std::min<int64_t>(2ll * n * ctx->world, ctx->n_node) * 16, 256);
        if (nb > 4096) nb = 4096;
        if (nb < 1) nb = 1;
        if (opt == GG_OPT_SGD) hipLaunchKernelGGL(sparse_opt_kernel<1>, dim3(nb), dim3(256), 0, ctx->stream, o);
        else hipLaunchKernelGGL(sparse_opt_kernel<0>, dim3(nb), dim3(256), 0, ctx->stream, o);
    }
    GG_HIP(ctx, hipGetLastError());
    step_done(ctx, which, n);
    return GG_OK;
}

void step_done(gg_ctx *ctx, int which, int64_t n) {
    Model &M = ctx->model[which];
    if (which == 0) { ctx->gen_dirty = true; generator_changed(ctx); }
    M.t += 1;
    M.b1p = M.b1p * ctx->cfg.adam_beta1;
    M.b2p = M.b2p * ctx->cfg.adam_beta2;
    if (which == 1) { ctx->ctr.d_pairs += n; ctx->ctr.d_steps += 1; }
    else { ctx->ctr.g_pairs += n; ctx->ctr.g_steps += 1; }
}

}

using namespace gg;

static int host_step(gg_ctx *ctx, int which, const int32_t *u, const int32_t *v, const float *x, int32_t n) {
    if (!ctx) return fail(nullptr, GG_EINVAL, "ctx is NULL");
    if (which == 0) discard_begun_walk(ctx);
    GG_CHECK(ctx, n >= 0 && (n == 0 || (u && v && x)), GG_EINVAL, "step: bad argument");
    if (n == 0) return GG_OK;
    for (int i = 0; i < n; ++i)
        GG_CHECK(ctx, u[i] >= 0 && u[i] < ctx->n_node && v[i] >= 0 && v[i] < ctx->n_node, GG_EINVAL, "step: id out of range at %d", i);
    GG_HIP(ctx, hipSetDevice(ctx->device));
    GG_HIP(ctx, ctx->step_u.reserve(sizeof(int32_t) * n));
    GG_HIP(ctx, ctx->step_v.reserve(sizeof(int32_t) * n));
    GG_HIP(ctx, ctx->step_x.reserve(sizeof(float) * n));
    GG_HIP(ctx, hipMemcpyAsync(ctx->step_u.p, u, sizeof(int32_t) * n, hipMemcpyHostToDevice, ctx->stream));
    GG_HIP(ctx, hipMemcpyAsync(ctx->step_v.p, v, sizeof(int32_t) * n, hipMemcpyHostToDevice, ctx->stream));
    GG_HIP(ctx, hipMemcpyAsync(ctx->step_x.p, x, sizeof(float) * n, hipMemcpyHostToDevice, ctx->stream));
    ctx->step_bound = n;
    if (ctx->comm && ctx->world > 1 && ctx->cfg.optimizer != GG_OPT_ADAM_DENSE) {
        GG_HIP(ctx, ctx->x_nglob.reserve(sizeof(int64_t) * 4));
        int64_t *w = ctx->x_nglob.as<int64_t>() + 3;
        const int64_t mine = n;
        GG_HIP(ctx, hipMemcpyAsync(w, &mine, sizeof(int64_t), hipMemcpyHostToDevice, ctx->stream));
        int rc0 = comm_allreduce_max_i64(ctx, w, 1);
        if (rc0 != GG_OK) return rc0;
        int64_t mx = n;
        GG_HIP(ctx, hipMemcpyAsync(&mx, w, sizeof(int64_t), hipMemcpyDeviceToHost, ctx->stream));
        GG_HIP(ctx, hipStreamSynchronize(ctx->stream));
        ctx->step_bound = mx;
    }
    int rc = run_step(ctx, which, ctx->step_u.as<int32_t>(), ctx->step_v.as<int32_t>(), ctx->step_x.as<float>(), n);
    if (rc != GG_OK) return rc;
    GG_HIP(ctx, hipStreamSynchronize(ctx->stream));
    return GG_OK;
}

static int run_pass(gg_ctx *ctx, int which, const int64_t *starts, int64_t n_batches, int32_t batch_size) {
    if (!ctx) return fail(nullptr, GG_EINVAL, "ctx is NULL");
    if (which == 0) discard_begun_walk(ctx);
    GG_CHECK(ctx, batch_size > 0 && n_batches >= 0 && (starts || n_batches == 0), GG_EINVAL, "pass: bad argument");
    const int64_t rows = which == 1 ? ctx->d_rows : ctx->g_pairs;
    const int32_t *u = which == 1 ? ctx->d_center.as<int32_t>() : ctx->g_node1.as<int32_t>();
    const int32_t *v = which == 1 ? ctx->d_neighbor.as<int32_t>() : ctx->g_node2.as<int32_t>();
    const float *x = which == 1 ? ctx->d_label.as<float>() : ctx->g_reward.as<float>();
    GG_HIP(ctx, hipSetDevice(ctx->device));
    const int64_t rows_max = std::max(rows, which == 1 ? ctx->d_rows_max : ctx->g_pairs_max);
    auto empty_step = [&]() -> int {
        if (!ctx->comm) return GG_OK;
        if (which == 0) {
            const int64_t *unused = nullptr;
            int rc = global_pair_count(ctx, 0, &unused);
            if (rc != GG_OK) return rc;
        }
        return apply_optimizer(ctx, which, 0);
    };
    if (rows == 0) {
        ctx->step_bound = std::min<int64_t>(batch_size, rows_max);
        for (int64_t k = 0; k < n_batches; ++k) {
            int rc = empty_step();
            if (rc != GG_OK) return rc;
        }
        if (ctx->comm && n_batches > 0) GG_HIP(ctx, hipStreamSynchronize(ctx->stream));
        return GG_OK;
    }
    const bool timed = ctx->profile_every == 1;
    if (timed) GG_HIP(ctx, hipEventRecord(ctx->ev0, ctx->stream));
    const bool whole = n_batches == 1 && starts[0] == 0 && batch_size >= rows && rows > 0;
    ctx->tm_cur = -1;
    if (whole && ctx->profile_every > 0 && (ctx->pass_call_index[which]++ % ctx->profile_every) == 0 && !(ctx->deterministic && rows <= DET_MAX_PAIRS)) {
        ctx->tm_cur = timing_slot(ctx);
        if (ctx->tm_cur >= 0) GG_HIP(ctx, hipEventRecord(ctx->tm_ev[ctx->tm_cur][0], ctx->stream));
    }
    ctx->step_bound = std::min<int64_t>(batch_size, rows_max);
    if (which == 0 && whole && ctx->g_paths_valid && ctx->cfg.window_size <= 2 && ctx->ld <= 256 && !getenv("GG_NO_PATH_GRAD")) {
        int rc = run_path_step(ctx);
        if (rc != GG_OK) { ctx->tm_cur = -1; return rc; }
    } else {
        if (which == 0) {
            int rc = ensure_g_pairs(ctx);
            if (rc != GG_OK) { ctx->tm_cur = -1; return rc; }
        }
        for (int64_t k = 0; k < n_batches; ++k) {
            const int64_t s = starts[k];
            if (s < 0) {
                int rc = empty_step();
                if (rc != GG_OK) return rc;
                continue;
            }
            GG_CHECK(ctx, s < rows, GG_EINVAL, "pass: start %lld outside the %lld prepared rows", (long long)s, (long long)rows);
            const int32_t n = (int32_t)std::min<int64_t>(batch_size, rows - s);
            int rc = run_step(ctx, which, u + s, v + s, x + s, n);
            if (rc != GG_OK) return rc;
        }
    }
    if (ctx->tm_cur >= 0) {
        const int ts = ctx->tm_cur;
        ctx->tm_cur = -1;
        GG_HIP(ctx, hipEventRecord(ctx->tm_ev[ts][2], ctx->stream));
        const bool has_rows = ctx->cfg.optimizer != GG_OPT_ADAM_DENSE;
        if (has_rows)
            GG_HIP(ctx, hipMemcpyAsync(ctx->h_pin + gg_ctx::H_ROWS + ts, ctx->touched_ptr.as<int64_t>() + ctx->n_node, sizeof(int64_t),
                                       hipMemcpyDeviceToHost, ctx->stream));
        ctx->tm_pending.push_back({which == 1 ? 1 : 2, rows, ts, has_rows});
    }
    if (which == 0) {
        GG_HIP(ctx, hipEventRecord(ctx->ev_gen_pass, ctx->stream));
        ctx->gen_pass_recorded = true;
        ctx->gen_dirty = false;
    }
    if (timed) {
        GG_HIP(ctx, hipEventRecord(ctx->ev1, ctx->stream));
        GG_HIP(ctx, hipStreamSynchronize(ctx->stream));
        harvest_timings(ctx);
        float ms = 0.f;
        GG_HIP(ctx, hipEventElapsedTime(&ms, ctx->ev0, ctx->ev1));
        ctx->ctr.last_kernel_ms = ms;
    }
    return GG_OK;
}

extern "C" {

int gg_d_step(gg_ctx *ctx, const int32_t *u, const int32_t *v, const float *label, int32_t n) { return host_step(ctx, 1, u, v, label, n); }
int gg_g_step(gg_ctx *ctx, const int32_t *u, const int32_t *v, const float *reward, int32_t n) { return host_step(ctx, 0, u, v, reward, n); }
int gg_d_pass(gg_ctx *ctx, const int64_t *starts, int64_t n_batches, int32_t batch_size) { return run_pass(ctx, 1, starts, n_batches, batch_size); }
int gg_g_pass(gg_ctx *ctx, const int64_t *starts, int64_t n_batches, int32_t batch_size) { return run_pass(ctx, 0, starts, n_batches, batch_size); }

}
```

graphgan_amd/engine.py:

```python
from __future__ import annotations

import ctypes

import numpy as np

from . import _lib
from ._lib import GGConfig, GGCounters, check, lib
from .evaluation.embedding_spectrum import pca_cov, pca_eig
from .evaluation import link_heuristics as _lheur
from .evaluation import label_propagation as _lprop
from .evaluation import graph_communities as _gcomm
from .evaluation import graph_ranking as _grank
from .evaluation import graph_ppr as _gppr


def _ptr(a):
    return None if a is None else a.ctypes.data_as(ctypes.c_void_p)


def _i32(a):
    return np.ascontiguousarray(a, dtype=np.int32)


EDGE_OPERATORS = ("hadamard", "average", "l1", "l2")
# ... 108 lines not shown
    def __getitem__(self, v):
        return self.col[self.rowptr[v]:self.rowptr[v + 1]].tolist()

    def get(self, v, default=None):
        return self[v] if 0 <= v < len(self) else default

    def keys(self):
        return range(len(self))

    def __iter__(self):
        return iter(range(len(self)))

    def __contains__(self, v):
        return 0 <= v < len(self)


def host_write_embeddings(path, emb, n_threads=0):
    emb = np.ascontiguousarray(emb, dtype=np.float32)
    check(lib.gg_host_write_embeddings(_ptr(emb), emb.shape[0], emb.shape[1], str(path).encode(), n_threads))


def synth_powerlaw(n_node, m, seed_graph=1, seed_perm=2):
    n = check(lib.gg_synth_powerlaw(n_node, m, seed_graph, seed_perm, None, 0))
    edges = np.empty((int(n), 2), dtype=np.int32)
    check(lib.gg_synth_powerlaw(n_node, m, seed_graph, seed_perm, _ptr(edges), int(n)))
    return edges


class Engine:

    def __init__(self, emb_gen, emb_dis, lr_gen=1e-3, lr_dis=1e-3, lambda_gen=1e-5, lambda_dis=1e-5, window_size=2,
                 optimizer=_lib.GG_OPT_ADAM_DENSE, device=0, adam_beta1=0.9, adam_beta2=0.999, adam_eps=1e-8):
        eg = np.ascontiguousarray(emb_gen, dtype=np.float32)
        ed = np.ascontiguousarray(emb_dis, dtype=np.float32)
        assert eg.shape == ed.shape and eg.ndim == 2
        self.n_node, self.n_emb = int(eg.shape[0]), int(eg.shape[1])
        cfg = GGConfig(lr_gen, lr_dis, lambda_gen, lambda_dis, adam_beta1, adam_beta2, adam_eps, window_size, optimizer, device)
        self._ctx = ctypes.c_void_p()
        check(lib.gg_create(self.n_node, self.n_emb, _ptr(eg), _ptr(ed), ctypes.byref(cfg), ctypes.byref(self._ctx)))
        self.tree_roots = np.zeros(0, dtype=np.int32)
        self.max_depth = 0
        self._rowptr = None
        self._col = None
        self._set_adj = None
        self.tree_mode = (-1, 0)
        self.last_graph_softmax_ms = 0.0

    def close(self):
        if getattr(self, "_ctx", None) is not None and self._ctx.value:
            lib.gg_destroy(self._ctx)
            self._ctx = ctypes.c_void_p()

    def __del__(self):
        try:
            self.close()
        except Exception:
            pass

    def _ck(self, rc):
        return check(rc, self._ctx)

    def set_graph_csr(self, rowptr, col):
        rowptr = np.ascontiguousarray(rowptr, dtype=np.int64)
        col = _i32(col)
        self._ck(lib.gg_set_graph_csr(self._ctx, _ptr(rowptr), _ptr(col)))
        self._rowptr = rowptr
        self._col = col
        self._set_adj = None

    def build_trees(self, roots, n_threads=0, device=False):
        roots = _i32(roots)
        if device:
            self._ck(lib.gg_build_trees_device(self._ctx, _ptr(roots), len(roots)))
        else:
            self._ck(lib.gg_build_trees(self._ctx, _ptr(roots), len(roots), n_threads))
        self._after_trees(roots)

    def tree_bytes_estimate(self, n_roots):
        return float(n_roots) * 12.0 * (self.n_node + 1)

    def set_tree_mode(self, mode, node_cap=0):
        self._ck(lib.gg_set_tree_mode(self._ctx, int(mode), int(node_cap)))
        self.tree_mode = (int(mode), int(node_cap))

    def lazy_stats(self):
        out = np.zeros(24, dtype=np.int64)
        self._ck(lib.gg_lazy_stats(self._ctx, _ptr(out)))
        return dict(lazy=bool(out[0]), min_level=int(out[1]), fallback_roots=int(out[2]), fallback_rounds=int(out[3]), exact_nodes=int(out[4]),
                    pool_entries=int(out[5]), lazy_slots=int(out[6]), max_level=int(out[7]), resolved=[int(x) for x in out[8:11]],
                    candidates=int(out[11]), scan_rounds=int(out[12]), max_rounds=int(out[13]), max_degree_resolved=int(out[14]), coop_lists=int(out[15]),
                    slots_by_level=[int(x) for x in out[16:24]])

    def get_lazy_trees(self):
        R = len(self.tree_roots)
        n = ctypes.c_int64()
        self._ck(lib.gg_get_lazy_trees(self._ctx, ctypes.byref(n), None, None, None, None, None, None))
        n = n.value
        info, base = np.zeros((R, 4), np.int32), np.zeros(R, np.int64)
        order, cstart, edge, pair = np.zeros(n, np.int32), np.zeros(n + R, np.int32), np.zeros(n, np.int32), np.zeros(n, np.uint64)
        self._ck(lib.gg_get_lazy_trees(self._ctx, None, _ptr(info), _ptr(base), _ptr(order), _ptr(cstart), _ptr(edge), _ptr(pair)))
        return dict(info=info, base=base, order=order, cstart=cstart, edge=edge, pair=pair)

    def set_trees(self, roots, off, nbr, nbr_base, max_depth=0):
        roots, off, nbr = _i32(roots), _i32(off), _i32(nbr)
        nbr_base = np.ascontiguousarray(nbr_base, dtype=np.int64)
        self._ck(lib.gg_set_trees(self._ctx, _ptr(roots), len(roots), _ptr(off), _ptr(nbr), _ptr(nbr_base), max_depth))
        self._after_trees(roots)

    def _after_trees(self, roots):
        self.tree_roots = roots.copy()
        nr, ne, md = ctypes.c_int32(), ctypes.c_int64(), ctypes.c_int32()
        self._ck(lib.gg_tree_info(self._ctx, ctypes.byref(nr), ctypes.byref(ne), ctypes.byref(md)))
        self.tree_entries, self.max_depth = ne.value, md.value

    def save_trees(self, path):
        self._ck(lib.gg_save_trees(self._ctx, str(path).encode()))

    def load_trees(self, path):
        self._ck(lib.gg_load_trees(self._ctx, str(path).encode()))
        nr = ctypes.c_int32()
        self._ck(lib.gg_tree_info(self._ctx, ctypes.byref(nr), None, None))
        roots = np.zeros(nr.value, dtype=np.int32)
        self._ck(lib.gg_tree_roots(self._ctx, _ptr(roots)))
        self._after_trees(roots)

    def get_trees(self):
        R = len(self.tree_roots)
        off = np.zeros((R, self.n_node + 1), dtype=np.int32)
        nbr = np.zeros(max(self.tree_entries, 1), dtype=np.int32)
        base = np.zeros(R + 1, dtype=np.int64)
        self._ck(lib.gg_get_trees(self._ctx, _ptr(off), _ptr(nbr), _ptr(base)))
        return off, nbr[: self.tree_entries], base

    def get_tree_order(self):
        R = len(self.tree_roots)
        base = np.zeros(R + 1, dtype=np.int64)
        self._ck(lib.gg_get_tree_order(self._ctx, _ptr(base), None, None, None, None))
        nodes = int(base[R])
        order, cstart, edge = np.zeros(nodes, np.int32), np.zeros(nodes + R, np.int32), np.zeros(nodes, np.int32)
        valid = ctypes.c_int32()
        self._ck(lib.gg_get_tree_order(self._ctx, _ptr(base), _ptr(order), _ptr(cstart), _ptr(edge), ctypes.byref(valid)))
        return base, order, cstart, edge, bool(valid.value)

    def walk_sample(self, slots, n_walks, for_d, seed, stream, stride=None, fetch=True):
        slots, n_walks = _i32(slots), _i32(n_walks)
        stride = int(stride or (self.max_depth + 3))
        total = int(n_walks.sum())
        if not fetch:
            self._ck(lib.gg_walk_sample(self._ctx, _ptr(slots), _ptr(n_walks), len(slots), int(bool(for_d)), seed, stream,
                                        None, None, None, stride, None))
            return None
        samples = np.full(total, -1, dtype=np.int32)
        paths = np.full((total, stride), -1, dtype=np.int32)
        plen = np.zeros(total, dtype=np.int32)
        status = np.zeros(len(slots), dtype=np.int32)
        self._ck(lib.gg_walk_sample(self._ctx, _ptr(slots), _ptr(n_walks), len(slots), int(bool(for_d)), seed, stream,
                                    _ptr(samples), _ptr(paths), _ptr(plen), stride, _ptr(status)))
        self._after_trees(self.tree_roots)
        return dict(samples=samples, paths=paths, path_len=plen, root_status=status)

    def get_walks(self):
        tot, stride, ns = ctypes.c_int64(), ctypes.c_int32(), ctypes.c_int32()
        self._ck(lib.gg_walk_info(self._ctx, ctypes.byref(tot), ctypes.byref(stride), ctypes.byref(ns)))
        total, stride, ns = tot.value, stride.value, ns.value
        samples = np.full(total, -1, dtype=np.int32)
        paths = np.full((total, max(stride, 1)), -1, dtype=np.int32)
# ... 940 lines not shown
```

include/graphgan_hip.h:

```cpp
#ifndef GRAPHGAN_HIP_H
#define GRAPHGAN_HIP_H

#include <stdint.h>

#ifdef __cplusplus
extern "C" {
#endif

#define GG_ABI_VERSION 9

enum {
    GG_OK = 0,
    GG_EINVAL = -1,
    GG_ECAPACITY = -2,
    GG_EHIP = -3,
    GG_ECOMM = -4,
    GG_ENOMEM = -5,
    GG_EIO = -6
};

enum {
    GG_OPT_ADAM_DENSE = 0,
    GG_OPT_ADAM_LAZY = 1,
    GG_OPT_SGD = 2
// ... 13 lines not shown
    float adam_beta1;
    float adam_beta2;
    float adam_eps;
    int32_t window_size;
    int32_t optimizer;
    int32_t device;
    int32_t reserved[6];
} gg_config;

typedef struct gg_counters {
    int64_t walks;
    int64_t hops;
    int64_t nbr_reads;
    int64_t reward_pairs;
    int64_t d_pairs;
    int64_t g_pairs;
    int64_t d_steps;
    int64_t g_steps;
    double last_kernel_ms;
    double walk_kernel_ms;
    int64_t walk_launches;
    int64_t rows_scored;
    double score_kernel_ms;
    int64_t score_launches;
    int64_t score_chunks;
    int64_t score_rows;
    double bfs_kernel_ms;
    int64_t bfs_trees;
    int64_t score_dists;
    double reward_kernel_ms;
    int64_t reward_pairs_timed;
    double d_grad_ms, d_opt_ms;
    int64_t d_pairs_timed, d_rows_timed;
    double g_grad_ms, g_opt_ms;
    int64_t g_pairs_timed, g_rows_timed;
    int64_t d_passes_timed, g_passes_timed;
    int64_t g_walk_nodes_timed;
    int64_t es_gathers;
    int64_t es_nodes;
    int64_t score_gathers;
    int64_t score_nodes;
    int64_t walk_reruns;
} gg_counters;

typedef struct gg_ctx gg_ctx;

int gg_abi_version(void);
const char *gg_last_error(const gg_ctx *ctx);

int gg_create(int32_t n_node, int32_t n_emb, const float *emb_gen, const float *emb_dis,
              const gg_config *cfg, gg_ctx **out);
int gg_destroy(gg_ctx *ctx);

int gg_set_graph_csr(gg_ctx *ctx, const int64_t *rowptr , const int32_t *col);

int64_t gg_host_build_trees(int32_t n_node, const int64_t *rowptr, const int32_t *col,
                            const int32_t *roots, int32_t n_roots,
                            int32_t *off , int32_t *nbr, int64_t *nbr_base ,
                            int64_t cap, int32_t n_threads, int32_t *max_depth_out);

int gg_build_trees(gg_ctx *ctx, const int32_t *roots, int32_t n_roots, int32_t n_threads);
int gg_build_trees_device(gg_ctx *ctx, const int32_t *roots, int32_t n_roots);
int gg_set_tree_mode(gg_ctx *ctx, int32_t mode, int64_t node_cap);
int gg_debug_words(gg_ctx *ctx, int32_t first, int32_t n, uint64_t *out);
int gg_lazy_stats(gg_ctx *ctx, int64_t *out24);
int gg_get_lazy_trees(gg_ctx *ctx, int64_t *n_entries, int32_t *info4, int64_t *base, int32_t *order, int32_t *cstart, int32_t *edge, uint64_t *pair);
int gg_set_trees(gg_ctx *ctx, const int32_t *roots, int32_t n_roots, const int32_t *off,
                 const int32_t *nbr, const int64_t *nbr_base, int32_t max_depth);
int gg_tree_info(const gg_ctx *ctx, int32_t *n_roots, int64_t *n_entries, int32_t *max_depth);
int gg_tree_roots(const gg_ctx *ctx, int32_t *roots );
int gg_save_trees(gg_ctx *ctx, const char *path);
int gg_load_trees(gg_ctx *ctx, const char *path);
int gg_get_trees(gg_ctx *ctx, int32_t *off, int32_t *nbr, int64_t *nbr_base);
int gg_get_tree_order(gg_ctx *ctx, int64_t *base, int32_t *order, int32_t *cstart, int32_t *edge, int32_t *edges_valid);

int gg_walk_sample(gg_ctx *ctx, const int32_t *slots, const int32_t *n_walks, int32_t n_slots,
                   int32_t for_d, uint64_t seed, uint32_t stream,
                   int32_t *samples, int32_t *paths, int32_t *path_len, int32_t stride,
                   int32_t *root_status);

int gg_walk_info(const gg_ctx *ctx, int64_t *total_walks, int32_t *stride, int32_t *n_slots);
int gg_get_walks(gg_ctx *ctx, int32_t *samples, int32_t *paths, int32_t *path_len, int32_t *root_status);

int gg_prepare_d(gg_ctx *ctx, const int32_t *slots, int32_t n_slots, uint64_t seed, uint32_t stream,
                 int64_t *n_rows_out, int32_t *root_status );
int gg_get_d_data(gg_ctx *ctx, int32_t *center, int32_t *neighbor, float *label);
int gg_prepare_g(gg_ctx *ctx, const int32_t *slots, int32_t n_slots, int32_t n_sample, uint64_t seed,
                 uint32_t stream, int64_t *n_pairs_out, int32_t *root_status);
int gg_prepare_g_begin(gg_ctx *ctx, const int32_t *slots, int32_t n_slots, int32_t n_sample, uint64_t seed, uint32_t stream);
int gg_get_g_data(gg_ctx *ctx, int32_t *node_1, int32_t *node_2, float *reward);

int gg_epoch_begin(gg_ctx *ctx, int32_t reset_d, int32_t reset_g);
int gg_epoch_add(gg_ctx *ctx, const int32_t *roots, int32_t n_roots, int32_t do_d, int32_t do_g, int32_t n_sample, uint64_t seed,
                 uint32_t stream_d, uint32_t stream_g, int64_t *rows_total_out, int64_t *pairs_total_out);
int gg_epoch_commit(gg_ctx *ctx, int32_t which, int64_t *n_out);
int gg_q3_clear(gg_ctx *ctx);
int gg_q3_get(gg_ctx *ctx, int64_t *word_off , uint32_t *words );

int gg_d_pass(gg_ctx *ctx, const int64_t *starts, int64_t n_batches, int32_t batch_size);
int gg_g_pass(gg_ctx *ctx, const int64_t *starts, int64_t n_batches, int32_t batch_size);

int gg_pair_reward(gg_ctx *ctx, const int32_t *u, const int32_t *v, int64_t n, float *out);
int gg_d_step(gg_ctx *ctx, const int32_t *u, const int32_t *v, const float *label, int32_t n);
int gg_g_step(gg_ctx *ctx, const int32_t *u, const int32_t *v, const float *reward, int32_t n);

int gg_all_score(gg_ctx *ctx, const int32_t *rows, int32_t n_rows, float *out);

int gg_all_score_reduce(gg_ctx *ctx, const int32_t *rows, int32_t n_rows, int32_t precision, int32_t want_lse, float *row_max,
                        int32_t *row_argmax, float *row_lse, double *kernel_ms_out);

int gg_topk_scores(gg_ctx *ctx, int32_t which, const int32_t *rows, int32_t n_rows, int32_t k, int32_t precision, int32_t exclude,
                   int32_t *out_col, float *out_score, double *kernel_ms_out);

int gg_rank_scores(gg_ctx *ctx, int32_t which, const int32_t *u, const int32_t *v, int64_t m, int32_t precision, int32_t exclude,
                   int32_t *rank_out, int32_t *n_cand_out, float *score_out, double *kernel_ms_out);

#define GG_GS_FOR_D     1
#define GG_GS_Q3_STORE  2
int gg_graph_softmax(gg_ctx *ctx, const int32_t *slots, int32_t n_slots, int32_t flags,
                     float *logp ,
                     const int64_t *q_off , const int32_t *q_node, float *q_logp,
                     float *abort_mass , double *kernel_ms_out);

int gg_pretrain_set_noise(gg_ctx *ctx, const uint32_t *weight );
int gg_pretrain_set_walk_bias(gg_ctx *ctx, uint32_t w_ret, uint32_t w_com, uint32_t w_out );
int gg_prepare_pretrain(gg_ctx *ctx, const int32_t *starts, int32_t n_starts, int32_t walks_per_start, int32_t walk_len,
                        int32_t window, int32_t n_neg, uint64_t seed, uint32_t stream, int64_t *n_rows_out,
                        int32_t *paths , int32_t *path_len );

int gg_classifier_lossgrad(gg_ctx *ctx, int which, const int32_t *nodes, const int32_t *labels, int64_t m, int n_class,
                           const float *W, const float *b, float l2, float *loss_out, float *gW_out, float *gb_out);
int gg_classifier_fit(gg_ctx *ctx, int which, const int32_t *nodes, const int32_t *labels, int64_t m, int n_class,
                      int iters, float lr, float l2, float *W_inout, float *b_inout, float *loss_out , double *ms_out);
int gg_classifier_predict(gg_ctx *ctx, int which, const int32_t *nodes, int64_t m, int n_class, const float *W, const float *b,
                          int32_t *pred_out, float *logits_out );

int gg_classifier_ml_lossgrad(gg_ctx *ctx, int which, const int32_t *nodes, const uint32_t *label_bits, int64_t m, int n_class,
                              const float *W, const float *b, float l2, float *loss_out, float *gW_out, float *gb_out);
int gg_classifier_ml_fit(gg_ctx *ctx, int which, const int32_t *nodes, const uint32_t *label_bits, int64_t m, int n_class,
                         int iters, float lr, float l2, float *W_inout, float *b_inout, float *loss_out , double *ms_out);
int gg_classifier_ml_predict(gg_ctx *ctx, int which, const int32_t *nodes, int64_t m, int n_class, const float *W, const float *b,
                             const int32_t *k , uint32_t *pred_bits , float *logits_out );

int gg_edge_classifier_lossgrad(gg_ctx *ctx, int which, int op, const int32_t *u, const int32_t *v, const int32_t *y , int64_t m,
                                const float *w, const float *b , float l2, float *loss_out, float *gw_out , float *gb_out );
int gg_edge_classifier_fit(gg_ctx *ctx, int which, int op, const int32_t *u, const int32_t *v, const int32_t *y, int64_t m, int iters,
                           float lr, float l2, float *w_inout, float *b_inout, float *loss_out , double *ms_out);
int gg_edge_classifier_predict(gg_ctx *ctx, int which, int op, const int32_t *u, const int32_t *v, int64_t m, const float *w,
                               const float *b, float *logits_out );

int gg_kmeans_step(gg_ctx *ctx, int which, const int32_t *nodes, int64_t m, int k, const float *centroids ,
                   const int32_t *centroid_nodes , int32_t *assign_out , float *dist2_out ,
                   float *sums_out , int32_t *counts_out , double *inertia_out );
int gg_kmeans_fit(gg_ctx *ctx, int which, const int32_t *nodes, int64_t m, int k, int max_iters, float *centroids_inout ,
                  const int32_t *init_nodes , int32_t *assign_out, float *dist2_out, int32_t *counts_out,
                  double *inertia_out , int32_t *iters_out, int32_t *converged_out, double *ms_out);

int gg_silhouette(gg_ctx *ctx, int which, const int32_t *nodes, const int32_t *assign, int64_t m, int k,
                  const int64_t *rows , int64_t n_rows, int precision ,
                  float *sil_out, float *a_out, float *b_out, int32_t *nearest_out ,
                  double *mean_out , double *ms_out);

int gg_gram(gg_ctx *ctx, int which, const int32_t *nodes, int64_t m, const float *center ,
            double *sums_out , double *gram_out , double *ms_out);

int gg_topk_metric(gg_ctx *ctx, int32_t which, const int32_t *rows, int32_t n_rows, int32_t k, int32_t precision, int32_t metric,
// ... 91 lines not shown
```

Before: 652.1 million.

## Speculatively enqueue discriminator gradient right after row generation, gated on device

After building discriminator rows in prepare_d, the staged discriminator gradient pass (index build plus pair gradient) is enqueued on the stream right away. A device-side go flag, written by d_fill_kernel, gates it so no host round trip is needed first, and the walk finalize waits on an event instead of a full stream sync. A later run_step whose inputs match adopts the speculative work and only runs the finish stage. Any other path that touches discriminator state drops it and clears the hub flags. This is meant to hide host sync latency between row preparation and the gradient step, at the cost of wasted GPU work and extra invalidation logic when the speculation is not used.

```diff
diff --git a/graphgan_amd/_lib.py b/graphgan_amd/_lib.py
--- a/graphgan_amd/_lib.py
+++ b/graphgan_amd/_lib.py
@@ -97,6 +97,7 @@
     "gg_walk_info": (ctypes.c_int, [_P, _P, _P, _P]),
     "gg_get_walks": (ctypes.c_int, [_P, _P, _P, _P, _P]),
     "gg_prepare_d": (ctypes.c_int, [_P, _P, _i32, _u64, _u32, _P, _P]),
+    "gg_debug_early_d": (ctypes.c_int, [_P, _P]),
     "gg_get_d_data": (ctypes.c_int, [_P, _P, _P, _P]),
     "gg_prepare_g": (ctypes.c_int, [_P, _P, _i32, _i32, _u64, _u32, _P, _P]),
     "gg_prepare_g_begin": (ctypes.c_int, [_P, _P, _i32, _i32, _u64, _u32]),
diff --git a/graphgan_amd/csrc/epoch.hip b/graphgan_amd/csrc/epoch.hip
--- a/graphgan_amd/csrc/epoch.hip
+++ b/graphgan_amd/csrc/epoch.hip
@@ -141,8 +141,9 @@
     GG_CHECK(ctx, which == 0 || which == 1, GG_EINVAL, "gg_epoch_commit: which must be 0 (generator pairs) or 1 (discriminator rows)");
     GG_HIP(ctx, hipSetDevice(ctx->device));
     discard_begun_walk(ctx);
+    int rc = which == 1 ? drop_early_d(ctx) : GG_OK;
+    if (rc != GG_OK) return rc;
     GG_HIP(ctx, hipStreamSynchronize(ctx->stream));
-    int rc;
     if (which == 1) {
         const int64_t rows = ctx->ep_rows;
         GG_HIP(ctx, ctx->ep_center.reserve(sizeof(int32_t)));
diff --git a/graphgan_amd/csrc/gg_api.hip b/graphgan_amd/csrc/gg_api.hip
--- a/graphgan_amd/csrc/gg_api.hip
+++ b/graphgan_amd/csrc/gg_api.hip
@@ -238,7 +238,12 @@
     return launch_and_join(ctx, n_slots, total, for_d, seed, stream, stride, !defer_join);
 }
 
-int gg::walk_finalize(gg_ctx *ctx, bool *retried) {
+int gg::walk_enqueue_readback(gg_ctx *ctx) {
+    GG_HIP(ctx, hipMemcpyAsync(ctx->h_pin, ctx->dev_ctr, sizeof(unsigned long long) * 2 * gg_ctx::CTR_WORDS, hipMemcpyDeviceToHost, ctx->stream));
+    return GG_OK;
+}
+
+int gg::walk_finalize(gg_ctx *ctx, bool *retried, hipEvent_t ready) {
     if (retried) *retried = false;
     if (ctx->w_nslots == 0) {
         GG_HIP(ctx, hipStreamSynchronize(ctx->stream));
@@ -247,8 +252,13 @@
     const int64_t total = ctx->w_total;
     unsigned long long *c = ctx->h_pin;
     constexpr int CW = gg_ctx::CTR_WORDS;
-    GG_HIP(ctx, hipMemcpyAsync(c, ctx->dev_ctr, sizeof(unsigned long long) * 2 * CW, hipMemcpyDeviceToHost, ctx->stream));
-    GG_HIP(ctx, hipStreamSynchronize(ctx->stream));
+    if (ready) {
+        GG_HIP(ctx, hipEventSynchronize(ready));
+    } else {
+        const int rc = walk_enqueue_readback(ctx);
+        if (rc != GG_OK) return rc;
+        GG_HIP(ctx, hipStreamSynchronize(ctx->stream));
+    }
     harvest_timings(ctx);
     for (int attempt = 0; c[3] == 2ull || (c[2] != 0ull && ctx->t_lazy); ++attempt) {
         GG_CHECK(ctx, attempt < 16, GG_EHIP, "walk: the launch was voided %d times in a row", attempt);
@@ -375,6 +385,7 @@
     if (const char *om = getenv("GG_COMM_OWNER_MIN")) ctx->owner_min_bound = atoll(om);
     if (const char *dt = getenv("GG_DETERMINISTIC")) ctx->deterministic = atoi(dt) != 0;
     if (const char *nc = getenv("GG_NO_DIST_CACHE")) ctx->dc_enabled = atoi(nc) == 0;
+    if (getenv("GG_NO_EARLY_D_GRAD")) ctx->d_early_on = false;
     if (const char *ft = getenv("GG_FIN_THRESHOLD")) ctx->fin_threshold = std::max(0, atoi(ft));
     if (const char *st = getenv("GG_STAGE_T")) ctx->sg_threshold = std::max(0, atoi(st));
     if (const char *ws = getenv("GG_WALK_SPLIT")) ctx->split_enabled = atoi(ws) != 0;
@@ -414,6 +425,7 @@
         GG_HIP(ctx, hipEventCreateWithFlags(&ctx->ev_walk_done, hipEventDisableTiming));
         GG_HIP(ctx, hipEventCreateWithFlags(&ctx->ev_gen_pass, hipEventDisableTiming));
         GG_HIP(ctx, hipEventCreateWithFlags(&ctx->ev_main_mark, hipEventDisableTiming));
+        GG_HIP(ctx, hipEventCreateWithFlags(&ctx->ev_rows_ready, hipEventDisableTiming));
         GG_HIP(ctx, hipHostMalloc((void **)&ctx->h_pin, sizeof(unsigned long long) * gg_ctx::PIN_WORDS, hipHostMallocDefault));
         memset(ctx->h_pin, 0, sizeof(unsigned long long) * gg_ctx::PIN_WORDS);
         const size_t tb = sizeof(float) * (size_t)n_node * ctx->ld, vb = sizeof(float) * (size_t)n_node;
@@ -487,7 +499,7 @@
                       &ctx->d_ptr, &ctx->g_node1, &ctx->g_node2, &ctx->g_reward, &ctx->g_cnt, &ctx->g_ptr, &ctx->scan_tmp,
                       &ctx->step_u, &ctx->step_v, &ctx->step_x, &ctx->sg_rows, &ctx->sg_bias, &ctx->touched_ptr, &ctx->x_cnt, &ctx->x_send_ids, &ctx->x_send_rows,
                       &ctx->x_recv_ids, &ctx->x_recv_rows, &ctx->x_nglob, &ctx->x_own, &ctx->st_item, &ctx->st_item2, &ctx->st_cur, &ctx->st_prev, &ctx->st_len,
-                      &ctx->st_alive, &ctx->st_rank, &ctx->bfs_key, &ctx->bfs_bm, &ctx->bfs_misc, &ctx->bfs_sparse, &ctx->bfs_rowptr32, &ctx->lv_pfx, &ctx->dc_keys, &ctx->dc_vals, &ctx->dc_words, &ctx->lv_beg, &ctx->lv_k, &ctx->lv_chunks, &ctx->lv_coff, &ctx->lv_scores, &ctx->lv_chunk_owner, &ctx->lv_prefix, &ctx->lv_big, &ctx->lv_fe, &ctx->fin_list, &ctx->table_bad, &ctx->hub_acc,
+                      &ctx->st_alive, &ctx->st_rank, &ctx->bfs_key, &ctx->bfs_bm, &ctx->bfs_misc, &ctx->bfs_sparse, &ctx->bfs_rowptr32, &ctx->lv_pfx, &ctx->dc_keys, &ctx->dc_vals, &ctx->dc_words, &ctx->lv_beg, &ctx->lv_k, &ctx->lv_chunks, &ctx->lv_coff, &ctx->lv_scores, &ctx->lv_chunk_owner, &ctx->lv_prefix, &ctx->lv_big, &ctx->lv_fe, &ctx->fin_list, &ctx->table_bad, &ctx->hub_acc, &ctx->d_early_go,
                       &ctx->q3_store, &ctx->q3s_off, &ctx->ep_center, &ctx->ep_neighbor, &ctx->ep_label, &ctx->ep_node1, &ctx->ep_node2, &ctx->ep_reward, &ctx->topk_adj,
                       &ctx->gs_es, &ctx->gs_cpre, &ctx->pt_starts, &ctx->pt_paths, &ctx->pt_len, &ctx->pt_cnt, &ctx->pt_ptr, &ctx->pt_noise, &ctx->pt_sample};
     for (DevBuf *b : bufs) b->release();
@@ -501,7 +513,7 @@
     for (hipEvent_t e : ctx->pt_ev)
         if (e) (void)hipEventDestroy(e);
     if (ctx->h_pin) (void)hipHostFree(ctx->h_pin);
-    for (hipEvent_t e : {ctx->ev_walk_done, ctx->ev_slots_done, ctx->ev_gen_pass, ctx->ev_main_mark, ctx->ev_fork, ctx->ev_join, ctx->ev_score[0], ctx->ev_score[1]})
+    for (hipEvent_t e : {ctx->ev_walk_done, ctx->ev_slots_done, ctx->ev_gen_pass, ctx->ev_main_mark, ctx->ev_rows_ready, ctx->ev_fork, ctx->ev_join, ctx->ev_score[0], ctx->ev_score[1]})
         if (e) (void)hipEventDestroy(e);
     if (ctx->stream3) {
         (void)hipStreamSynchronize(ctx->stream3);
@@ -908,6 +920,13 @@
     return GG_OK;
 }
 
+int gg_debug_early_d(gg_ctx *ctx, int64_t *out) {
+    if (!ctx || !out) return fail(ctx, GG_EINVAL, "gg_debug_early_d: NULL argument");
+    for (int i = 0; i < 3; ++i) out[i] = ctx->d_early_stats[i];
+    out[3] = ctx->d_early_valid ? 1 : 0;
+    return GG_OK;
+}
+
 int gg_set_tree_mode(gg_ctx *ctx, int32_t mode, int64_t node_cap) {
     if (!ctx) return fail(nullptr, GG_EINVAL, "ctx is NULL");
     GG_CHECK(ctx, mode >= -1 && mode <= 1 && node_cap >= 0, GG_EINVAL, "gg_set_tree_mode: mode must be -1 (auto), 0 (whole trees) or 1 (lazy), node_cap >= 0");
@@ -989,6 +1008,10 @@
     GG_CHECK(ctx, which == 0 || which == 1, GG_EINVAL, "which must be 0 (gen) or 1 (dis)");
     GG_CHECK(ctx, out || in, GG_EINVAL, "buffer is NULL");
     GG_HIP(ctx, hipSetDevice(ctx->device));
+    if (in && which == 1) {
+        const int rc = drop_early_d(ctx);
+        if (rc != GG_OK) return rc;
+    }
     GG_HIP(ctx, hipStreamSynchronize(ctx->stream));
     Model &M = ctx->model[which];
     const int n = ctx->n_node, d = ctx->n_emb, ld = ctx->ld;
@@ -1084,7 +1107,7 @@
 
 int gg::timing_slot(gg_ctx *ctx) {
     for (int s = 0; s < 8; ++s) {
-        bool busy = false;
+        bool busy = s == ctx->d_early_ts;
         for (const auto &t : ctx->tm_pending) busy |= t.slot == s;
         if (busy) continue;
         for (int k = 0; k < 3; ++k)
@@ -1116,6 +1139,10 @@
     if (!ctx) return gg::fail(nullptr, GG_EINVAL, "ctx is NULL");
     GG_CHECK(ctx, path, GG_EINVAL, "state: path is NULL");
     GG_HIP(ctx, hipSetDevice(ctx->device));
+    if (!save) {
+        const int rc0 = drop_early_d(ctx);
+        if (rc0 != GG_OK) return rc0;
+    }
     GG_HIP(ctx, hipStreamSynchronize(ctx->stream));
     if (!save) discard_begun_walk(ctx);
     const bool slots = ctx->cfg.optimizer != GG_OPT_SGD;
diff --git a/graphgan_amd/csrc/gg_internal.h b/graphgan_amd/csrc/gg_internal.h
--- a/graphgan_amd/csrc/gg_internal.h
+++ b/graphgan_amd/csrc/gg_internal.h
@@ -249,6 +249,15 @@
     bool g_slots_ready = false;
     int64_t g_slots_walks = 0; int32_t g_slots_stride = 0;
     int g_slots_unused = 0;
+    bool d_early_on = true;
+    bool d_early_valid = false;
+    int64_t d_early_n = 0;
+    const void *d_early_buf[3] = {};
+    int d_early_ts = -1;
+    int d_early_unused = 0;
+    int64_t d_early_stats[3] = {};
+    gg::DevBuf d_early_go;
+    hipEvent_t ev_rows_ready = nullptr;
     const gg::StageIndex *sg_applying = nullptr;
     gg::DevBuf sg_rows, sg_bias, hub_acc;
     int64_t hub_cap = 0;
@@ -342,7 +351,10 @@
 int walk_launch_async(gg_ctx *ctx, const int32_t *slots, const int32_t *n_walks, int32_t uniform_walks, int32_t n_slots,
                       int32_t for_d, uint64_t seed, uint32_t stream, int32_t stride, bool side_stream = false, bool defer_join = false);
 void discard_begun_walk(gg_ctx *ctx);
-int walk_finalize(gg_ctx *ctx, bool *retried);
+int walk_enqueue_readback(gg_ctx *ctx);
+int walk_finalize(gg_ctx *ctx, bool *retried, hipEvent_t ready = nullptr);
+int enqueue_early_d(gg_ctx *ctx);
+int drop_early_d(gg_ctx *ctx);
 int timing_slot(gg_ctx *ctx);
 int check_exchange_flag(gg_ctx *ctx);
 void harvest_timings(gg_ctx *ctx);
diff --git a/graphgan_amd/csrc/prepare.hip b/graphgan_amd/csrc/prepare.hip
--- a/graphgan_amd/csrc/prepare.hip
+++ b/graphgan_amd/csrc/prepare.hip
@@ -377,9 +377,10 @@
 __global__ __launch_bounds__(256) void d_fill_kernel(const int32_t *slots, const int32_t *t_root, const int64_t *g_rowptr,
                                                      const int32_t *g_col, const int32_t *samples, const int64_t *walk_ptr,
                                                      const int64_t *row_ptr, int n_slots, int32_t *center, int32_t *neighbor,
-                                                     float *label, const unsigned long long *flag) {
+                                                     float *label, const unsigned long long *flag, int64_t expect, int32_t *go) {
     const int lane = threadIdx.x & 63;
     const int i = (blockIdx.x * blockDim.x + threadIdx.x) >> 6;
+    if (blockIdx.x == 0 && threadIdx.x == 0) *go = (*flag != 2ull && row_ptr[n_slots] == expect) ? 1 : 0;
     if (i >= n_slots || *flag == 2ull) return;
     const int64_t o = row_ptr[i], rows = row_ptr[i + 1] - o;
     if (rows == 0) return;
@@ -430,7 +431,7 @@
     hipLaunchKernelGGL(d_fill_kernel, dim3(cdiv((int64_t)n_slots * 64, 256)), dim3(256), 0, ctx->stream,
                        ctx->w_slots_buf().as<int32_t>(), ctx->t_root, ctx->g_rowptr, ctx->g_col, ctx->w_samples.as<int32_t>(),
                        ctx->w_ptr_buf().as<int64_t>(), ctx->d_ptr.as<int64_t>(), n_slots, ctx->d_center.as<int32_t>(),
-                       ctx->d_neighbor.as<int32_t>(), ctx->d_label.as<float>(), ctx->dev_ctr + 3);
+                       ctx->d_neighbor.as<int32_t>(), ctx->d_label.as<float>(), ctx->dev_ctr + 3, 2 * ctx->w_total, ctx->d_early_go.as<int32_t>());
     GG_HIP(ctx, hipMemcpyAsync(ctx->h_pin + gg_ctx::H_TOTAL, ctx->d_ptr.as<int64_t>() + n_slots, sizeof(int64_t), hipMemcpyDeviceToHost, ctx->stream));
     GG_HIP(ctx, hipGetLastError());
     return GG_OK;
@@ -444,8 +445,11 @@
     ctx->d_rows = 0;
     ctx->dc_valid = false;
     discard_begun_walk(ctx);
+    int rc = drop_early_d(ctx);
+    if (rc != GG_OK) return rc;
     ctx->dc_request = ctx->dc_enabled ? 1 : 0;
-    int rc = walk_launch_async(ctx, slots, nullptr, -1, n_slots, 1, seed, stream, stride);
+    const bool sized_launch = ctx->walk_levels > 0 && ctx->lv_cap_chunks == 0;
+    rc = walk_launch_async(ctx, slots, nullptr, -1, n_slots, 1, seed, stream, stride);
     if (rc != GG_OK) { ctx->dc_request = 0; return rc; }
     if (n_slots > 0) {
         const int64_t cap = 2 * ctx->w_total;
@@ -454,20 +458,34 @@
         GG_HIP(ctx, ctx->d_center.reserve(sizeof(int32_t) * (cap + 1)));
         GG_HIP(ctx, ctx->d_neighbor.reserve(sizeof(int32_t) * (cap + 1)));
         GG_HIP(ctx, ctx->d_label.reserve(sizeof(float) * (cap + 1)));
+        GG_HIP(ctx, ctx->d_early_go.reserve(sizeof(int32_t)));
         rc = enqueue_d_rows(ctx, n_slots);
         if (rc != GG_OK) return rc;
+        rc = walk_enqueue_readback(ctx);
+        if (rc != GG_OK) return rc;
+        GG_HIP(ctx, hipEventRecord(ctx->ev_rows_ready, ctx->stream));
+        if (!sized_launch) {
+            rc = enqueue_early_d(ctx);
+            if (rc != GG_OK) return rc;
+        }
     }
     bool retried = false;
-    rc = walk_finalize(ctx, &retried);
+    rc = walk_finalize(ctx, &retried, n_slots > 0 ? ctx->ev_rows_ready : nullptr);
     ctx->dc_request = 0;
-    if (rc != GG_OK) return rc;
+    if (rc != GG_OK) { (void)drop_early_d(ctx); return rc; }
     if (n_slots > 0) {
         if (retried) {
+            rc = drop_early_d(ctx);
+            if (rc != GG_OK) return rc;
             rc = enqueue_d_rows(ctx, n_slots);
             if (rc != GG_OK) return rc;
             GG_HIP(ctx, hipStreamSynchronize(ctx->stream));
         }
         ctx->d_rows = (int64_t)ctx->h_pin[gg_ctx::H_TOTAL];
+        if (ctx->d_early_valid && ctx->d_rows != ctx->d_early_n) {
+            rc = drop_early_d(ctx);
+            if (rc != GG_OK) return rc;
+        }
         ctx->dc_valid = ctx->dc_enabled && ctx->walk_levels > 0;
         if (root_status) GG_HIP(ctx, hipMemcpy(root_status, ctx->w_status.p, sizeof(int32_t) * n_slots, hipMemcpyDeviceToHost));
     }
diff --git a/graphgan_amd/csrc/pretrain.hip b/graphgan_amd/csrc/pretrain.hip
--- a/graphgan_amd/csrc/pretrain.hip
+++ b/graphgan_amd/csrc/pretrain.hip
@@ -329,6 +329,10 @@
         const int rc = ensure_sorted_adjacency(ctx);
         if (rc != GG_OK) return rc;
     }
+    {
+        const int rc = drop_early_d(ctx);
+        if (rc != GG_OK) return rc;
+    }
     ctx->d_rows = 0;
     if (nw > 0) {
         const int64_t rows_bound = nw * (1 + n_neg) * pt_pairs_of_path(walk_len, window);
diff --git a/graphgan_amd/csrc/steps.hip b/graphgan_amd/csrc/steps.hip
--- a/graphgan_amd/csrc/steps.hip
+++ b/graphgan_amd/csrc/steps.hip
@@ -20,6 +20,8 @@
 __device__ __forceinline__ void hub_add(unsigned long long *p, float x, float scale) {
     atomicAdd(p, (unsigned long long)__float2ll_rn(x * scale));
 }
+
+__device__ __forceinline__ bool gate_shut(const int32_t *go) { return go && *go == 0; }
 
 struct StepArgs {
     float *E, *b;
@@ -36,21 +38,22 @@
     const int32_t *slot_v, *slot_u;
     float *stage, *stage_b;
     HubAcc hub;
+    const int32_t *gate;
 };
 
 __global__ __launch_bounds__(256) void pair_occ_count_kernel(const int32_t *u, const int32_t *v, int n, int ppg, int32_t *cnt,
-                                                             int32_t *slot_v, int32_t *slot_u) {
+                                                             int32_t *slot_v, int32_t *slot_u, const int32_t *gate) {
     const int p = blockIdx.x * blockDim.x + threadIdx.x;
-    if (p >= n) return;
+    if (p >= n || gate_shut(gate)) return;
     slot_v[p] = atomicAdd(&cnt[v[p]], 1);
     const bool run_end = p == n - 1 || (p + 1) % ppg == 0 || u[p + 1] != u[p];
     slot_u[p] = run_end ? atomicAdd(&cnt[u[p]], 1) : -2;
 }
 
 __global__ __launch_bounds__(256) void pair_occ_slot_kernel(const int32_t *u, const int32_t *v, int n, const int32_t *cnt, const int32_t *off,
-                                                            int T, int32_t *slot_v, int32_t *slot_u, int32_t *key) {
+                                                            int T, int32_t *slot_v, int32_t *slot_u, int32_t *key, const int32_t *gate) {
     const int p = blockIdx.x * blockDim.x + threadIdx.x;
-    if (p >= n) return;
+    if (p >= n || gate_shut(gate)) return;
     const int iv = v[p], iu = u[p];
     const int sv = cnt[iv] <= T ? off[iv] + slot_v[p] : -3 - off[iv];
     slot_v[p] = sv;
@@ -162,7 +165,7 @@
     const int t = threadIdx.x & 15;
     const int64_t g = ((int64_t)blockIdx.x * blockDim.x + threadIdx.x) >> 4;
     const int64_t p0 = g * 16;
-    if (p0 >= a.n) return;
+    if (p0 >= a.n || (STAGED && gate_shut(a.gate))) return;
     const int np = (int)min((int64_t)16, (int64_t)a.n - p0);
     const float inv_n = a.n_glob ? 1.0f / (float)(*a.n_glob) : a.inv_n;
     const bool mine = t < np;
@@ -1214,13 +1217,13 @@
     return GG_OK;
 }
 
-static int build_from_pairs(gg_ctx *ctx, StageIndex &ix, const int32_t *u, const int32_t *v, int32_t n, int ppg, hipStream_t stream) {
+static int build_from_pairs(gg_ctx *ctx, StageIndex &ix, const int32_t *u, const int32_t *v, int32_t n, int ppg, hipStream_t stream, const int32_t *gate) {
     int32_t *cnt = ix.cnt.as<int32_t>(), *slot_v = ix.slots(), *slot_u = slot_v + n;
-    hipLaunchKernelGGL(pair_occ_count_kernel, dim3(cdiv(n, 256)), dim3(256), 0, stream, u, v, n, ppg, cnt, slot_v, slot_u);
+    hipLaunchKernelGGL(pair_occ_count_kernel, dim3(cdiv(n, 256)), dim3(256), 0, stream, u, v, n, ppg, cnt, slot_v, slot_u, gate);
     const int rc = index_rows(ctx, ix, stream);
     if (rc != GG_OK) return rc;
     hipLaunchKernelGGL(pair_occ_slot_kernel, dim3(cdiv(n, 256)), dim3(256), 0, stream, u, v, n, cnt, ix.off.as<int32_t>(), ctx->sg_threshold, slot_v, slot_u,
-                       ix.key.as<int32_t>());
+                       ix.key.as<int32_t>(), gate);
     GG_HIP(ctx, hipGetLastError());
     return GG_OK;
 }
@@ -1317,24 +1320,96 @@
     }
 }
 
-int run_step(gg_ctx *ctx, int which, const int32_t *d_u, const int32_t *d_v, const float *d_x, int32_t n) {
-    if (n <= 0) return GG_OK;
-    Model &M = ctx->model[which];
-    const int opt = ctx->cfg.optimizer;
+static StepArgs make_step_args(gg_ctx *ctx, int which, const int32_t *d_u, const int32_t *d_v, const float *d_x, int32_t n) {
+    const Model &M = ctx->model[which];
     StepArgs s{};
     s.E = M.E; s.b = M.b; s.gE = ctx->gradE; s.gb = ctx->gradb;
     s.touched = ctx->touched; s.touched_list = ctx->touched_list; s.touched_cnt = ctx->touched_cnt;
     s.ld = ctx->ld;
-    s.track = opt != GG_OPT_ADAM_DENSE;
+    s.track = ctx->cfg.optimizer != GG_OPT_ADAM_DENSE;
     s.u = d_u; s.v = d_v; s.x = d_x; s.n = n;
     s.lambda = M.lambda;
     s.inv_n = 1.0f / (float)n;
     s.is_d = which == 1;
+    s.ppg = n >= 16384 ? PAIRS_PER_GROUP : (n >= 2048 ? 4 : 1);
+    return s;
+}
+
+__global__ __launch_bounds__(256) void clear_hub_flags_kernel(const int32_t *rows, const int64_t *nhub, int64_t cap, int32_t *touched) {
+    const int64_t n = min(*nhub, cap);
+    for (int64_t i = (int64_t)blockIdx.x * blockDim.x + threadIdx.x; i < n; i += (int64_t)gridDim.x * blockDim.x) {
+        const int r = rows[i];
+        if ((unsigned)r < (unsigned)cap) touched[r] = 0;
+    }
+}
+
+int drop_early_d(gg_ctx *ctx) {
+    if (!ctx->d_early_valid) return GG_OK;
+    ctx->d_early_valid = false;
+    ctx->d_early_ts = -1;
+    ctx->d_early_unused++;
+    ctx->d_early_stats[2]++;
+    const StageIndex &ix = ctx->sg_own;
+    const int64_t cap = ctx->n_node;
+    hipLaunchKernelGGL(clear_hub_flags_kernel, dim3((unsigned)std::max<int64_t>(1, std::min<int64_t>(cdiv(cap, 256), 1024))), dim3(256), 0, ctx->stream,
+                       ix.hub.as<int32_t>(), ix.tot.as<int64_t>() + 2, cap, ctx->touched);
+    GG_HIP(ctx, hipGetLastError());
+    return GG_OK;
+}
+
+static bool early_d_matches(const gg_ctx *ctx, const int32_t *u, const int32_t *v, const float *x, int64_t n) {
+    return ctx->d_early_valid && n == ctx->d_early_n && n == ctx->d_rows && u == ctx->d_early_buf[0] && v == ctx->d_early_buf[1] && x == ctx->d_early_buf[2];
+}
+
+int enqueue_early_d(gg_ctx *ctx) {
+    if (!ctx->d_early_on || ctx->comm || ctx->fake_world > 1 || ctx->in_epoch_add || !staged_allowed(ctx)) return GG_OK;
+    if (ctx->d_early_unused >= 2) return GG_OK;
+    const int64_t n = 2 * ctx->w_total;
+    if (n < 16384 || n >= (1 << 30)) return GG_OK;
+    const int fit = staged_reserve(ctx, 2 * n, 2 * n);
+    if (fit < 0) return fit;
+    if (fit != GG_OK) return GG_OK;
+    ctx->d_early_ts = -1;
+    if (ctx->profile_every > 0 && (ctx->pass_call_index[1] % ctx->profile_every) == 0) {
+        ctx->d_early_ts = timing_slot(ctx);
+        if (ctx->d_early_ts >= 0) GG_HIP(ctx, hipEventRecord(ctx->tm_ev[ctx->d_early_ts][0], ctx->stream));
+    }
+    ctx->d_early_valid = true;
+    ctx->d_early_n = n;
+    ctx->d_early_buf[0] = ctx->d_center.p; ctx->d_early_buf[1] = ctx->d_neighbor.p; ctx->d_early_buf[2] = ctx->d_label.p;
+    ctx->d_early_stats[0]++;
+    StepArgs s = make_step_args(ctx, 1, ctx->d_center.as<int32_t>(), ctx->d_neighbor.as<int32_t>(), ctx->d_label.as<float>(), (int32_t)n);
+    s.gate = ctx->d_early_go.as<int32_t>();
+    StageIndex &ix = ctx->sg_own;
+    const int rc = build_from_pairs(ctx, ix, s.u, s.v, s.n, s.ppg, ctx->stream, s.gate);
+    if (rc != GG_OK) return rc;
+    s.slot_v = ix.slots(); s.slot_u = s.slot_v + n;
+    s.stage = ctx->sg_rows.as<float>(); s.stage_b = ctx->sg_bias.as<float>();
+    s.hub = hub_args(ctx, hub_scale(false, n));
+    launch_pair_grad<true>(ctx, s, cdiv((int64_t)cdiv(s.n, s.ppg) * 16, 256), (ctx->ld + 15) / 16);
+    GG_HIP(ctx, hipGetLastError());
+    return GG_OK;
+}
+
+int run_step(gg_ctx *ctx, int which, const int32_t *d_u, const int32_t *d_v, const float *d_x, int32_t n) {
+    if (n <= 0) return GG_OK;
+    if (which == 1 && early_d_matches(ctx, d_u, d_v, d_x, n)) {
+        ctx->d_early_valid = false;
+        ctx->d_early_ts = -1;
+        ctx->d_early_unused = 0;
+        ctx->d_early_stats[1]++;
+        return staged_finish(ctx, 1, n, 2 * (int64_t)n, ctx->sg_own, hub_scale(false, n));
+    }
+    {
+        const int rc = drop_early_d(ctx);
+        if (rc != GG_OK) return rc;
+    }
+    const int opt = ctx->cfg.optimizer;
+    StepArgs s = make_step_args(ctx, which, d_u, d_v, d_x, n);
     if (which == 0) {
         int rc = global_pair_count(ctx, n, &s.n_glob);
         if (rc != GG_OK) return rc;
     }
-    s.ppg = n >= 16384 ? PAIRS_PER_GROUP : (n >= 2048 ? 4 : 1);
     if (ctx->deterministic && n <= DET_MAX_PAIRS) {
         const int nfd = (ctx->ld + 15) / 16;
         const bool replicas = ctx->comm || ctx->fake_world > 1;
@@ -1360,8 +1435,9 @@
     if (fit < 0) return fit;
     if (fit == GG_OK) {
         StageIndex &ix = ctx->sg_own;
-        const int rc = build_from_pairs(ctx, ix, d_u, d_v, n, s.ppg, ctx->stream);
+        const int rc = build_from_pairs(ctx, ix, d_u, d_v, n, s.ppg, ctx->stream, nullptr);
         if (rc != GG_OK) return rc;
+        if (which == 1 && d_u == ctx->d_center.p && n == ctx->d_rows) ctx->d_early_unused = 0;
         s.slot_v = ix.slots(); s.slot_u = s.slot_v + n;
         s.stage = ctx->sg_rows.as<float>(); s.stage_b = ctx->sg_bias.as<float>();
         const float scale = hub_scale(!s.is_d, n);
@@ -1852,6 +1928,11 @@
     if (!ctx) return fail(nullptr, GG_EINVAL, "ctx is NULL");
     if (which == 0) discard_begun_walk(ctx);
     GG_CHECK(ctx, batch_size > 0 && n_batches >= 0 && (starts || n_batches == 0), GG_EINVAL, "pass: bad argument");
+    if (which == 0) {
+        GG_HIP(ctx, hipSetDevice(ctx->device));
+        const int rc = drop_early_d(ctx);
+        if (rc != GG_OK) return rc;
+    }
     const int64_t rows = which == 1 ? ctx->d_rows : ctx->g_pairs;
     const int32_t *u = which == 1 ? ctx->d_center.as<int32_t>() : ctx->g_node1.as<int32_t>();
     const int32_t *v = which == 1 ? ctx->d_neighbor.as<int32_t>() : ctx->g_node2.as<int32_t>();
@@ -1881,8 +1962,12 @@
     const bool whole = n_batches == 1 && starts[0] == 0 && batch_size >= rows && rows > 0;
     ctx->tm_cur = -1;
     if (whole && ctx->profile_every > 0 && (ctx->pass_call_index[which]++ % ctx->profile_every) == 0 && !(ctx->deterministic && rows <= DET_MAX_PAIRS)) {
-        ctx->tm_cur = timing_slot(ctx);
-        if (ctx->tm_cur >= 0) GG_HIP(ctx, hipEventRecord(ctx->tm_ev[ctx->tm_cur][0], ctx->stream));
+        if (which == 1 && ctx->d_early_ts >= 0 && early_d_matches(ctx, u, v, x, rows)) {
+            ctx->tm_cur = ctx->d_early_ts;
+        } else {
+            ctx->tm_cur = timing_slot(ctx);
+            if (ctx->tm_cur >= 0) GG_HIP(ctx, hipEventRecord(ctx->tm_ev[ctx->tm_cur][0], ctx->stream));
+        }
     }
     ctx->step_bound = std::min<int64_t>(batch_size, rows_max);
     if (which == 0 && whole && ctx->g_paths_valid && ctx->cfg.window_size <= 2 && ctx->ld <= 256 && !getenv("GG_NO_PATH_GRAD")) {
diff --git a/graphgan_amd/engine.py b/graphgan_amd/engine.py
--- a/graphgan_amd/engine.py
+++ b/graphgan_amd/engine.py
@@ -214,6 +214,11 @@
     def set_tree_mode(self, mode, node_cap=0):
         self._ck(lib.gg_set_tree_mode(self._ctx, int(mode), int(node_cap)))
         self.tree_mode = (int(mode), int(node_cap))
+
+    def early_d_stats(self):
+        out = np.zeros(4, dtype=np.int64)
+        self._ck(lib.gg_debug_early_d(self._ctx, _ptr(out)))
+        return dict(enqueued=int(out[0]), adopted=int(out[1]), dropped=int(out[2]), pending=bool(out[3]))
 
     def lazy_stats(self):
         out = np.zeros(24, dtype=np.int64)
diff --git a/include/graphgan_hip.h b/include/graphgan_hip.h
--- a/include/graphgan_hip.h
+++ b/include/graphgan_hip.h
@@ -119,6 +119,7 @@
 int gg_walk_info(const gg_ctx *ctx, int64_t *total_walks, int32_t *stride, int32_t *n_slots);
 int gg_get_walks(gg_ctx *ctx, int32_t *samples, int32_t *paths, int32_t *path_len, int32_t *root_status);
 
+int gg_debug_early_d(gg_ctx *ctx, int64_t *out4);
 int gg_prepare_d(gg_ctx *ctx, const int32_t *slots, int32_t n_slots, uint64_t seed, uint32_t stream,
                  int64_t *n_rows_out, int32_t *root_status );
 int gg_get_d_data(gg_ctx *ctx, int32_t *center, int32_t *neighbor, float *label);
```

Result: no change. 656.2 million (median of 2 runs) (+0.6%).
